# shivendrra/shredword-trainer

Measured on AMD Instinct MI355X. Metric: BPE merges/sec, higher is better.
Workload: dtype int32

## Files before the change

### include/shredword_bpe.h

```cpp
#ifndef SHREDWORD_BPE_H
#define SHREDWORD_BPE_H

#include <stddef.h>
#include <stdint.h>

#ifdef __cplusplus
extern "C" {
#endif

typedef struct BPEConfig {
  size_t target_vocab_size;
  int32_t unk_id;
  float character_coverage;
  uint64_t min_pair_freq;
} BPEConfig;

typedef struct Trainer Trainer;

Trainer* create_trainer(const BPEConfig* config);
void bpe_trainer_destroy(Trainer* trainer);
int bpe_load_corpus(Trainer* trainer, const char* input_path);
void bpe_init(Trainer* trainer);
void bpe_count_bigrams(Trainer* trainer);
int bpe_merge_batch(Trainer* trainer, int batch_size);
// ... 11 lines not shown
int updateTokenScores(void* trainer, char** texts, int n);
int trainUnigram(void* trainer, char** texts, int n, int iterations);
int getVocab(void* trainer, char*** tokens, double** scores, int* n);
int saveVocab(void* trainer, const char* path);
int loadVocab(void* trainer, const char* path);

int shred_set_option(Trainer* trainer, const char* key, const char* value);
int shred_reset(Trainer* trainer);
typedef const void* (*shred_gather_fn)(void* ctx, const void* send, size_t nbytes, size_t* out_bytes);
int shred_set_load_gather(Trainer* trainer, int rank, int world, shred_gather_fn gather, void* ctx);
double shred_probe_merge(Trainer* trainer, int32_t a, int32_t b, int iters);
int shred_probe_rollback(Trainer* trainer, int32_t a, int32_t b);
int64_t shred_debug_tokens(Trainer* trainer, int32_t* out, size_t cap);

int64_t shred_index_trace(Trainer* trainer, uint32_t* out, size_t cap);

typedef struct ShredStats {
  double load_seconds, init_seconds, train_seconds;
  double host_select_seconds, host_launch_seconds, host_wait_seconds, host_apply_seconds;
  double merge_kernel_ms, count_kernel_ms;
  double merge_kernel_bytes, count_kernel_bytes;
  uint64_t merge_launches, count_launches;
  uint64_t num_words, num_symbols, num_occurrences, num_merges, heap_size, live_tokens;
  uint64_t device_bytes, num_tiles;
  int32_t layout, world_size;
  uint64_t heap_pops, heap_stale_pops, heap_pushes, delta_records, tiles_visited;
  uint64_t apply_cycles_combine, apply_cycles_order, apply_cycles_walk;
  uint64_t spec_hits, spec_misses;
  uint64_t exchange_overflows;
  double hist_kernel_ms, hist_kernel_bytes;
  uint64_t hist_launches;
  uint64_t resident_launches;
  double resident_ms;
  double resident_latency_us;
  uint64_t load_on_gpu;
  uint64_t index_on;
  uint64_t index_merges, index_undos, index_launches;
  uint64_t index_candidates;
  uint64_t index_changed;
  uint64_t index_occurrences;
  double index_ms;
  double index_dev_us;
  double index_wait_us;
  double index_dev_lookup_us;
  double index_dev_scan_us;
  uint64_t index_scanned;
  double index_build_us;
  uint64_t index_no_sub;
  uint64_t index_staged;
  int64_t index_switch_merge;
  double index_switch_ms;
  uint64_t resident_aborts;
  uint64_t verify_checks;
  uint64_t verify_failures;
  uint64_t resident_merges;
  double resident_bytes;
  double resident_kernel_ms;
  uint64_t index_run_ints_read;
  uint64_t index_run_ints_written;
  uint64_t index_records;
  double resident_k3_bytes;
  uint64_t sel_merges;
  uint64_t sel_launches;
  uint64_t sel_rebuilds;
  double sel_kernel_ms;
  double sel_rebuild_ms;
  double sel_select_us;
  double sel_merge_us;
  uint64_t sel_table_pairs;
  uint64_t sel_table_slots;
  uint64_t sel_host_merges;
  uint64_t sel_table_grows;
  uint64_t index_raw_records;
  uint64_t index_finalized;
  double index_dev_out_us;
  double index_dev_fin_us;
  uint64_t index_fin_records;
  double sel_table_us;
  uint64_t index_spill_merges;
  uint64_t index_spill_keys;
  double host_apply_combine_seconds, host_apply_correct_seconds, host_apply_finish_seconds;
  double host_apply_early_seconds, host_apply_offer_seconds;
  uint64_t helper_adopted, apply_cycles_push;
} ShredStats;
int shred_get_stats(const Trainer* trainer, ShredStats* out);

int shred_device_count(void);

int shred_hbm_probe(int device, size_t bytes, int reps, double* read_gbps, double* copy_gbps);

void* shred_occupy(int device, int free_cus, double max_seconds);
void shred_release(void* handle);

int shred_dist_unique_id(void* out, size_t cap);
int shred_dist_init(int rank, int world_size, const void* unique_id, size_t len, int device);
int shred_dist_finalize(void);
int shred_dist_ranks(void);

#ifdef __cplusplus
}
#endif
#endif
```

### shredword-trainer_amd/csrc/hip/bpe_device.hip

```cpp
#include <algorithm>
#include <cstring>
#include <iterator>

#include "../host/device.h"
#include "../host/dist.h"
#include "hip_common.h"

namespace shred {

namespace {

constexpr uint32_t kFusedCollectMax = 4096;
constexpr uint32_t kNeedCollect = 0x80000000u;
constexpr uint32_t kTimingStride = 8;
constexpr uint32_t kInlineTiles = 768;
constexpr int kGroup = 4;
constexpr uint32_t kWin = 32;
constexpr int kMaxChain = 8;
constexpr int kChainShift = 27;
constexpr uint32_t kMtLds = 256;
[[maybe_unused]] constexpr int kStamps = 18;
#ifdef SHRED_STAMPS
#define STAMP(k) \
  if (threadIdx.x == 0) p.stamps[blockIdx.x * kStamps + (k)] = __builtin_amdgcn_s_memrealtime()
// ... 1437 lines not shown
  const u64* hs = (const u64*)(sl.host_count + 4);
  size_t n;
  const uint32_t nm = launched ? sl.host_count[2] : 0;
  const DeltaRecord* all = sl.host_recs;
  if (exchange_) {
    n = exchange_finish(sl, &all);
  } else {
    n = sl.host_count[0];
    if (n & kNeedCollect) {
      n &= ~kNeedCollect;
      k_collect<<<256, kThreads, 0, S(aux_stream_)>>>(sl.dcount, sl.dlist, U(sl.dsum), U(sl.dft),
                                                        drec + sl.host_count[3]);
      HIP_OK(hipGetLastError());
      k_zero_u32<<<1, 1, 0, S(aux_stream_)>>>(sl.dcount);
      HIP_OK(hipGetLastError());
      HIP_OK(hipStreamSynchronize(S(aux_stream_)));
    }
  }
  if (run_.n == 1) {
    run_.rp[0] = all;
    run_.rn[0] = n;
    run_.tp[0] = sl.host_mlist;
    run_.tn[0] = nm;
  } else {
    for (int i = 0; i < run_.n; ++i) {
      run_.recs[i].clear();
      run_.tiles[i].clear();
    }
    const DeltaRecord* r = all;
    for (size_t i = 0; i < n; ++i) {
      const uint32_t j = r[i].key / keys_per_merge_;
      if (j >= (uint32_t)run_.n) fatal("k_merge record of a merge outside the chain");
      DeltaRecord d = r[i];
      d.key -= j * keys_per_merge_;
      run_.recs[j].push_back(d);
    }
    for (uint32_t i = 0; i < nm; ++i) {
      const uint32_t e = sl.host_mlist[i];
      const uint32_t j = e >> kChainShift;
      if (j >= (uint32_t)run_.n) fatal("k_merge matched tile of a merge outside the chain");
      run_.tiles[j].push_back(e & ((1u << kChainShift) - 1u));
    }
    for (int i = 0; i < run_.n; ++i) {
      run_.rp[i] = run_.recs[i].data();
      run_.rn[i] = run_.recs[i].size();
      run_.tp[i] = run_.tiles[i].data();
      run_.tn[i] = run_.tiles[i].size();
    }
  }
  if (timing_) flush_timing(false);
  if (launched) live_tokens_est_ -= hs[0];
  records_total_ += n;
  records_max_ = std::max<uint64_t>(records_max_, n);
  if (merge_log_) {
    std::fprintf(merge_log_, "C %u %d %u %u %d %llu %zu", sl.seq, run_.X0, sl.n_iter, sl.grid, run_.n,
                 (unsigned long long)hs[0], n);
#ifdef SHRED_STAMPS
    std::vector<u64> st((size_t)sl.grid * kStamps);
    HIP_OK(hipStreamSynchronize(S(stream_)));
    HIP_OK(hipMemcpy(st.data(), stamps_, st.size() * sizeof(u64), hipMemcpyDeviceToHost));
    u64 t0 = ~0ull;
    for (uint32_t g = 0; g < sl.grid; ++g) t0 = std::min(t0, st[(size_t)g * kStamps]);
    for (int k = 1; k < 8; ++k) {
      u64 mx = 0;
      for (uint32_t g = 0; g < sl.grid; ++g) {
        const u64 v = st[(size_t)g * kStamps + k];
        if (v != 0 && v != ~0ull) mx = std::max(mx, v);
      }
      std::fprintf(merge_log_, " %.2f", mx >= t0 ? (double)(mx - t0) / 100.0 : -1.0);
    }
    std::fprintf(merge_log_, " %.0f", st[4] > st[0] ? (double)(st[17] - st[16]) / (double)(st[4] - st[0]) * 100.0 : -1.0);
    for (int k = 8; k < 16; ++k) {
      const u64 v = st[k], s0 = st[0];
      std::fprintf(merge_log_, " %.2f", v >= s0 && v != 0 ? (double)(v - s0) / 100.0 : -1.0);
    }
    HIP_OK(hipMemset(stamps_, 0, st.size() * sizeof(u64)));
#endif
    std::fprintf(merge_log_, "\n");
  }
}

size_t Device::collect(int32_t X, const DeltaRecord** recs) {
  HIP_OK(hipSetDevice(ordinal_));
  last_changes_ = false;
  if (wl_ && wl_->in_flight()) {
    const size_t n = wl_->collect(X, recs);
    last_changes_ = wl_->last_changes();
    records_total_ += n;
    records_max_ = std::max<uint64_t>(records_max_, n);
    return n;
  }
  if (!res_posted_.empty()) return collect_resident(X, recs);
  if (run_count_ == 0) fatal("collect: no launch in flight");
  ChainRun& run = run_at(0);
  const int j = X - run.X0;
  if (j != run.collected || j >= run.n) fatal("collect: merge X is not the next merge of the oldest launch");
  if (!run.waited) finish_launch(run);
  index_.set_tiles(X, run.tp[j], run.tn[j]);
  ++run.collected;
  *recs = run.rp[j];
  const size_t n = run.rn[j];
  if (run.collected == run.n) {
    run_head_ = (run_head_ + 1) & 1;
    --run_count_;
  }
  return n;
}

bool Device::peek(int32_t X, const DeltaRecord** recs, size_t* n) {
  return wl_ && wl_->in_flight() && wl_->peek(X, recs, n);
}

void Device::rollback(int32_t X) {
  HIP_OK(hipSetDevice(ordinal_));
  if (wl_ && wl_->in_flight()) {
    wl_->rollback(X);
    ++rollbacks_;
    return;
  }
  if (!res_posted_.empty()) {
    undo_resident_from(X);
    return;
  }
  park();
  ++rollbacks_;
  for (int k = run_count_ - 1; k >= 0; --k) {
    ChainRun& run = run_at(k);
    const int j0 = std::max(X - run.X0, run.collected);
    if (j0 >= run.n) continue;
    if (!run.waited && run.n == 1) {
      if (ntiles_) unmerge_launch(run, nullptr, 0);
      slot_[run.slot].launched = false;
      run.waited = true;
    } else {
      if (!run.waited) finish_launch(run);
      unmerge_run(run, j0);
    }
    run.n = j0;
  }
  while (run_count_ > 0 && run_at(run_count_ - 1).collected == run_at(run_count_ - 1).n) --run_count_;
}

void Device::unmerge_run(ChainRun& run_, int j0) {
  const int nundo = run_.n - j0;
  if (!ntiles_ || nundo <= 0) return;
  ulist_.clear();
  for (int j = j0; j < j0 + nundo; ++j) ulist_.insert(ulist_.end(), run_.tp[j], run_.tp[j] + run_.tn[j]);
  if (nundo > 1) {
    std::sort(ulist_.begin(), ulist_.end());
    ulist_.erase(std::unique(ulist_.begin(), ulist_.end()), ulist_.end());
  }
  MergeSlot& sl = slot_[run_.slot];
  if (merge_log_) std::fprintf(merge_log_, "R %u %d %zu %d\n", sl.seq, run_.X0 + j0, ulist_.size(), nundo);
  if (ulist_.empty()) return;
  if (unmerge_pending_) HIP_OK(hipStreamSynchronize(S(stream_)));
  std::memcpy(host_ulist_, ulist_.data(), ulist_.size() * sizeof(uint32_t));
  unmerge_pending_ = true;
  unmerge_launch(run_, host_ulist_, ulist_.size(), j0);
}

void Device::unmerge_launch(ChainRun& run_, const uint32_t* tiles, size_t n_tiles, int j0) {
  const int nundo = run_.n - j0;
  MergeSlot& sl = slot_[run_.slot];
  UnmergeParams& up = *static_cast<UnmergeParams*>(unmerge_params_);
  up.tok = tok_;
  up.tile_off = tile_off_;
  up.tile_len = tile_len_;
  if (tiles) {
    void* d = nullptr;
    HIP_OK(hipHostGetDevicePointer(&d, const_cast<uint32_t*>(tiles), 0));
    up.tiles = (const uint32_t*)d;
    up.ntl = (uint32_t)n_tiles;
    up.ntl_dev = nullptr;
  } else {
    up.tiles = (const uint32_t*)sl.dev_mlist;
    up.ntl = 0;
    up.ntl_dev = (const uint32_t*)sl.dev_count + 2;
  }
  up.nundo = nundo;
  up.ux0 = run_.X0 + j0;
  for (int j = 0; j < nundo; ++j) {
    up.ua[j] = run_.ab[2 * (j0 + j)];
    up.ub[j] = run_.ab[2 * (j0 + j) + 1];
  }
  up.dcount = sl.dcount;
  up.dlist = sl.dlist;
  up.dsum = U(sl.dsum);
  up.dft = U(sl.dft);
  up.sig = sig_;
  const int grid = tiles ? (int)std::min<size_t>((n_tiles + kWaves - 1) / kWaves, (size_t)kMaxMergeGroups)
                         : kMaxMergeGroups;
  k_unmerge<<<grid, kThreads, 0, S(stream_)>>>(up);
  HIP_OK(hipGetLastError());
}
// ... 34 lines not shown
```

### shredword-trainer_amd/csrc/hip/word_loop.hip

```cpp
#include <hip/hip_runtime.h>
#include <hipcub/hipcub.hpp>

#include <algorithm>
#include <cstdio>
#include <cstdlib>
#include <cstring>
#include <functional>
#include <thread>
#include <vector>

#include "../host/common.h"
#include "../host/word_loop.h"
#include "hip_common.h"

namespace shred {

namespace {

constexpr int kWlThreads = 512;
constexpr int kDh = 2048;
constexpr int kStripV = 7;
constexpr int kStrip = 4 * kStripV;
constexpr uint32_t kRunHdr = 3;
constexpr uint32_t kStripTok = kStrip - kRunHdr;
constexpr uint32_t kRunAlign = 4;
__host__ __device__ constexpr uint32_t run_cap(uint32_t len) {
  return (kRunHdr + len + kRunAlign - 1u) & ~(kRunAlign - 1u);
}
constexpr int kB = 8;
#ifdef SHRED_WL_NO_PREFETCH
constexpr bool kWlPrefetch = false;
#else
constexpr bool kWlPrefetch = true;
#endif
constexpr int kQ = kWlThreads * kB + kWlThreads;
constexpr int kBSelf = 6;
template <bool kSelf>
struct QueueShape {
  static constexpr int kBatch = kSelf ? kBSelf : kB;
  static constexpr int kCap = kWlThreads * kBatch + kWlThreads;
};
#ifdef SHRED_WL_STAMPS
#define WL_ST(...) __VA_ARGS__
#else
#define WL_ST(...)
#endif
constexpr int kXs = 16;
typedef int v4i_t __attribute__((ext_vector_type(4)));
__device__ __forceinline__ void st16(void* dst, int4 v) {
#ifdef SHRED_WL_NT_WORDS
  v4i_t x = {v.x, v.y, v.z, v.w};
  __builtin_nontemporal_store(x, reinterpret_cast<v4i_t*>(dst));
#else
  *reinterpret_cast<int4*>(dst) = v;
#endif
}
__device__ __forceinline__ void wl_stamp(uint32_t* xs, int i, unsigned long long t0) {
#ifdef SHRED_WL_STAMPS
  const unsigned long long now = __builtin_amdgcn_s_memrealtime();
  if ((threadIdx.x >> 6) == 0 && (threadIdx.x & 63) == (uint32_t)(__ffsll((long long)__ballot(1)) - 1))
    xs[i] = (uint32_t)(now - t0);
#endif
}
constexpr uint32_t kDeltaBucketsDev = 1024;
constexpr uint32_t kRing = 64;
constexpr uint32_t kOpMerge = 1, kOpStop = 2, kOpTimeout = 3, kOpUnmerge = 4;
constexpr uint32_t kNoList = 0xFFFFFFFFu;
constexpr int kStPoolTop = 1, kStError = 3;
constexpr uint32_t kErrPool = 1, kErrList = 2, kErrLookup = 4;

struct WlCmd {
  u64 g[8];
};
constexpr int kCmdGranules = 6;

struct WlSlotDev {
  DeltaRecord* recs;
  uint32_t* hdr;
  uint32_t rec_cap;
};

struct WEnt {
  u64 e;
  u64 sig;
};
__host__ __device__ __forceinline__ u64 hand_weight(uint32_t i) { return 0x9E3779B97F4A7C15ull + 2ull * i; }
constexpr int kCksWord = 30;
constexpr int kGroupShift = 28;
constexpr u64 kWordMask = (1ull << kGroupShift) - 1;
__host__ __device__ __forceinline__ uint32_t ent_groups(u64 e) { return (uint32_t)(e >> kGroupShift) & 0xFu; }

struct SelParams {
  u64* tab;
  u64 pmask;
  uint32_t* fr[2];
  uint32_t fcap;
  uint32_t* st;
  const u64* thr;
  u64* out;
  u64* log;
  u64 log_cap;
  int32_t X0;
  uint32_t n_max;
  u64 min_freq;
  uint32_t fill_max;
  uint32_t probe;
};
constexpr int kSelM = 0, kSelNF = 1, kSelBuf = 2, kSelStatus = 3, kSelIns = 4, kSelErr = 5, kSelStats = 6;
constexpr int kSelWords = kSelStats + 2 * 12 + 2;
constexpr int kSelLogW = kSelStats + 2 * 12;
constexpr uint32_t kSelDone = 1, kSelRebuild = 2, kSelFull = 3;
constexpr uint32_t kSelF = 1536, kSelK = 768, kSelRoom = 384, kSelSlack = 96;
constexpr u64 kCntMask = (1ull << 48) - 1;
constexpr int kPosShift = 48;
template <bool kOn>
struct SelLds {
  u64 key[1], cnt[1];
  uint32_t idx[1], n;
};
constexpr uint32_t kSelIdx = 4096;
template <>
struct SelLds<true> {
  u64 key[kSelF], cnt[kSelF];
  uint32_t idx[kSelIdx / 2], n;
};
struct WlParams {
  int32_t* wtok;
  const u64* weight;
  WEnt* pool;
  u64 pool_cap;
  const u64* dkey;
  const u64* dval;
  u64 dir_mask;
  u64* lst;
  uint32_t* lseq;
  uint32_t id_cap;
  u64* dsum;
  u64* dft;
  uint32_t* dlist;
  uint32_t* dstate;
  uint32_t cap;
  int32_t unk;
  const WlCmd* ring;
  uint32_t* status;
  uint32_t seq0;
  uint32_t idle_polls;
  uint32_t fin_max;
  uint32_t fin_min;
  uint32_t prefetch;
  uint32_t drain;
  uint32_t fast;
  WlSlotDev sl[WordLoop::kSlots];
  SelParams sel;
};

__device__ __forceinline__ u64 pair_key(int32_t a, int32_t b) { return ((u64)(uint32_t)a << 32) | (uint32_t)b; }
__device__ __forceinline__ uint32_t sel_idx_home(u64 k) { return (uint32_t)(mix64(k) >> 40) & (kSelIdx - 1); }
__device__ __forceinline__ int sel_idx_find(const SelLds<true>& F, u64 k) {
  uint32_t h = sel_idx_home(k);
#pragma unroll 1
  for (uint32_t probe = 0; probe < kSelIdx; ++probe) {
    const uint32_t v = (F.idx[h >> 1] >> ((h & 1u) * 16u)) & 0xFFFFu;
    if (v == 0) return -1;
    if (F.key[v - 1u] == k) return (int)(v - 1u);
    h = (h + 1u) & (kSelIdx - 1u);
  }
  return -1;
}
__device__ __forceinline__ bool sel_idx_insert(SelLds<true>& F, u64 k, uint32_t pos) {
  uint32_t h = sel_idx_home(k);
#pragma unroll 1
  for (uint32_t probe = 0; probe < kSelIdx;) {
    const uint32_t sh = (h & 1u) * 16u;
    const uint32_t old = F.idx[h >> 1];
    if (((old >> sh) & 0xFFFFu) == 0u) {
      if (atomicCAS(&F.idx[h >> 1], old, old | ((pos + 1u) << sh)) == old) return true;
      continue;
    }
    h = (h + 1u) & (kSelIdx - 1u);
    ++probe;
  }
  return false;
}

__device__ __forceinline__ u64 nbit(int32_t id, uint32_t s) {
  const uint32_t v = (uint32_t)id * 2u + s;
  return 1ull << ((v ^ (v >> 6) ^ (v >> 12) ^ (v >> 18)) & 63u);
}
__device__ __forceinline__ uint32_t ld_agent(const uint32_t* p) {
  return __hip_atomic_load(p, __ATOMIC_RELAXED, __HIP_MEMORY_SCOPE_AGENT);
}
__device__ __forceinline__ u64 ld_agent64(const u64* p) {
  return __hip_atomic_load(p, __ATOMIC_RELAXED, __HIP_MEMORY_SCOPE_AGENT);
}
__device__ __forceinline__ bool sel_better(u64 c, u64 k, u64 c2, u64 k2) { return c > c2 || (c == c2 && k < k2); }
__device__ __forceinline__ bool sel_at_least(u64 c, u64 k, u64 tc, u64 tk) { return c > tc || (c == tc && k <= tk); }
__device__ __forceinline__ u64 sel_slot(const SelParams& q, u64 pk, uint32_t* ins, uint32_t* err) {
  u64 h = mix64(pk) & q.pmask;
#pragma unroll 1
  for (uint32_t probe = 0; probe < 4096u; ++probe) {
    const u64 cur = ld_agent64(q.tab + 2 * h);
    if (cur == pk) return h;
    if (cur == kEmpty64) {
      const u64 prev = atomicCAS(q.tab + 2 * h, kEmpty64, pk);
      if (prev == kEmpty64) {
        atomicAdd(ins, 1u);
        return h;
      }
      if (prev == pk) return h;
    }
    h = (h + 1) & q.pmask;
  }
  atomicMax(err, 1u);
  return ~0ull;
}
struct SelNew {
  u64* key;
  u64* cnt;
  uint32_t* n;
  uint32_t cap;
  u64* dxa;
  uint32_t* over;
  u64* log;
  uint32_t* nlog;
};
__device__ __forceinline__ void sel_record(const SelParams& q, SelLds<true>& F, const SelNew& nw, int32_t unk,
                                           uint32_t key, u64 sum, int32_t a, int32_t b, int32_t X) {
  const uint32_t sl = key >> 2, cat = key & 3u;
  const int32_t id = sl == 0 ? unk : (int32_t)(sl - 1u);
  if (id == unk || sum == 0) return;
  const int32_t f = cat < 2u ? id : (cat == 2u ? b : X);
  const int32_t g = cat == 0u ? a : (cat == 1u ? X : id);
  if (f == a && g == b) return;
  const u64 pk = pair_key(f, g);
// ... 146 lines not shown
    const int32_t t1 = j + 1 < (int)kStripTok ? run_at(x, (int)kRunHdr + 1 + j) : 0;
    const bool emit = (uint32_t)j < L && !skip;
    const bool m = emit && (uint32_t)(j + 1) < L && t0 == a && t1 == b;
    s[(emit ? kRunHdr + k : 0u) * kWlThreads] = m ? X : t0;
    xm |= (m ? 1u : 0u) << k;
    k += emit ? 1u : 0u;
    skip = m;
  }
  if (xs) wl_stamp(xs, 4, t0);
  *len = k;
  *sig = 0;
  if (!xm) return 0;
  const uint32_t occ = (uint32_t)__popc(xm);
  const u64 rank = (e & kWordMask) << 32;
  uint32_t m = xm, o = 0;
  u64 f = 0;
  while (__ballot(m != 0u)) {
    if (m) {
      const uint32_t ko = (uint32_t)__ffs(m) - 1u;
      m &= m - 1u;
      const uint32_t jo = ko + o;
      ++o;
      const int32_t prev = ko > 0 ? s[(kRunHdr - 1u + ko) * kWlThreads] : 0;
      const bool has_n = jo + 2 < L;
      const int32_t nx = has_n ? s[(kRunHdr + 1u + ko) * kWlThreads] : 0;
      f |= occurrence<kProbes>(p, h, c, ko > 0, prev, has_n, nx == X ? a : nx, wc, rank | ((u64)jo << 2));
    }
  }
  if (xs) wl_stamp(xs, 5, t0);
  *sig = f;
  s[0] = (int32_t)k;
  int4* r4 = reinterpret_cast<int4*>(r);
  const uint32_t q0 = ((uint32_t)__ffs(xm) + kRunHdr - 1u) >> 2;
  int4 v[kStripV];
#pragma unroll
  for (int q = 0; q < kStripV; ++q) {
    v[q].x = s[(4 * q + 0) * kWlThreads];
    v[q].y = s[(4 * q + 1) * kWlThreads];
    v[q].z = s[(4 * q + 2) * kWlThreads];
    v[q].w = s[(4 * q + 3) * kWlThreads];
  }
  v[0].y = x.v[0].y;
  v[0].z = x.v[0].z;
#pragma unroll
  for (int q = 0; q < kStripV; ++q)
    if ((uint32_t)q <= ((k + kRunHdr - 1u) >> 2) && (q == 0 || (uint32_t)q >= q0)) st16(&r4[q], v[q]);
  if (xs) wl_stamp(xs, 6, t0);
  return occ;
}

__device__ __forceinline__ uint32_t unmerge_run(int32_t* t, uint32_t L, int32_t a, int32_t b, int32_t X) {
  uint32_t nx = 0;
  for (uint32_t j = 0; j < L; ++j) nx += t[j] == X;
  if (!nx) return L;
  uint32_t q = L + nx;
  for (uint32_t j = L; j-- > 0;) {
    const int32_t v = t[j];
    if (v == X) {
      t[--q] = b;
      t[--q] = a;
    } else {
      t[--q] = v;
    }
  }
  return L + nx;
}

__device__ __forceinline__ u64 wave_max64(u64 x) { return lane_read64(wave_scan_max64(x), 63); }

__device__ __forceinline__ uint32_t wave_incl_add(uint32_t x) {
  const int lane = threadIdx.x & 63;
#pragma unroll
  for (int d = 1; d < 64; d <<= 1) {
    const uint32_t y = __shfl_up(x, d, 64);
    if (lane >= d) x += y;
  }
  return x;
}

struct LoopS {
  alignas(16) uint32_t hs[32];
  uint32_t cmd[8];
  uint32_t nout, nchg, pool_top, err, scan, filter, nspill, qn, nkeys, nfin;
  uint32_t rd, wr;
  u64 lst_x;
  u64 last_lst;
  int32_t last_x;
  uint32_t st[4];
  u64 lk[2];
  u64 need;
  u64 occ, t[2];
  u64 t_wait, t_idle, t_undo;
  u64 t_seen;
  uint32_t t_rel;
  uint32_t xs[kXs];
  uint32_t sm, snk, snew, status, sel_pos, sover, scompact, sins, serr;
  u64 sel_cnt, dxa, t_rec, t_app, logn;
  uint32_t lognew, newtot;
  u64 bc[kWlThreads / 64], bk[kWlThreads / 64];
  uint32_t bs[kWlThreads / 64];
};


constexpr uint32_t kFinMax = 1024;
constexpr uint32_t kFinTab = 2 * kFinMax;
constexpr u64 kFinEmpty = 0x7FFFFFFF7FFFFFFFull;
static_assert(4 * kFinMax <= (uint32_t)kQ, "record arrays in the queue");
static_assert(3 * kFinTab * 8 <= (uint32_t)(kStrip * kWlThreads * 4), "combine table in the strip");
static_assert(kDeltaBucketsDev * 4 <= kDh * 4, "bucket counters in the hash keys");

__device__ __forceinline__ void fin_record(u64* q, uint32_t r, uint32_t key, u64 sum, u64 ft, int32_t unk, int32_t a,
                                           int32_t b, int32_t X) {
  const uint32_t sl = key >> 2, cat = key & 3u;
  const int32_t id = sl == 0 ? unk : (int32_t)(sl - 1u);
  const int32_t f = cat < 2u ? id : (cat == 2u ? b : X);
  const int32_t g = cat == 0u ? a : (cat == 1u ? X : id);
  q[r] = ((u64)(int64_t)f << 32) | (u64)(int64_t)g;
  q[kFinMax + r] = (cat & 1u) ? sum : (u64)(-(int64_t)sum);
  q[2 * kFinMax + r] = ft;
}

__device__ __forceinline__ void fin_gather(const WlParams& p, DeltaH& h, LoopS& S, u64* q, int32_t a, int32_t b,
                                           int32_t X) {
  const uint32_t tid = threadIdx.x;
  for (int i = tid; i < kDh; i += kWlThreads) {
    const uint32_t key = h.key[i];
    if (key != kEmpty32) fin_record(q, atomicAdd(&S.nout, 1u), key, h.sum[i], h.ft[i], p.unk, a, b, X);
  }
  const uint32_t nsp = S.nspill;
  for (uint32_t i = tid; i < nsp; i += kWlThreads) {
    const uint32_t key = p.dlist[i];
    const u64 sum = atomicExch(&p.dsum[key], 0ull);
    const u64 ft = atomicExch(&p.dft[key], kEmpty64);
    fin_record(q, atomicAdd(&S.nout, 1u), key, sum, ft, p.unk, a, b, X);
  }
}

__device__ uint32_t finalize_wave(const u64* q, const WlSlotDev& sd, int32_t a, int32_t b, uint32_t n) {
  const int lane = threadIdx.x & 63;
  const bool mine = (uint32_t)lane < n;
  const u64 hk = mine ? q[lane] : kFinEmpty;
  const u64 d = mine ? q[kFinMax + lane] : 0ull;
  const u64 ft = mine ? q[2 * kFinMax + lane] : kEmpty64;
  const u64 kab = ((u64)(int64_t)a << 32) | (u64)(int64_t)b;
  u64 sum = 0;
  bool lead = mine && hk != kab;
#pragma unroll 1
  for (uint32_t j = 0; j < n; ++j) {
    const u64 hj = lane_read64(hk, (int)j), fj = lane_read64(ft, (int)j), dj = lane_read64(d, (int)j);
    const bool same = hj == hk;
    sum += same ? dj : 0ull;
    lead = lead && !(same && fj < ft);
  }
  const u64 lm = __ballot(lead);
  const uint32_t bk = (uint32_t)hk & (kDeltaBucketsDev - 1);
  uint32_t r = 0;
#pragma unroll 1
  for (u64 rest = lm; rest; rest &= rest - 1) {
    const uint32_t j = (uint32_t)__builtin_ctzll(rest);
    const uint32_t bj = (uint32_t)__builtin_amdgcn_readlane((int)(uint32_t)hk, (int)j) & (kDeltaBucketsDev - 1);
    const u64 fj = lane_read64(ft, (int)j);
    r += (bj < bk || (bj == bk && fj > ft)) ? 1u : 0u;
  }
  if (lead) {
    u64* dst = reinterpret_cast<u64*>(sd.recs + r);
    dst[0] = hk;
    dst[1] = sum;
    dst[2] = ft;
  }
  return (uint32_t)__popcll(lm);
}

__device__ uint32_t finalize_changes(const WlParams& p, DeltaH& h, LoopS& S, u64* q, u64* tab, const WlSlotDev& sd,
                                     int32_t a, int32_t b, int32_t X, uint32_t n) {
  const uint32_t tid = threadIdx.x;
  const int lane = tid & 63, wid = tid >> 6;
  u64* const fhk = q;
  u64* const fd = q + kFinMax;
  u64* const fft = q + 2 * kFinMax;
  u64* const mft = q + 3 * kFinMax;
  u64* const thk = tab;
  u64* const tft = tab + kFinTab;
  u64* const td = tab + 2 * kFinTab;
  uint32_t* const cnt = h.key;
  fin_gather(p, h, S, q, a, b, X);
  for (uint32_t i = tid; i < kFinTab; i += kWlThreads) {
    thk[i] = kFinEmpty;
    tft[i] = kEmpty64;
    td[i] = 0;
  }
  __syncthreads();
  constexpr int kPer = (int)(kFinMax / kWlThreads);
  uint32_t slot[kPer];
#pragma unroll
  for (int j = 0; j < kPer; ++j) {
    const uint32_t i = tid + (uint32_t)j * kWlThreads;
    slot[j] = 0;
    if (i < n) {
      const u64 hk = fhk[i];
      uint32_t t = (uint32_t)mix64(hk) & (kFinTab - 1);
#pragma unroll 1
// ... 238 lines not shown
        S.cmd[2] = b;
        S.cmd[3] = X;
        S.cmd[4] = (op >> 8) & 0xFFu;
        S.cmd[5] = expect;
        S.cmd[6] = lcnt1;
        S.cmd[7] = loff;
        S.t_wait = t_wait;
      }
    }
    __syncthreads();
    const uint32_t op = S.cmd[0];
    const int32_t a = (int32_t)S.cmd[1], b = (int32_t)S.cmd[2], X = (int32_t)S.cmd[3];
    const uint32_t slot = S.cmd[4], seq = S.cmd[5];
    ++expect;
    if (op != kOpMerge && op != kOpUnmerge) {
      exit_op = kSelf ? S.status : op;
      break;
    }
    const u64 t_cmd = __builtin_amdgcn_s_memrealtime();
    WL_ST(const u64 c_cmd = __builtin_amdgcn_s_memtime();)
    if (wid == 0) {
      const bool undo = op == kOpUnmerge;
      const int32_t M = undo ? X : (a > b ? a : b);
      const bool recent = !undo && M == S.last_x;
      const uint32_t given = undo ? 0u : (S.cmd[6] ? S.cmd[6] : recent ? (uint32_t)(S.last_lst >> 32) + 1u : 0u);
      const uint32_t goff = S.cmd[6] ? S.cmd[7] : (uint32_t)S.last_lst;
      u64 lv64 = 0;
      bool lv = false;
      if (!given && (lane == 16 || lane == 17) && M >= 0 && (uint32_t)M < p.id_cap) {
        if (lane == 16) lv = p.lseq[M] != kNoList;
        if (lane == 17) lv64 = p.lst[M];
      }
      const u64 key = pair_key(a, b);
      const u64 h = mix64(key) & p.dir_mask;
      u64 dk = kEmpty64, dv = 0;
      if (!given && !undo && lane < 16) {
        dk = p.dkey[(h + (u64)lane) & p.dir_mask];
        dv = p.dval[(h + (u64)lane) & p.dir_mask];
      }
      const bool has_list = given || ((__ballot(lv) >> 16) & 1ull);
      const u64 wl = given ? ((u64)goff | ((u64)(given - 1u) << 32)) : __shfl(lv64, 17, 64);
      u64 off = 0, cnt = 0, need = 0;
      bool err = false;
      if (has_list) {
        off = (uint32_t)wl;
        cnt = wl >> 32;
        if (!undo) need = a == b ? nbit(M, 0) : b == M ? nbit(a, 0) : nbit(b, 1);
      } else if (undo) {
        err = true;
      } else {
        for (u64 base = 0;; base += 16) {
          if (base) {
            dk = kEmpty64;
            if (lane < 16) {
              dk = p.dkey[(h + base + (u64)lane) & p.dir_mask];
              dv = p.dval[(h + base + (u64)lane) & p.dir_mask];
            }
          }
          const u64 hit = __ballot(lane < 16 && dk == key);
          const u64 emp = __ballot(lane < 16 && dk == kEmpty64);
          const u64 any = hit | emp;
          if (any) {
            const int f = __ffsll((long long)any) - 1;
            const u64 vf = __shfl(dv, f, 64);
            if ((hit >> f) & 1ull) {
              off = (uint32_t)vf;
              cnt = vf >> 32;
            } else {
              err = true;
            }
            break;
          }
          if (base > p.dir_mask) {
            err = true;
            break;
          }
        }
      }
      if (lane == 0) {
        S.lk[0] = off;
        S.lk[1] = err ? 0 : cnt;
        S.need = need;
        S.nout = 0;
        S.nchg = 0;
        S.scan = 0;
        S.rd = 0;
        S.wr = 0;
        S.nspill = 0;
        S.nkeys = 0;
        S.filter = need != 0;
        S.occ = 0;
        S.err = 0;
        S.st[0] = S.st[1] = S.st[2] = S.st[3] = 0;
        WL_ST(for (int i = 0; i < kXs; ++i) S.xs[i] = 0; S.xs[8] = given ? 1u : 0u;)
        if (err) atomicMax(&p.dstate[kStError], undo ? kErrList : kErrLookup);
        if (!undo && (u64)S.pool_top + cnt > p.pool_cap) {
          S.err = 1;
          atomicMax(&p.dstate[kStError], kErrPool);
        }
        S.t[0] = __builtin_amdgcn_s_memrealtime() - t_cmd;
      }
    }
    __syncthreads();
    WL_ST(if (tid == 0) S.xs[0] = (uint32_t)(__builtin_amdgcn_s_memrealtime() - t_cmd);)
    const u64 off = S.lk[0], cnt = S.lk[1];
    const uint32_t top = S.pool_top;
    if (op == kOpUnmerge) {
      for (u64 i = tid; i < cnt; i += kWlThreads) {
        const u64 e = p.pool[off + i].e;
        int32_t* r = p.wtok + (uint32_t)(e >> 32);
        const uint32_t L = (uint32_t)r[0];
        const uint32_t nl = unmerge_run(r + kRunHdr, L, a, b, X);
        if (nl != L) r[0] = (int32_t)nl;
      }
      __syncthreads();
      if (tid == 0 && X >= 0 && (uint32_t)X < p.id_cap) {
        if (off + cnt == (u64)S.pool_top) S.pool_top = (uint32_t)off;
        p.lseq[X] = kNoList;
        if (S.last_x == X) S.last_x = -1;
      }
      if (tid == 0) {
        S.t_idle += t_cmd - S.t_wait;
        S.t_undo += __builtin_amdgcn_s_memrealtime() - t_cmd;
      }
      __syncthreads();
      continue;
    }
    const bool append = S.err == 0;
    const u64 need = S.need;
    if ((fast || (kSelf && p.fast != 0)) && op == kOpMerge && cnt <= (u64)kWlThreads) {
      u64 e = kEmpty64;
      bool pass = false;
      if (tid < cnt) {
        const WEnt v = p.pool[off + tid];
        e = v.e;
        pass = (v.sig & need) == need;
      }
      WL_ST(if (pass) wl_stamp(S.xs, 2, t_cmd);)
      uint32_t occ = 0, L = 0, nl = 0;
      u64 nsig = 0;
      if (pass) {
        int32_t* r = p.wtok + (uint32_t)(e >> 32);
        const Run x = load_run(r, ent_groups(e));
        const u64 wc = run_weight(x);
        L = (uint32_t)x.v[0].x;
        nl = L;
        WL_ST(wl_stamp(S.xs, 3, t_cmd);)
        if (L >= 2) {
          if (L <= kStripTok) {
            occ = merge_regs<kProbes>(p, s_h, mc, mys, r, x, L, e, wc, a, b, X, &nl, &nsig
                                      WL_ST(, S.xs, t_cmd));
          } else {
            occ = merge_run<kProbes>(p, s_h, mc, r + kRunHdr, L, e, wc, a, b, X, &nl, &nsig);
            if (occ) r[0] = (int32_t)nl;
          }
        }
      }
      const u64 chg = __ballot(occ != 0);
      if (chg) {
        const int lead = __ffsll((long long)chg) - 1;
        uint32_t nb = 0;
        if (lane == lead) nb = atomicAdd(&S.nchg, (uint32_t)__popcll(chg));
        nb = __shfl(nb, lead, 64);
        if (occ && append) {
          WEnt ne;
          ne.e = e;
          ne.sig = nsig;
          st16(&p.pool[(u64)top + nb + (uint32_t)__popcll(chg & ((1ull << lane) - 1ull))],
               make_int4((int)(uint32_t)ne.e, (int)(uint32_t)(ne.e >> 32), (int)(uint32_t)ne.sig, (int)(uint32_t)(ne.sig >> 32)));
        }
      }
      if (const u64 sm = __ballot(pass)) {
        const uint32_t w_occ = wave_sum(occ), w_rd = wave_sum(pass ? 1u + L : 0u);
        const uint32_t w_wr = wave_sum(occ ? 1u + nl : 0u);
        if (lane == 0) {
          atomicAdd(&S.occ, (u64)w_occ);
          atomicAdd(&S.scan, (uint32_t)__popcll(sm));
          atomicAdd(&S.rd, w_rd);
          atomicAdd(&S.wr, w_wr);
        }
      }
      WL_ST(wl_stamp(S.xs, 7, t_cmd);)
      const u64 t_wait = S.t_wait;
      WL_ST(const u64 t_seen_m = S.t_seen;)
      asm volatile("s_waitcnt lgkmcnt(0)\n\ts_barrier" ::: "memory");
      if (p.drain != 0 || S.nspill) __syncthreads();
      WL_ST(wl_stamp(S.xs, 9, t_cmd);)
      if constexpr (!kSelf) {
        const uint32_t nchg = append ? S.nchg : 0u;
        if (wid == 0 && lane == 0 && X >= 0 && (uint32_t)X < p.id_cap) {
          p.lst[X] = (u64)top | ((u64)nchg << 32);
          p.lseq[X] = seq;
        }
        if (wid == kFlagWave) {
          const WlSlotDev& sd = p.sl[slot & (WordLoop::kSlots - 1)];
          const u64 t_out = __builtin_amdgcn_s_memrealtime();
          WL_ST(if (lane == 0) S.xs[12] = (uint32_t)(t_out - t_cmd);)
          const uint32_t nsp = S.nspill;
          uint32_t bw = s_kbits[lane];
          s_kbits[lane] = 0;
          const uint32_t nb = (uint32_t)__popc(bw);
          const uint32_t incl = wave_scan_add(nb);
          const uint32_t nk = (uint32_t)__builtin_amdgcn_readlane((int)incl, 63);
          uint32_t ri = incl - nb;
          WL_ST(if (lane == 0) S.xs[13] = (uint32_t)(__builtin_amdgcn_s_memrealtime() - t_cmd);)
          u64 cks = 0;
          for (; bw; bw &= bw - 1u, ++ri) {
            const uint32_t h = (uint32_t)lane * 32u + (uint32_t)__builtin_ctz(bw);
            u64* dst = reinterpret_cast<u64*>(sd.recs + ri);
            const u64 w0 = (u64)s_h.key[h], w1 = s_h.sum[h], w2 = s_h.ft[h];
            dst[0] = w0;
            dst[1] = w1;
            dst[2] = w2;
            cks += w0 * hand_weight(16u + 3u * ri) + w1 * hand_weight(17u + 3u * ri) + w2 * hand_weight(18u + 3u * ri);
            s_h.key[h] = kEmpty32;
            s_h.sum[h] = 0;
            s_h.ft[h] = kEmpty64;
          }
          WL_ST(if (lane == 0) S.xs[14] = (uint32_t)(__builtin_amdgcn_s_memrealtime() - t_cmd);)
          for (uint32_t i = (uint32_t)lane; i < nsp; i += 64u) {
            const uint32_t key = p.dlist[i];
            const u64 sum = atomicExch(&p.dsum[key], 0ull);
            const u64 ft = atomicExch(&p.dft[key], kEmpty64);
            u64* dst = reinterpret_cast<u64*>(sd.recs + nk + i);
            dst[0] = (u64)key;
            dst[1] = sum;
            dst[2] = ft;
            const uint32_t r = nk + i;
            cks += (u64)key * hand_weight(16u + 3u * r) + sum * hand_weight(17u + 3u * r) + ft * hand_weight(18u + 3u * r);
          }
          WL_ST(if (lane == 0) S.xs[10] = (uint32_t)(__builtin_amdgcn_s_memrealtime() - t_cmd);)
          if (lane == 0) {
            S.lst_x = 0;
            S.last_x = -1;
            if (X >= 0 && (uint32_t)X < p.id_cap) {
              S.pool_top = top + nchg;
              S.lst_x = (u64)top | ((u64)(nchg + 1u) << 32);
              S.last_x = X;
              S.last_lst = (u64)top | ((u64)nchg << 32);
            }
            uint32_t* hs = S.hs;
            u64* hs64 = reinterpret_cast<u64*>(hs);
            const u64 now = __builtin_amdgcn_s_memrealtime();
            hs[0] = nk + nsp;
            hs[1] = 0u;
            hs[2] = (uint32_t)cnt;
            hs[3] = S.nchg;
            hs64[2] = S.occ;
            hs64[3] = now - t_cmd;
            hs64[4] = S.t[0];
            hs64[5] = t_out - t_cmd;
            hs[12] = S.scan;
            hs[13] = S.filter;
            hs[14] = S.rd;
            hs[15] = S.wr;
            hs[16] = hs[17] = hs[18] = 0u;
            hs[19] = nsp;
            hs[20] = (uint32_t)(S.t_idle + (t_cmd - t_wait));
            hs[21] = (uint32_t)S.t_undo;
            hs[22] = 0u;
            hs[23] = nk + nsp;
            hs64[12] = S.lst_x;
            hs64[13] = t_cmd;
            hs64[14] = t_wait;
            hs[30] = (uint32_t)(now - t_out);
            hs[31] = S.t_rel;
            S.t_idle = 0;
            S.t_undo = 0;
          }
          if (lane < 8) {
            const int4 hv = reinterpret_cast<const int4*>(S.hs)[lane];
            reinterpret_cast<int4*>(sd.hdr)[lane] = hv;
            const u64 lo = (u64)(uint32_t)hv.x | ((u64)(uint32_t)hv.y << 32), hi = (u64)(uint32_t)hv.z | ((u64)(uint32_t)hv.w << 32);
            cks += lo * hand_weight(2u * lane) + hi * hand_weight(2u * lane + 1u);
          }
          {
            cks += dpp64<0x111>(cks);
            cks += dpp64<0x112>(cks);
            cks += dpp64<0x114>(cks);
            cks += dpp64<0x118>(cks);
            cks += dpp64<0x142, 0xa, false>(cks);
            cks += dpp64<0x143, 0xc, false>(cks);
            cks = lane_read64(cks, 63);
          }
          if (lane == 0) {
            const u64 t_r0 = __builtin_amdgcn_s_memrealtime();
            WL_ST(sd.hdr[48] = (uint32_t)t_seen_m;
                const u64 c_now = __builtin_amdgcn_s_memtime(); const u64 t_now = __builtin_amdgcn_s_memrealtime();
                  S.xs[1] = (uint32_t)((c_now - c_cmd) * 100ull / (t_now - t_cmd + 1ull));
                  S.xs[11] = (uint32_t)(t_r0 - t_cmd); for (int i = 0; i < kXs; ++i) sd.hdr[32 + i] = S.xs[i];)
            u64* h64w = reinterpret_cast<u64*>(sd.hdr);
            h64w[kCksWord] = ((u64)seq << 32) | (cks & 0xFFFFFFFFull);
            h64w[kCksWord + 1] = ((u64)seq << 32) | (cks >> 32);
            __builtin_amdgcn_fence(__ATOMIC_RELEASE, "");
            S.t_rel = (uint32_t)(__builtin_amdgcn_s_memrealtime() - t_r0);
          }
        } else if (pfon && wid == poll_wave) {
          pre_v = lane < kCmdGranules
                      ? __hip_atomic_load(p.ring[expect % kRing].g + lane, __ATOMIC_RELAXED, __HIP_MEMORY_SCOPE_SYSTEM)
                      : 0ull;
          pre_ok = true;
        }
        continue;
      }
    } else {
    uint32_t my_occ = 0, my_scan = 0, my_rd = 0, my_wr = 0;
    if (tid == 0) S.qn = 0;
    for (u64 base = 0; base < cnt; base += (u64)kWlThreads * kBq) {
      u64 ex[kBq], sx[kBq];
#pragma unroll
      for (int q = 0; q < kBq; ++q) {
        const u64 i = base + (u64)q * kWlThreads + tid;
        ex[q] = kEmpty64;
        sx[q] = 0;
        if (i < cnt) {
          const WEnt v = p.pool[off + i];
          ex[q] = v.e;
          sx[q] = v.sig;
        }
      }
      if (base == 0 && tid == 0) {
        asm volatile("s_waitcnt vmcnt(0)" ::: "memory");
        S.st[0] = (uint32_t)(__builtin_amdgcn_s_memrealtime() - t_cmd);
      }
#pragma unroll
      for (int q = 0; q < kBq; ++q) {
        const bool pass = ex[q] != kEmpty64 && (sx[q] & need) == need;
        const u64 bl = __ballot(pass);
        if (bl) {
          const int lead = __ffsll((long long)bl) - 1;
          uint32_t qb = 0;
          if (lane == lead) qb = atomicAdd(&S.qn, (uint32_t)__popcll(bl));
          qb = __shfl(qb, lead, 64);
          if (pass) s_q[qb + (uint32_t)__popcll(bl & ((1ull << lane) - 1ull))] = ex[q];
        }
      }
      __syncthreads();
      const uint32_t qn = S.qn;
      __syncthreads();
      const bool last = base + (u64)kWlThreads * kBq >= cnt;
      if (qn < (uint32_t)kWlThreads && !last) continue;
      WL_ST(if (tid == 0) { if (!S.xs[1]) S.xs[1] = (uint32_t)(__builtin_amdgcn_s_memrealtime() - t_cmd); ++S.xs[9]; })
      const uint32_t qend = ((qn + kWlThreads - 1) / kWlThreads) * kWlThreads;
      u64 e_n = kEmpty64;
      Run x_n{};
      if (kWlPrefetch && tid < qn) {
        e_n = s_q[tid];
        x_n = load_run(p.wtok + (uint32_t)(e_n >> 32), ent_groups(e_n));
      }
      for (uint32_t qi = tid; qi < qend; qi += kWlThreads) {
        if (!kWlPrefetch && qi < qn) {
          e_n = s_q[qi];
          x_n = load_run(p.wtok + (uint32_t)(e_n >> 32), ent_groups(e_n));
        }
        const u64 e = e_n;
        const Run x = x_n;
        const u64 wc = run_weight(x);
// ... 154 lines not shown
        for (uint32_t i = tid; i < kSelIdx / 2; i += kWlThreads) s_f.idx[i] = 0;
        asm volatile("s_waitcnt lgkmcnt(0)\n\ts_barrier" ::: "memory");
        const uint32_t b0 = base;
#pragma unroll
        for (int j = 0; j < kPer; ++j) {
          const uint32_t i = (uint32_t)kPer * tid + (uint32_t)j;
          if (i >= n0 || !((keepm >> j) & 1u)) continue;
          s_f.cnt[base] = ck[j];
          s_f.key[base] = kk[j];
          ++base;
        }
        asm volatile("s_waitcnt lgkmcnt(0)\n\ts_barrier" ::: "memory");
        for (uint32_t i = b0; i < base; ++i)
          if (!sel_idx_insert(s_f, s_f.key[i], i)) S.sover = 1;
        asm volatile("s_waitcnt lgkmcnt(0)\n\ts_barrier" ::: "memory");
        if (tid == 0) {
          s_f.n = tot;
          ++S.scompact;
          if (tot > kSelF - kSelRoom) S.sover = 1;
        }
      }
      if (tid == 0) {
        q.st[kSelNF] = min(s_f.n, kSelF);
        q.st[kSelM] = S.sm + 1u;
        ++S.sm;
        u64* t64 = reinterpret_cast<u64*>(q.st + kSelStats);
        const u64 now = __builtin_amdgcn_s_memrealtime();
        t64[0] += t_cmd - S.t_wait;
        t64[1] += now - t_cmd;
        t64[2] += cnt;
        t64[3] += nchg;
        t64[4] += S.occ;
        t64[5] += nnew;
        t64[6] += now - t_tab;
        t64[7] += S.scompact ? 1u : 0u;
        t64[8] += S.t_rec - t_tab;
        t64[9] += S.t_app - S.t_rec;
        t64[10] += now - S.t_app;
        q.st[kSelBuf] = S.scompact;
        S.status = S.sover ? kSelRebuild : 0u;
      }
      __syncthreads();
      if (S.status) {
        exit_op = S.status;
        break;
      }
      continue;
    }
    const WlSlotDev& sd = p.sl[slot & (WordLoop::kSlots - 1)];
    if (tid == 0) {
      S.t[1] = __builtin_amdgcn_s_memrealtime() - t_cmd;
      S.lst_x = 0;
      if (X >= 0 && (uint32_t)X < p.id_cap) {
        p.lst[X] = (u64)top | ((u64)nchg << 32);
        p.lseq[X] = seq;
        S.pool_top = top + nchg;
        S.lst_x = (u64)top | ((u64)(nchg + 1u) << 32);
      }
      S.last_x = S.lst_x ? X : -1;
      S.last_lst = (u64)top | ((u64)nchg << 32);
    }
    const uint32_t nrec = S.nkeys + S.nspill;
    const bool fin = p.fin_max != 0 && nrec <= p.fin_max && nrec <= kFinMax && nrec >= p.fin_min;
    const u64 t_fin = __builtin_amdgcn_s_memrealtime();
    if (fin && nrec <= 64u) {
      fin_gather(p, s_h, S, s_q, a, b, X);
      __syncthreads();
      if (wid == 0) {
        const uint32_t m = finalize_wave(s_q, sd, a, b, nrec);
        if (lane == 0) S.nfin = m;
      }
      asm volatile("s_waitcnt vmcnt(0)" ::: "memory");
    } else if (fin) {
      finalize_changes(p, s_h, S, s_q, reinterpret_cast<u64*>(s_strip), sd, a, b, X, nrec);
      asm volatile("s_waitcnt vmcnt(0)" ::: "memory");
    } else if (pfon && wid == 1) {
      pre_v = lane < kCmdGranules
                  ? __hip_atomic_load(p.ring[expect % kRing].g + lane, __ATOMIC_RELAXED, __HIP_MEMORY_SCOPE_SYSTEM)
                  : 0ull;
      pre_ok = true;
    } else {
      const uint32_t rt = pfon ? (tid < 64u ? tid : tid - 64u) : tid;
      const uint32_t rs = pfon ? (uint32_t)kWlThreads - 64u : (uint32_t)kWlThreads;
      for (uint32_t i = rt; i < (uint32_t)kDh; i += rs) {
        const uint32_t key = s_h.key[i];
        if (key == kEmpty32) continue;
        const uint32_t r = atomicAdd(&S.nout, 1u);
        u64* dst = reinterpret_cast<u64*>(sd.recs + r);
        dst[0] = (u64)key;
        dst[1] = s_h.sum[i];
        dst[2] = s_h.ft[i];
        s_h.key[i] = kEmpty32;
        s_h.sum[i] = 0;
        s_h.ft[i] = kEmpty64;
      }
      const uint32_t nsp = S.nspill;
      for (uint32_t i = rt; i < nsp; i += rs) {
        const uint32_t key = p.dlist[i];
        const u64 sum = atomicExch(&p.dsum[key], 0ull);
        const u64 ft = atomicExch(&p.dft[key], kEmpty64);
        const uint32_t r = atomicAdd(&S.nout, 1u);
        u64* dst = reinterpret_cast<u64*>(sd.recs + r);
        dst[0] = (u64)key;
        dst[1] = sum;
        dst[2] = ft;
      }
      asm volatile("s_waitcnt vmcnt(0)" ::: "memory");
    }
    asm volatile("s_waitcnt lgkmcnt(0)\n\ts_barrier" ::: "memory");
    WL_ST(if (tid == 0) S.xs[10] = (uint32_t)(__builtin_amdgcn_s_memrealtime() - t_cmd);)
    if (fin)
      for (int i = tid; i < kDh; i += kWlThreads) {
        s_h.key[i] = kEmpty32;
        s_h.sum[i] = 0;
        s_h.ft[i] = kEmpty64;
      }
    if (tid == 0) {
      sd.hdr[0] = fin ? S.nfin : S.nout;
      sd.hdr[22] = fin ? 1u : 0u;
      sd.hdr[23] = nrec;
      sd.hdr[30] = (uint32_t)(__builtin_amdgcn_s_memrealtime() - t_fin);
      sd.hdr[2] = (uint32_t)cnt;
      sd.hdr[3] = S.nchg;
      u64* h64 = reinterpret_cast<u64*>(sd.hdr);
      h64[2] = S.occ;
      h64[3] = (u64)__builtin_amdgcn_s_memrealtime() - t_cmd;
      h64[4] = S.t[0];
      h64[5] = S.t[1];
      sd.hdr[12] = S.scan;
      sd.hdr[13] = S.filter;
      sd.hdr[14] = S.rd;
      sd.hdr[15] = S.wr;
      sd.hdr[16] = S.st[0];
      sd.hdr[17] = S.st[1];
      sd.hdr[18] = S.st[2];
      sd.hdr[19] = S.nspill;
      sd.hdr[20] = (uint32_t)(S.t_idle + (t_cmd - S.t_wait));
      sd.hdr[21] = (uint32_t)S.t_undo;
      sd.hdr[31] = S.t_rel;
      h64[12] = S.lst_x;
      h64[13] = t_cmd;
      h64[14] = S.t_wait;
      S.t_idle = 0;
      S.t_undo = 0;
      const u64 t_r0 = __builtin_amdgcn_s_memrealtime();
      WL_ST(S.xs[11] = (uint32_t)(t_r0 - t_cmd); for (int i = 0; i < kXs; ++i) sd.hdr[32 + i] = S.xs[i];)
      __hip_atomic_store(sd.hdr + 1, seq, __ATOMIC_RELEASE, __HIP_MEMORY_SCOPE_SYSTEM);
      S.t_rel = (uint32_t)(__builtin_amdgcn_s_memrealtime() - t_r0);
    }
    asm volatile("s_waitcnt lgkmcnt(0)\n\ts_barrier" ::: "memory");
  }
  if (tid == 0) {
    p.dstate[kStPoolTop] = S.pool_top;
    if constexpr (kSelf) {
      p.sel.st[kSelIns] = S.sins;
      *reinterpret_cast<u64*>(p.sel.st + kSelLogW) = S.logn;
      p.sel.st[kSelErr] = S.serr;
      p.sel.st[kSelStatus] = exit_op;
      __threadfence_system();
      return;
    }
    p.status[1] = expect - 1u;
    __threadfence_system();
    __hip_atomic_store(&p.status[0], exit_op, __ATOMIC_RELEASE, __HIP_MEMORY_SCOPE_SYSTEM);
  }
}

namespace {

__global__ void k_wl_pair_counts(const int32_t* wtok, const uint32_t* woff, uint32_t W, uint32_t* cnt) {
  for (uint32_t w = blockIdx.x * blockDim.x + threadIdx.x; w <= W; w += gridDim.x * blockDim.x) {
    const uint32_t L = w < W ? (uint32_t)wtok[woff[w]] : 0u;
    cnt[w] = L >= 2 ? L - 1 : 0u;
  }
}
__global__ void k_wl_emit_pairs(const int32_t* wtok, const uint32_t* woff, const uint32_t* base, uint32_t W,
                                int32_t unk, u64* key, uint32_t* val) {
  for (uint32_t w = blockIdx.x * blockDim.x + threadIdx.x; w < W; w += gridDim.x * blockDim.x) {
    const uint32_t o = woff[w], b = base[w], np = base[w + 1] - b;
    const int32_t* t = wtok + o + kRunHdr;
    for (uint32_t j = 0; j < np; ++j) {
      const int32_t x = t[j], y = t[j + 1];
      key[b + j] = (x != unk && y != unk) ? pair_key(x, y) : kEmpty64;
      val[b + j] = w;
    }
  }
}

__global__ void k_wl_mark(const u64* key, const uint32_t* val, uint64_t n, uint32_t* keep, uint32_t* head) {
  for (uint64_t i = blockIdx.x * (uint64_t)blockDim.x + threadIdx.x; i < n; i += (uint64_t)gridDim.x * blockDim.x) {
    const u64 k = key[i];
    const bool valid = k != kEmpty64;
    const bool first_key = valid && (i == 0 || key[i - 1] != k);
    keep[i] = valid && (first_key || val[i - 1] != val[i]);
    head[i] = first_key;
  }
}

__global__ void k_wl_scatter(const u64* key, const uint32_t* val, uint64_t n, const uint32_t* keep,
                             const uint32_t* pos, const uint32_t* head, const uint32_t* kidx, const uint32_t* woff,
                             WEnt* pool, u64* ikey, u64* ival) {
  for (uint64_t i = blockIdx.x * (uint64_t)blockDim.x + threadIdx.x; i < n; i += (uint64_t)gridDim.x * blockDim.x) {
// ... 136 lines not shown
    }
    const u64 bl = __ballot(take);
    if (!bl) continue;
    const int lead = __ffsll((long long)bl) - 1;
    uint32_t base = 0;
    if (lane == lead) base = atomicAdd(nout, (uint32_t)__popcll(bl));
    base = __shfl(base, lead, 64);
    const uint32_t pos = base + (uint32_t)__popcll(bl & ((1ull << lane) - 1ull));
    if (take && pos < cap) out[pos] = (uint32_t)i;
  }
}

__global__ void k_sel_gather(const uint32_t* slots, uint32_t n, const u64* tab, u64* key, u64* negc, uint32_t* idx) {
  for (uint32_t i = blockIdx.x * blockDim.x + threadIdx.x; i < n; i += gridDim.x * blockDim.x) {
    key[i] = tab[2 * (u64)slots[i]];
    negc[i] = ~(tab[2 * (u64)slots[i] + 1] & kCntMask);
    idx[i] = i;
  }
}

__global__ void k_sel_pick(const uint32_t* slots, const uint32_t* idx, uint32_t n, uint32_t* fr) {
  for (uint32_t i = blockIdx.x * blockDim.x + threadIdx.x; i < n; i += gridDim.x * blockDim.x)
    fr[i] = slots[idx ? idx[i] : i];
}

__global__ void k_sel_insert(const PairCount* pc, uint64_t n, SelParams q) {
  for (uint64_t i = blockIdx.x * (uint64_t)blockDim.x + threadIdx.x; i < n; i += (uint64_t)gridDim.x * blockDim.x) {
    const u64 h = sel_slot(q, pair_key(pc[i].a, pc[i].b), q.st + kSelIns, q.st + kSelErr);
    if (h != ~0ull) q.tab[2 * h + 1] = pc[i].count & kCntMask;
  }
}

__global__ void k_sel_apply_log(const u64* log, u64 n, SelParams q) {
  for (u64 i = blockIdx.x * (u64)blockDim.x + threadIdx.x; i < n; i += (u64)gridDim.x * blockDim.x) {
    const u64 h = sel_slot(q, log[2 * i], q.st + kSelIns, q.st + kSelErr);
    if (h != ~0ull) atomicAdd(q.tab + 2 * h + 1, log[2 * i + 1]);
  }
}

__global__ void k_sel_clear(u64* tab, u64 n) {
  for (u64 i = blockIdx.x * (u64)blockDim.x + threadIdx.x; i < n; i += (u64)gridDim.x * blockDim.x) {
    tab[2 * i] = kEmpty64;
    tab[2 * i + 1] = 0;
  }
}

__global__ void k_sel_export(const u64* tab, u64 cap, PairCount* out, uint32_t* n) {
  for (u64 i = blockIdx.x * (u64)blockDim.x + threadIdx.x; i < cap; i += (u64)gridDim.x * blockDim.x) {
    const u64 k = tab[2 * i], c = tab[2 * i + 1] & kCntMask;
    if (k == kEmpty64 || c == 0) continue;
    const uint32_t j = atomicAdd(n, 1u);
    out[j] = PairCount{(int32_t)(uint32_t)(k >> 32), (int32_t)(uint32_t)k, c, 0};
  }
}

template <class T>
T* wl_alloc(size_t n, size_t* acc) {
  void* p = nullptr;
  HIP_OK(hipMalloc(&p, std::max<size_t>(n, 1) * sizeof(T)));
  *acc += std::max<size_t>(n, 1) * sizeof(T);
  return static_cast<T*>(p);
}

constexpr uint32_t kRunPad = 4 * kStripV + 4;

}

WordLoop::WordLoop(int ordinal, void* stream, int32_t unk_id) : ordinal_(ordinal), stream_(stream), unk_(unk_id) {
  HIP_OK(hipSetDevice(ordinal_));
  const unsigned pin = hipHostMallocMapped | hipHostMallocCoherent;
  HIP_OK(hipHostMalloc(&ring_, sizeof(WlCmd) * kRing, pin));
  std::memset(ring_, 0, sizeof(WlCmd) * kRing);
  HIP_OK(hipHostGetDevicePointer(&ring_dev_, ring_, 0));
  HIP_OK(hipHostMalloc((void**)&status_, 64, pin));
  std::memset(status_, 0, 64);
  HIP_OK(hipHostGetDevicePointer(&status_dev_, status_, 0));
  if (const char* e = std::getenv("SHREDWORD_WL_IDLE_POLLS")) idle_polls_ = (uint32_t)std::strtoul(e, nullptr, 10);
  if (const char* e = std::getenv("SHREDWORD_WL_FINALIZE")) fin_max_ = (uint32_t)std::strtoul(e, nullptr, 10);
  if (const char* e = std::getenv("SHREDWORD_WL_FIN_MIN")) fin_min_ = (uint32_t)std::strtoul(e, nullptr, 10);
  if (const char* e = std::getenv("SHREDWORD_WL_PREFETCH")) prefetch_ = std::atoi(e) != 0;
  if (const char* e = std::getenv("SHREDWORD_WL_DRAIN")) drain_ = std::atoi(e) != 0;
  if (const char* e = std::getenv("SHREDWORD_WL_PROBES")) probes_ = std::atoi(e);
  if (const char* e = std::getenv("SHREDWORD_WL_FAST")) fast_ = std::atoi(e) != 0;
  if (const char* e = std::getenv("SHREDWORD_SELECT_REPORT")) sel_report_ = std::atoi(e) != 0;
  for (auto& e : ev_) {
    hipEvent_t ev;
    HIP_OK(hipEventCreate(&ev));
    e = ev;
  }
}

WordLoop::~WordLoop() {
  (void)hipSetDevice(ordinal_);
  if (running_ && posted_.empty()) stop();
  (void)hipStreamSynchronize(S(stream_));
  free_all();
  for (Slot& s : slot_) {
    if (s.host_recs) (void)hipHostFree(s.host_recs);
    if (s.host_hdr) (void)hipHostFree(s.host_hdr);
  }
  if (ring_) (void)hipHostFree(ring_);
  if (status_) (void)hipHostFree(status_);
  for (auto e : ev_)
    if (e) (void)hipEventDestroy((hipEvent_t)e);
}

void WordLoop::free_all() {
  sel_free();
  void* ptrs[] = {wtok_, wtok0_, woff_, tile_first_, tile_nw_, pool_, dkey_, dval_, init_key_, init_val_,
                  lst_, lseq_, dsum_, dft_, dlist_, dstate_};
  for (void* p : ptrs)
    if (p) HIP_OK(hipFree(p));
  wtok_ = wtok0_ = nullptr;
  woff_ = tile_first_ = tile_nw_ = lseq_ = dlist_ = dstate_ = nullptr;
  pool_ = dkey_ = dval_ = init_key_ = init_val_ = lst_ = dsum_ = dft_ = nullptr;
  cap_ = id_cap_ = 0;
  dir_cap_ = 0;
  bytes_ = 0;
  ready_ = false;
}

bool WordLoop::upload(const TiledStream& ts, const uint64_t* d_weight) {
  HIP_OK(hipSetDevice(ordinal_));
  if (running_) stop();
  free_all();
  const size_t T = ts.num_tiles();
  const int P = (int)std::max<size_t>(1, std::min<size_t>({16, std::max(1u, std::thread::hardware_concurrency()),
                                                          T / 64 + 1}));
  auto par = [&](const std::function<void(int)>& f) {
    if (P == 1) return f(0);
    std::vector<std::thread> pool;
    for (int k = 0; k < P; ++k) pool.emplace_back(f, k);
    for (auto& th : pool) th.join();
  };
  auto range = [&](int k, size_t* t0, size_t* t1) {
    *t0 = T * (size_t)k / (size_t)P;
    *t1 = T * (size_t)(k + 1) / (size_t)P;
  };
  std::vector<uint32_t> tnw(T, 0), tfirst(T, 0);
  std::vector<uint64_t> tints(T + 1, 0), ttok(T, 0);
  std::vector<int32_t> tr0(T, -1);
  std::vector<char> bad((size_t)P, 0);
  par([&](int k) {
    size_t t0, t1;
    range(k, &t0, &t1);
    for (size_t t = t0; t < t1 && !bad[(size_t)k]; ++t) {
      const int32_t* p = ts.tok.data() + ts.off[t];
      uint32_t nw = 0, wl = 0;
      uint64_t ints = 0, ntk = 0;
      for (uint32_t i = 0; i < ts.len[t]; ++i) {
        if (p[i] < kHeaderLimit) {
          const int32_t r = (int32_t)(uint32_t)(p[i] - kHeaderBase);
          if (nw == 0) tr0[t] = r;
          else if (r != tr0[t] + (int32_t)nw) bad[(size_t)k] = 1;
          if (nw) ints += run_cap(wl);
          ++nw;
          wl = 0;
        } else {
          if (nw == 0) bad[(size_t)k] = 1;
          ++wl;
          ++ntk;
        }
      }
      if (nw) ints += run_cap(wl);
      tnw[t] = nw;
      tints[t] = ints;
// ... 232 lines not shown

void WordLoop::ensure_slots(uint32_t cap) {
  const uint32_t rec_cap = 4 * (cap + 1) + 64;
  const unsigned pin = hipHostMallocMapped | hipHostMallocNonCoherent;
  for (Slot& sl : slot_) {
    if (sl.host_recs) HIP_OK(hipHostFree(sl.host_recs));
    HIP_OK(hipHostMalloc((void**)&sl.host_recs, (size_t)rec_cap * sizeof(DeltaRecord), pin));
    HIP_OK(hipHostGetDevicePointer(&sl.dev_recs, sl.host_recs, 0));
    if (!sl.host_hdr) {
      HIP_OK(hipHostMalloc((void**)&sl.host_hdr, 256, pin));
      std::memset(sl.host_hdr, 0, 256);
      HIP_OK(hipHostGetDevicePointer(&sl.dev_hdr, sl.host_hdr, 0));
    }
    sl.rec_cap = rec_cap;
  }
}

void WordLoop::reserve(int32_t max_id) {
  const uint32_t need = (uint32_t)std::max<int32_t>(max_id, 0) + 2 + kSlots;
  if (need <= cap_ && dsum_) return;
  if (!posted_.empty()) fatal("WordLoop::reserve with a merge in flight");
  stop();
  uint32_t cap = std::max<uint32_t>(cap_ ? cap_ : 4096, 4096);
  while (cap < need) cap *= 2;
  hipStream_t s = S(stream_);
  for (void* p : {(void*)dsum_, (void*)dft_, (void*)dlist_})
    if (p) HIP_OK(hipFree(p));
  const size_t keys = 4 * ((size_t)cap + 1);
  dsum_ = wl_alloc<u64>(keys, &bytes_);
  dft_ = wl_alloc<u64>(keys, &bytes_);
  dlist_ = wl_alloc<uint32_t>(keys, &bytes_);
  HIP_OK(hipMemsetAsync(dsum_, 0, keys * sizeof(u64), s));
  HIP_OK(hipMemsetAsync(dft_, 0xFF, keys * sizeof(u64), s));
  u64* nl = wl_alloc<u64>(cap, &bytes_);
  uint32_t* ns = wl_alloc<uint32_t>(cap, &bytes_);

  HIP_OK(hipMemsetAsync(ns, 0xFF, (size_t)cap * sizeof(uint32_t), s));

  if (lseq_) {
    HIP_OK(hipMemcpyAsync(nl, lst_, (size_t)id_cap_ * sizeof(u64), hipMemcpyDeviceToDevice, s));
    HIP_OK(hipMemcpyAsync(ns, lseq_, (size_t)id_cap_ * sizeof(uint32_t), hipMemcpyDeviceToDevice, s));

    HIP_OK(hipStreamSynchronize(s));
    for (void* q : {(void*)lst_, (void*)lseq_}) HIP_OK(hipFree(q));
  }
  lst_ = nl;
  lseq_ = ns;

  id_cap_ = cap;
  cap_ = cap;
  lists_.resize(cap, 0ull);
  ensure_slots(cap);
  HIP_OK(hipStreamSynchronize(s));
}

void WordLoop::launch(uint32_t seq0) {
  WlParams p{};
  p.wtok = wtok_;
  p.weight = weight_;
  p.pool = reinterpret_cast<WEnt*>(pool_);
  p.pool_cap = pool_cap_;
  p.dkey = dkey_;
  p.dval = dval_;
  p.dir_mask = dir_cap_ - 1;
  p.lst = lst_;
  p.lseq = lseq_;

  p.id_cap = id_cap_;
  p.dsum = dsum_;
  p.dft = dft_;
  p.dlist = dlist_;
  p.dstate = dstate_;
  p.cap = cap_;
  p.unk = unk_;
  p.ring = static_cast<const WlCmd*>(ring_dev_);
  p.status = static_cast<uint32_t*>(status_dev_);
  p.seq0 = seq0;
  p.idle_polls = idle_polls_;
  p.fin_max = fin_max_;
  p.fin_min = fin_min_;
  p.prefetch = prefetch_ ? 1u : 0u;
  p.drain = drain_ ? 1u : 0u;
  p.fast = fast_ ? 1u : 0u;
  for (int k = 0; k < kSlots; ++k) {
    p.sl[k].recs = static_cast<DeltaRecord*>(slot_[k].dev_recs);
    p.sl[k].hdr = static_cast<uint32_t*>(slot_[k].dev_hdr);
    p.sl[k].rec_cap = slot_[k].rec_cap;
  }
  status_[0] = 0;
  HIP_OK(hipEventRecord((hipEvent_t)ev_[0], S(stream_)));
  switch (probes_) {
    case 0: k_word_loop<false, 0><<<1, kWlThreads, 0, S(stream_)>>>(p); break;
    case 1: k_word_loop<false, 1><<<1, kWlThreads, 0, S(stream_)>>>(p); break;
    default: k_word_loop<false, kProbesDefault><<<1, kWlThreads, 0, S(stream_)>>>(p); break;
  }
  HIP_OK(hipGetLastError());
  HIP_OK(hipEventRecord((hipEvent_t)ev_[1], S(stream_)));
  running_ = true;
  ++st_.launches;
}

void WordLoop::recover_timeout() {
  HIP_OK(hipStreamSynchronize(S(stream_)));
  running_ = false;
  const uint32_t next = __atomic_load_n(&status_[1], __ATOMIC_ACQUIRE);
  if (next != seq_ + 1) {
    if (seq_ + 1 - next > kRing) fatal("k_word_loop: more commands behind its time-out than the ring holds");
    launch(next);
  }
}

uint32_t WordLoop::post(uint32_t op, int32_t a, int32_t b, int32_t X, uint32_t loff, uint32_t lcnt1) {
  if (running_ && __atomic_load_n(&status_[0], __ATOMIC_ACQUIRE) == kOpTimeout) recover_timeout();
  if (!running_) {
    if (op == kOpStop) return 0;
    launch(seq_ + 1);
  }
  const uint32_t seq = ++seq_;
  const uint32_t slot = (uint32_t)X & (kSlots - 1);
  u64* g = static_cast<WlCmd*>(ring_)[seq % kRing].g;
  const uint32_t vals[kCmdGranules] = {op | (slot << 8), (uint32_t)a, (uint32_t)b, (uint32_t)X, loff, lcnt1};
  for (int k = 0; k < kCmdGranules; ++k) __atomic_store_n(&g[k], (u64)seq | ((u64)vals[k] << 32), __ATOMIC_RELAXED);
  std::atomic_thread_fence(std::memory_order_release);
  return seq;
}

void WordLoop::post_merge(int32_t a, int32_t b, int32_t X) {
  if (!ready_) fatal("WordLoop::post_merge before upload");
  if (posted_.size() >= (size_t)kSlots) fatal("WordLoop: every merge slot is in flight");
  if (X < 0 || (uint32_t)X + 2 > cap_) fatal("WordLoop: merge id beyond the reserved ids");
  const int32_t M = a > b ? a : b;
  const uint64_t l = M >= 0 && (size_t)M < lists_.size() ? lists_[M] : 0;
  const uint32_t seq = post(kOpMerge, a, b, X, (uint32_t)l, (uint32_t)(l >> 32));
  posted_.push_back({X, a, b, seq, now_seconds()});
  dirty_ = true;
}

bool WordLoop::handed_over(const Slot& sl, uint32_t seq) const {
  const uint64_t* h64 = reinterpret_cast<const uint64_t*>(sl.host_hdr);
  const uint64_t g0 = __atomic_load_n(&h64[kCksWord], __ATOMIC_ACQUIRE), g1 = __atomic_load_n(&h64[kCksWord + 1], __ATOMIC_ACQUIRE);
  if ((uint32_t)(g0 >> 32) != seq || (uint32_t)(g1 >> 32) != seq) return false;
  const uint64_t want = (g0 & 0xFFFFFFFFull) | (g1 << 32);
  const uint32_t n = __atomic_load_n(&sl.host_hdr[0], __ATOMIC_ACQUIRE);
  if (n > sl.rec_cap) return false;
  uint64_t c = 0;
  for (uint32_t i = 0; i < 16; ++i) c += __atomic_load_n(&h64[i], __ATOMIC_RELAXED) * hand_weight(i);
  const uint64_t* r = reinterpret_cast<const uint64_t*>(sl.host_recs);
  for (uint32_t i = 0; i < 3 * n; ++i) c += __atomic_load_n(&r[i], __ATOMIC_RELAXED) * hand_weight(16u + i);
  return c == want;
}

void WordLoop::wait_flag(const Slot& sl, uint32_t seq) {
  volatile uint32_t* flag = sl.host_hdr + 1;
  const uint64_t* h64 = reinterpret_cast<const uint64_t*>(sl.host_hdr);
  const double t0 = now_seconds();
  unsigned spins = 0;
  for (;;) {
    if (__atomic_load_n(flag, __ATOMIC_ACQUIRE) == seq) break;
    if ((uint32_t)(__atomic_load_n(&h64[kCksWord + 1], __ATOMIC_ACQUIRE) >> 32) == seq && handed_over(sl, seq)) break;
    __builtin_ia32_pause();
    if (++spins % 4096 != 0) continue;
    const uint32_t st = __atomic_load_n(&status_[0], __ATOMIC_ACQUIRE);
    if (st == kOpTimeout) {
      recover_timeout();
    } else if (st != 0) {
      fatal("k_word_loop ended with a merge in flight");
    }
    if (now_seconds() - t0 > 60.0) {
      const hipError_t e = hipStreamQuery(S(stream_));
      if (e != hipSuccess && e != hipErrorNotReady) HIP_OK(e);
      if (now_seconds() - t0 > 300.0) fatal("k_word_loop did not signal completion within 300 s");
    }
  }
}

size_t WordLoop::collect(int32_t X, const DeltaRecord** recs) {
  if (posted_.empty() || posted_.front().X != X) fatal("WordLoop::collect: X is not the oldest posted merge");
  const Post pp = posted_.front();
  posted_.erase(posted_.begin());
  const Slot& sl = slot_[(uint32_t)X & (kSlots - 1)];
  wait_flag(sl, pp.seq);
  const double t_seen = now_seconds();
  st_.wait_us += 1e6 * (t_seen - pp.t_post);
  const uint32_t* h = sl.host_hdr;
  const uint64_t* h64 = reinterpret_cast<const uint64_t*>(h);
  const size_t n = h[0];
  st_.merges += 1;
  st_.candidates += h[2];
  st_.scanned += h[12];
  st_.run_ints_read += h[14];
  st_.run_ints_written += h[15];
  st_.records += h[0];
  st_.raw_records += h[22] ? h[23] : h[0];
  st_.finalized += h[22] ? 1u : 0u;
  st_.dev_out_us += 1e-2 * (double)h[30];
  st_.dev_rel_us += 1e-2 * (double)h[31];
  st_.spill_merges += h[19] ? 1u : 0u;
  st_.spill_keys += h[19];
  if (h[22]) {
    st_.dev_fin_us += 1e-2 * (double)h[30];
    st_.fin_records += h[23];
  }
  last_changes_ = h[22] != 0;
  st_.changed += h[3];
  st_.occurrences += h64[2];
  st_.dev_us += 1e-2 * (double)h64[3];
  st_.dev_lookup_us += 1e-2 * (double)h64[4];
  st_.dev_scan_us += 1e-2 * (double)(h64[5] - h64[4]);
  if (timing_) {
    const uint32_t rec[kTraceFields] = {(uint32_t)X, h[2], h[12], h[3], (uint32_t)h64[2], (uint32_t)(10 * h64[3]),
                                        (uint32_t)(10 * h64[4]), (uint32_t)(10 * (h64[5] - h64[4])),
                                        10 * h[16], 10 * h[17], 10 * h[18], h[19], 10 * h[20],
                                        10 * h[21], (uint32_t)(1e9 * (t_seen - pp.t_post)),
                                        (uint32_t)(1e8 * (pp.t_post - t_epoch_)), (uint32_t)(1e8 * (t_seen - t_epoch_)),
                                        (uint32_t)h64[13], (uint32_t)h64[14],
                                        h[32], h[33], h[34], h[35], h[36], h[37], h[38], h[39], h[40], h[41],
                                        h[42], h[43], h[44], h[45], h[46], h[47],
                                        h[31], h[48]};
    trace_.insert(trace_.end(), rec, rec + kTraceFields);
  }
  if (n > sl.rec_cap) fatal("k_word_loop: record overflow");
  if (h64[12] && (size_t)X < lists_.size()) lists_[X] = h64[12];
  *recs = sl.host_recs;
  return n;
}

bool WordLoop::peek(int32_t X, const DeltaRecord** recs, size_t* n) const {
  if (posted_.empty() || posted_.front().X != X) return false;
  const Slot& sl = slot_[(uint32_t)X & (kSlots - 1)];
  if (__atomic_load_n(sl.host_hdr + 1, __ATOMIC_ACQUIRE) != posted_.front().seq &&
      !handed_over(sl, posted_.front().seq))
    return false;
  if (sl.host_hdr[22]) return false;
  const size_t k = sl.host_hdr[0];
  if (k > sl.rec_cap) return false;
  *recs = sl.host_recs;
  *n = k;
  return true;
}

void WordLoop::rollback(int32_t X) {
  while (!posted_.empty() && posted_.back().X >= X) {
    const Post pp = posted_.back();
    posted_.pop_back();
    post(kOpUnmerge, pp.a, pp.b, pp.X);
    ++st_.undos;
  }
}

void WordLoop::stop() {
  if (!running_) return;
  HIP_OK(hipSetDevice(ordinal_));
  if (!posted_.empty()) fatal("WordLoop::stop with a merge in flight");
  post(kOpStop, 0, 0, 0);
  HIP_OK(hipStreamSynchronize(S(stream_)));
  running_ = false;
  float ms = 0;
  HIP_OK(hipEventElapsedTime(&ms, (hipEvent_t)ev_[0], (hipEvent_t)ev_[1]));
  st_.kernel_ms += ms;
  uint32_t ds[8];
  HIP_OK(hipMemcpy(ds, dstate_, sizeof(ds), hipMemcpyDeviceToHost));

  if (std::getenv("SHREDWORD_WL_REPORT") && st_.merges)
    std::fprintf(stderr, "[WL] %llu merges: device %.2f us a merge, of it the flag's system release %.2f us, "
                 "records out %.2f us; %llu merges spilled %llu delta keys to HBM\n", (unsigned long long)st_.merges,
                 st_.dev_us / (double)st_.merges, st_.dev_rel_us / (double)st_.merges,
                 st_.dev_out_us / (double)st_.merges, (unsigned long long)st_.spill_merges,
                 (unsigned long long)st_.spill_keys);
  if (ds[kStError]) {
    static const char* what[] = {"", "index pool exhausted", "an undone merge had no word list", "",
                                 "a merged pair had no word list"};
    std::fprintf(stderr, "[ERROR]\t k_word_loop: %s (code %u)\n", ds[kStError] < 5 ? what[ds[kStError]] : "?",
                 ds[kStError]);
    fatal("k_word_loop failed");
  }
}


void WordLoop::sel_free() {
  void* ptrs[] = {ptab_, fr_[0], fr_[1], sst_dev_, thr_, sout_, upd_, shist_, scol_};
  for (void* q : ptrs)
    if (q) HIP_OK(hipFree(q));
  ptab_ = thr_ = sout_ = nullptr;
  fr_[0] = fr_[1] = sst_dev_ = upd_ = shist_ = scol_ = nullptr;
  pcap_ = sout_cap_ = upd_cap_ = scol_cap_ = 0;
  fcap_ = 0;
}

bool WordLoop::sel_rebuild(uint64_t min_freq) {
  const double t0 = now_seconds();
  hipStream_t s = S(stream_);
  HIP_OK(hipMemsetAsync(shist_, 0, kSelBuckets * sizeof(uint32_t), s));
  k_sel_hist<<<1024, 512, 0, s>>>(ptab_, pcap_, min_freq, shist_);
  HIP_OK(hipGetLastError());
  std::vector<uint32_t> hist(kSelBuckets);
  HIP_OK(hipMemcpyAsync(hist.data(), shist_, kSelBuckets * sizeof(uint32_t), hipMemcpyDeviceToHost, s));
  HIP_OK(hipStreamSynchronize(s));
  uint64_t acc = 0;
  uint32_t bstar = kSelBuckets;
  for (uint32_t b = kSelBuckets; b-- > 0;) {
    if (!hist[b]) continue;
    acc += hist[b];
    bstar = b;
    if (acc >= kSelK) break;
  }
  uint32_t st[kSelStats] = {};
  HIP_OK(hipMemcpyAsync(st, sst_dev_, sizeof(st), hipMemcpyDeviceToHost, s));
  HIP_OK(hipStreamSynchronize(s));
  u64 thr[2] = {~0ull, 0ull};
  uint32_t nf = 0;
  if (acc > 0) {
    if (acc > scol_cap_) {
      if (scol_) HIP_OK(hipFree(scol_));
      scol_cap_ = std::max<uint64_t>(2 * acc, 1 << 16);
      scol_ = wl_alloc<uint32_t>(scol_cap_ + 1, &bytes_);
    }
// ... 293 lines not shown
```

### shredword-trainer_amd/csrc/host/device.h

```cpp
#pragma once

#include <algorithm>
#include <cstddef>
#include <cstdio>
#include <cstdint>
#include <string>
#include <vector>

#include "corpus.h"
#include "engine.h"
#include "selector.h"
#include "tiles.h"
#include "word_loop.h"

namespace shred {

struct KernelTimes {
  double merge_ms = 0;
  double compact_ms = 0;
  double count_ms = 0;
  uint64_t merge_launches = 0;
  uint64_t count_launches = 0;
  double merge_bytes = 0;
  double count_bytes = 0;
  double hist_ms = 0;
  double hist_bytes = 0;
  uint64_t hist_launches = 0;
  uint64_t res_merges = 0;
  double res_bytes = 0;
  double res_k3_bytes = 0;
  double res_ms = 0;
};

class Device : public Backend {
 public:
  static bool available(std::string* why);
  static int hbm_probe(int ordinal, size_t bytes, int reps, double* read_gbps, double* copy_gbps);
  static void* occupy(int ordinal, int free_cus, double max_seconds);
  static void release(void* handle);

  explicit Device(int device_ordinal);
  ~Device();
  Device(const Device&) = delete;
  Device& operator=(const Device&) = delete;

  void upload(const TiledStream& ts, Layout layout, const std::vector<uint64_t>& weights, int32_t max_id);
  void reset_tokens();
  bool has_tokens() const { return ntiles_ > 0 || uploaded_; }

  void count_pairs(int32_t unk_id, std::vector<PairCount>* out) override;
  void pair_max(int32_t unk_id, int32_t a, int32_t b, uint64_t* max_freq, uint64_t* ab_freq) override;

  void merge_chain(const int32_t* ab, int n, int32_t X0) override;
  int device_select(const std::vector<PairCount>& pairs, int32_t X0, int n, uint64_t min_freq,
                    std::vector<SelectedMerge>* out) override;
  bool device_select_now() const override { return !hybrid_resident_phase() || switch_pending_; }
  struct Exchange {
    int rank = 0, world = 1;
    void* comm = nullptr;
    void (*allgather)(void* comm, const void* send, void* recv, size_t bytes, void* stream) = nullptr;
    uint32_t bucket_records = 1024;
  };
  void set_exchange(const Exchange& x);
  size_t collect(int32_t X, const DeltaRecord** recs) override;
  bool records_are_changes() const override { return last_changes_; }
  bool peek(int32_t X, const DeltaRecord** recs, size_t* n) override;
  static constexpr int kChainMax = 8;
  int max_chain() const override {
    return speculate_ && !resident_eligible() && !index_eligible() ? kChainMax : 1;
  }
  bool index_id_room(int32_t max_id) const;
  bool can_overlap() const override {
    if (switch_pending_) return false;
    if (index_eligible()) return speculate_ && index_id_room(max_id_seen_ + 1 + spec_depth_);
    return speculate_ && (!resident_eligible() || (uint32_t)max_id_seen_ + 3 < min_slot_cap());
  }
  static constexpr int kResSlots = 4;
  int overlap_depth() const override { return resident_eligible() || index_eligible() ? spec_depth_ : 1; }
  int max_guesses() const override { return resident_eligible() || index_eligible() ? kResSlots - 1 : 1; }
  void set_spec_depth(int d) { spec_depth_ = std::max(1, std::min(d, kResSlots - 1)); }
  uint32_t min_slot_cap() const {
    uint32_t c = UINT32_MAX;
    for (const MergeSlot& s : slot_) c = std::min(c, s.cap);
    return c;
  }
  void reserve_ids(int32_t max_id) override;
  uint64_t exchange_overflows() const { return x_overflows_; }
  void rollback(int32_t X) override;
  void quiesce() override { park(); }
  void park();
  void set_resident(bool on);
  bool resident() const { return resident_on_; }
  bool resident_eligible() const { return resident_on_ && resident_ok_ && !exchange_ && !index_eligible(); }
  void set_index(bool on);
  bool index_on() const { return index_on_; }
  bool hybrid_resident_phase() const {
    return hybrid_ && !idx_phase_ && resident_on_ && resident_ok_ && !exchange_ && ntiles_ > 0;
  }
  bool index_eligible() const {
    return index_on_ && wl_ && wl_->ready() && !exchange_ && !hybrid_resident_phase();
  }
  void set_hybrid(bool on) {
    park();
    hybrid_ = on;
  }
  void set_switch_occurrences(uint64_t n) { switch_occ_ = n; }
  void set_finalize(int64_t n) {
    fin_ = n;
    if (wl_ && n >= 0) {
      index_sync();
      wl_->set_finalize((uint32_t)n);
    }
  }
  int64_t switch_merge() const { return switch_x_; }
  double switch_ms() const { return switch_ms_; }
  const WordLoop* word_loop() const { return wl_; }
  uint64_t resident_launches() const { return res_launches_; }
  uint64_t resident_aborts() const { return res_aborts_; }
  bool resident_tokens_in_lds() const { return res_lds_tok_; }
  double resident_ms() const { return res_ms_; }
  double resident_latency_us() const { return res_lat_n_ ? res_lat_us_ / (double)res_lat_n_ : 0.0; }
  void set_speculation(bool on) { speculate_ = on; }
  uint64_t rollbacks() const { return rollbacks_; }
  void set_merge_groups(int groups);

  void token_freq(size_t T, std::vector<uint64_t>* freq) override;
  void download_tokens(std::vector<int32_t>* out);

  void set_timing(bool on) {
    timing_ = on;
    if (wl_) wl_->set_timing(on);
  }
  const KernelTimes& times() {
    flush_timing(true);
    return times_;
  }
  void set_unk(int32_t unk) { unk_ = unk; }
  uint64_t records_total() const { return records_total_; }
  uint64_t visited_tiles() const { return visited_tiles_; }
  uint64_t records_max() const { return records_max_; }
  void clear_times() {
    flush_timing(true);
    times_ = KernelTimes();
    records_total_ = records_max_ = 0;
    visited_tiles_ = 0;
    res_launches_ = 0;
    res_ms_ = res_lat_us_ = 0;
    res_lat_n_ = 0;
// ... 47 lines not shown
    int32_t ab[2 * kChainMax] = {};
    const DeltaRecord* rp[kChainMax] = {};
    size_t rn[kChainMax] = {};
    const uint32_t* tp[kChainMax] = {};
    size_t tn[kChainMax] = {};
    std::vector<DeltaRecord> recs[kChainMax];
    std::vector<uint32_t> tiles[kChainMax];
  };
  void ensure_slots(MergeSlot& s, uint32_t need);
  void free_slot(MergeSlot& s, bool keep_host);
  void free_all();
  void wait_flag(const MergeSlot& s);
  void finish_launch(ChainRun& run);
  size_t exchange_bucket_bytes() const { return 32 + (size_t)xchg_.bucket_records * 24; }
  void exchange_launch(MergeSlot& sl);
  size_t exchange_finish(MergeSlot& sl, const DeltaRecord** recs);
  void count_pairs_dense(int32_t unk_id, uint64_t live, std::vector<PairCount>* out);
  struct PairMaxQuery {
    int32_t a, b;
    uint64_t max_freq, ab_freq;
  };
  PairMaxQuery* pmq_ = nullptr;
  void reduce_pair_max(const PairCount* dout, uint32_t n);
  void unmerge_run(ChainRun& run, int j0);
  void unmerge_launch(ChainRun& run, const uint32_t* tiles, size_t n_tiles, int j0 = 0);
  void flush_timing(bool block);
  void rebuild_signatures();

  int ordinal_ = 0;
  void* stream_ = nullptr;
  void* aux_stream_ = nullptr;
  void* ev_[6] = {};
  static constexpr int kEvPairs = 16;
  void* mev_[kEvPairs][2] = {};
  struct PendingEv {
    int pair;
    double bytes;
  };
  std::vector<PendingEv> ev_pending_;
  std::vector<int> ev_free_;
  bool timing_ = false;
  KernelTimes times_;
  Exchange xchg_;
  bool exchange_ = false;
  uint8_t* xrecv2_ = nullptr;
  size_t xrecv2_bytes_ = 0;
  std::vector<uint8_t> xstage_;
  uint64_t x_overflows_ = 0;
  int cu_count_ = 256;
  bool uploaded_ = false;
  Layout layout_ = Layout::kTypes;

  size_t ntiles_ = 0;
  size_t tok_elems_ = 0;
  int32_t* tok_ = nullptr;
  int32_t* tok0_ = nullptr;
  uint64_t* tile_off_ = nullptr;
  uint32_t* tile_len_ = nullptr;
  uint32_t* tile_len0_ = nullptr;
  uint64_t* weight_ = nullptr;
  uint64_t live_tokens0_ = 0;
  uint32_t* sig_ = nullptr;
  unsigned long long* stamps_ = nullptr;
  uint64_t nentries_ = 0;
  size_t ft_tiles_ = 0;
  uint64_t ft_live_tokens_ = 0;
  uint64_t live_tokens_est_ = 0;

  MergeSlot slot_[kResSlots];
  ChainRun runs_[2];
  int run_head_ = 0, run_count_ = 0;
  ChainRun& run_at(int k) { return runs_[(run_head_ + k) & 1]; }
  uint32_t keys_per_merge_ = 0;
  uint32_t* host_ulist_ = nullptr;
  void* dev_ulist_ = nullptr;
  std::vector<uint32_t> ulist_;
  bool unmerge_pending_ = false;
  uint32_t seq_ = 0;
  int32_t unk_ = 0;
  uint64_t records_total_ = 0, records_max_ = 0;
  int32_t max_id_seen_ = 0;
  int32_t max_id0_ = 0;
  bool speculate_ = true;
  bool last_changes_ = false;
  int64_t fin_ = -1;
  uint64_t rollbacks_ = 0;

  void* merge_params_ = nullptr;
  void* unmerge_params_ = nullptr;
  int max_groups_ = 256;
  FILE* merge_log_ = nullptr;
  TileIndex index_;
  bool skip_ = true;
  std::vector<uint32_t> cand_, cand1_, cand2_;
  uint64_t visited_tiles_ = 0;
  int merge_blocks_per_cu_ = 4;

  size_t bytes_alloc_ = 0;

  void index_sync();
  void index_refresh();
  WordLoop* wl_ = nullptr;
  bool index_on_ = true;
  bool words_stale_ = false;
  bool wl_pristine_index_ = true;
  bool hybrid_ = true;
  bool idx_phase_ = false;
  bool switch_pending_ = false;
  uint64_t switch_occ_ = 2000;
  static constexpr int kSwitchWindow = 64;
  uint64_t sw_win_[kSwitchWindow] = {};
  uint64_t sw_n_ = 0;
  int64_t switch_x_ = -1;
  double switch_ms_ = 0;
  int32_t reserved_max_id_ = 0;
  void hybrid_switch(int32_t X);
  void resident_abort_fallback();
  std::vector<void*> retired_streams_;
  uint64_t res_aborts_ = 0;
  uint32_t* res_arrive_ = nullptr;
  uint32_t res_arrive_polls_ = 20000;
  uint32_t res_region_keys_ = 32;
  uint64_t wl_ms_seen_ = 0;
  double wl_kms_seen_ = 0;

  struct ResPost {
    int32_t X, a, b;
    uint32_t seq;
    int slot;
    uint32_t nparts;
    double t_post;
  };
  void plan_resident(const TiledStream& ts);
  void free_resident();
  void drain_retired();
  void start_resident();
  uint32_t post_resident(uint32_t op, int32_t a, int32_t b, int32_t X, int slot);
  bool wait_resident(const MergeSlot& sl, int32_t X);
  int pick_resident_slot();
  bool resident_aborted() const;
  void post_resident_merge(const int32_t* ab, int32_t X0);
  void undo_resident_from(int32_t X);
  size_t collect_resident(int32_t X, const DeltaRecord** recs);
  [[noreturn]] void resident_dump(const char* why);
  bool resident_on_ = true;
  bool resident_ok_ = false;
  bool res_running_ = false;
  bool res_lds_tok_ = true;
  std::vector<ResPost> res_posted_;
  std::vector<uint32_t> res_post_parts_[kResSlots];
  int spec_depth_ = 1;
  int32_t res_abandoned_[kResSlots] = {-1, -1, -1, -1};
  int res_next_slot_ = 0;
  uint32_t res_grid_ = 0, res_tok_words_ = 0, res_w_words_ = 0;
  uint32_t res_sig_words_ = 0;
  bool res_w_global_ = false;
  size_t res_shm_ = 0;
  uint32_t* res_wg_tiles_ = nullptr;
  uint32_t* res_wg_rank_ = nullptr;
  uint32_t* res_tile_lofs_ = nullptr;
  std::vector<uint32_t> res_owner_;
  std::vector<uint32_t> res_wg_ntiles_;
  std::vector<uint32_t> res_all_;
  std::vector<uint32_t> res_wg_first_;
  std::vector<uint32_t> res_parts_;
  void* res_mbox_ = nullptr;
  void* res_mbox_dev_ = nullptr;
// ... 22 lines not shown
```

### shredword-trainer_amd/csrc/host/engine.cpp

```cpp
#include "engine.h"

#include <algorithm>
#include <string>
#include <unordered_map>

#include "common.h"

namespace shred {

void Engine::configure(size_t target_vocab_size, int32_t unk_id, uint64_t min_pair_freq) {
  target_vocab_ = target_vocab_size;
  unk_ = unk_id;
  min_freq_ = min_pair_freq;
  sel_.reset(unk_, min_freq_);
}

void Engine::forget_merges() {
  merge_a_.clear();
  merge_b_.clear();
  sel_.reset(unk_, min_freq_);
}

void Engine::refresh_selector(Backend& be) {
  if (!selector_stale_) return;
  selector_stale_ = false;
  sel_.reset(unk_, min_freq_);
  std::vector<PairCount> pairs;
  be.count_pairs(unk_, &pairs);
  sel_.add_counts(std::move(pairs));
}

void Engine::check_exact(Backend& be) {
  if (!verify_exact_ || !sel_.exact() || selector_stale_) return;
  std::vector<PairCount> fresh;
  be.count_pairs(unk_, &fresh);
  ++exact_checks_;
  const size_t bad = sel_.exact_mismatches(fresh);
  if (bad) {
    if (!exact_fail_)
      std::fprintf(stderr, "[ERROR]\t exactness check after %zu merges: %zu pair counts differ from a fresh K1\n",
                   merge_a_.size(), bad);
    ++exact_fail_;
  }
}

void Engine::count_bigrams(Backend& be) {
  refresh_selector(be);
  std::vector<PairCount> pairs;
  be.count_pairs(unk_, &pairs);
  const size_t unique = pairs.size();
  if (capture_) {
    const uint64_t n = pairs.size();
    std::fwrite("P", 1, 1, capture_);
    std::fwrite(&n, 8, 1, capture_);
    std::fwrite(pairs.data(), sizeof(PairCount), n, capture_);
  }
  sel_.add_counts(std::move(pairs));
  check_exact(be);
  if (log_ >= 1)
    std::printf("[INFO]\t Counted %zu unique pairs\n[INFO]\t Added %zu pairs to heap (freq >= %llu)\n", unique,
                sel_.heap_size(), (unsigned long long)min_freq_);
}

Engine::~Engine() { helper_stop(); }

void Engine::helper_start() {
  if (helper_ || !helper_on_) return;
  helper_ = new Helper();
  Helper* h = helper_;
  const Selector* sel = &sel_;
  h->th = std::thread([h, sel] {
    unsigned idle = 0;
    for (;;) {
      const int st = h->state.load(std::memory_order_acquire);
      if (st == 1) {
        sel->prepare(h->a, h->b, h->X, h->recs, h->n, &h->out, h->pf, h->pfm);
        h->state.store(2, std::memory_order_release);
        idle = 0;
      } else if (st == 3) {
        return;
      } else if (++idle < (1u << 20)) {
        __builtin_ia32_pause();
      } else {
        std::this_thread::yield();
      }
    }
  });
}

void Engine::helper_stop() {
  if (!helper_) return;
  helper_drain();
  helper_->state.store(3, std::memory_order_release);
  helper_->th.join();
  delete helper_;
  helper_ = nullptr;
}

void Engine::helper_drain() {
  if (!helper_) return;
  while (helper_->state.load(std::memory_order_acquire) == 1) __builtin_ia32_pause();
  helper_->state.store(0, std::memory_order_relaxed);
}

void Engine::helper_offer(Backend& be) {
  if (!helper_ || pending_.empty() || helper_->state.load(std::memory_order_acquire) != 0) return;
  const Guess& g = pending_.front();
  const DeltaRecord* recs = nullptr;
  size_t n = 0;
  if (!be.peek(g.X, &recs, &n)) return;
  Helper* h = helper_;
  h->a = g.a;
  h->b = g.b;
  h->X = g.X;
  h->recs = recs;
  h->n = n;
  h->pf = sel_.table_base();
  h->pfm = sel_.table_mask();
  h->state.store(1, std::memory_order_release);
}

void Engine::finish_speculation(Backend& be) {
  if (pending_.empty()) return;
  helper_drain();
  be.undo_guesses(pending_.front().X);
  pending_.clear();
  ++spec_misses_;
}

void Engine::verify_selection(Backend& be, int32_t a, int32_t b, uint64_t freq) {
  if (!pending_.empty()) {
    helper_drain();
    be.undo_guesses(pending_.front().X);
    pending_.clear();
  }
  uint64_t mx = 0, fab = 0;
  be.pair_max(unk_, a, b, &mx, &fab);
  ++verify_checks_;
  if (mx != freq || fab != freq) {
    if (!verify_fail_)
      std::fprintf(stderr, "[ERROR]\t argmax check at merge %zu: selected (%d,%d) freq=%llu, device recount: max=%llu, "
                   "(%d,%d)=%llu\n", merge_a_.size(), a, b, (unsigned long long)freq, (unsigned long long)mx, a, b,
                   (unsigned long long)fab);
    ++verify_fail_;
  }
}

bool Engine::merge_one(Backend& be, int remaining) {
  int32_t a, b;
  uint64_t freq;
  const bool exact = sel_.exact();
  if (!exact) {
    finish_speculation(be);
    if (!sel_.truth_live()) {
      std::vector<PairCount> pc;
      be.count_pairs(unk_, &pc);
      sel_.set_truth(pc);
    }
  }
  if (exact) helper_offer(be);
  const double t0 = now_seconds();
  const bool ok = sel_.select(&a, &b, &freq);
  const double t1 = now_seconds();
  times_.select_s += t1 - t0;
  if (!ok) {
    finish_speculation(be);
    return false;
  }
  const int32_t X = kBaseVocab + (int32_t)merge_a_.size();
  if (verify_every_ && merge_a_.size() % (size_t)verify_every_ == 0) verify_selection(be, a, b, freq);
  if (log_ >= 2)
    std::printf("[MERGE]\t Merging (%d,%d) freq=%llu -> new_id=%d (merge %zu)\n", a, b, (unsigned long long)freq, X,
                merge_a_.size() + 1);
  if (trace_) std::fprintf(trace_, "M %d %d %llu %d\n", a, b, (unsigned long long)freq, X);
  merge_a_.push_back(a);
  merge_b_.push_back(b);
  if (probe_k_) {
    std::vector<int32_t> c(2 * probe_k_);
    c.resize(2 * sel_.predict_chain(a, b, probe_window_, probe_k_, c.data()));
    chain_log_.push_back(std::move(c));
  }
  bool launched = false;
  if (!pending_.empty()) {
    const Guess& g = pending_.front();
    if (g.X == X && g.a == a && g.b == b) {
      launched = true;
      if (g.posted) be.guess_confirmed();
      pending_.erase(pending_.begin());
      ++spec_hits_;
    } else {
      finish_speculation(be);
    }
  }
  const bool spec = speculate_ && exact;
  const int chain = spec ? std::max(1, std::min(std::min(chain_max_, be.max_chain()), remaining)) : 1;
  if (!launched) {
    chain_ab_.assign(2 * (size_t)chain, 0);
    chain_ab_[0] = a;
    chain_ab_[1] = b;
    const int n = 1 + (chain > 1 ? (int)sel_.predict_chain(a, b, chain_window_, (size_t)chain - 1, chain_ab_.data() + 2) : 0);
    for (int i = 1; i < n; ++i) pending_.push_back({chain_ab_[2 * i], chain_ab_[2 * i + 1], X + i});
    ++launches_;
    be.merge_chain(chain_ab_.data(), n, X);
  }
  if (spec && chain == 1) {
    const size_t depth = early_guess_ ? 1 : (size_t)std::max(1, be.overlap_depth());
    while (pending_.size() < depth && (int)pending_.size() + 1 < remaining && be.can_overlap()) {
      used_.assign({a, b});
      for (const Guess& p : pending_) {
        used_.push_back(p.a);
        used_.push_back(p.b);
      }
      Guess g{0, 0, X + 1 + (int32_t)pending_.size(), true};
      if (!sel_.predict_avoid(used_.data(), used_.size(), pred_window_, &g.a, &g.b)) break;
      pending_.push_back(g);
      ++launches_;
      be.post_guess(g.a, g.b, g.X);
    }
  }
  const double t2 = now_seconds();
  const DeltaRecord* recs = nullptr;
  bool adopted = false;
  if (helper_) {
    const int st = helper_->state.load(std::memory_order_acquire);
    if (st != 0 && launched && helper_->X == X && helper_->a == a && helper_->b == b) {
      while (helper_->state.load(std::memory_order_acquire) == 1) __builtin_ia32_pause();
      be.collect(X, &recs);
      sel_.adopt(&helper_->out);
      helper_->state.store(0, std::memory_order_relaxed);
      adopted = true;
      ++helper_used_;
    } else if (st != 0) {
      helper_drain();
    }
  }
  const size_t n = adopted ? 0 : be.collect(X, &recs);
  const double t3 = now_seconds();
  if (capture_ && !adopted && !be.records_are_changes()) {
    const int32_t h[3] = {a, b, X};
    const uint64_t nn = n;
    std::fwrite("M", 1, 1, capture_);
    std::fwrite(h, 4, 3, capture_);
    std::fwrite(&nn, 8, 1, capture_);
    std::fwrite(recs, sizeof(DeltaRecord), n, capture_);
  }
  if (!adopted) {
    if (be.records_are_changes())
      sel_.apply_changes(a, b, X, reinterpret_cast<const Selector::Change*>(recs), n);
    else
      sel_.apply_combine(a, b, X, recs, n);
  }
  const double ta = now_seconds();
  if (correct_ && spec && chain == 1 && pending_.size() == 1 && pending_.front().X == X + 1 && remaining > 1 &&
      be.can_overlap()) {
    const Guess g = pending_.front();
    int32_t pa, pb;
    uint64_t pf = 0, gf = 0;
    uint32_t gv = 0;
    sel_.lookup(g.a, g.b, &gf, &gv);
    if (sel_.predict_after(X, gf, &pa, &pb, &pf)) {
      helper_drain();
      be.undo_guesses(g.X);
      pending_.clear();
      pending_.push_back({pa, pb, X + 1, true});
      ++launches_;
      ++corrections_;
      be.post_guess(pa, pb, X + 1);
    }
  }
  const double tb = now_seconds();
  sel_.apply_finish(a, b, X);
  const double tc = now_seconds();
  if (early_guess_ && spec && chain == 1 && pending_.size() == 1 && pending_.front().X == X + 1 && remaining > 2 &&
      be.can_overlap() && be.max_guesses() >= 2 && (uint64_t)sel_.last_records() <= early_max_records_) {
    const Guess g1 = pending_.front();
    used_.assign({g1.a, g1.b});
    Guess g{0, 0, X + 2, true};
    if (sel_.predict_avoid(used_.data(), used_.size(), pred_window_, &g.a, &g.b)) {
      pending_.push_back(g);
      ++launches_;
      be.post_guess(g.a, g.b, g.X);
    }
  }
  const double td = now_seconds();
  if (spec) helper_offer(be);
  times_.launch_s += t2 - t1;
  times_.wait_s += t3 - t2;
  if (launched) {
    times_.wait_hit_s += t3 - t2;
    ++times_.n_hit;
  } else {
    times_.wait_miss_s += t3 - t2;
    ++times_.n_miss;
  }
  const double t4 = now_seconds();
  times_.apply_s += t4 - t3;
  times_.combine_s += ta - t3;
  times_.correct_s += tb - ta;
  times_.finish_s += tc - tb;
  times_.early_s += td - tc;
  times_.offer_s += t4 - td;
  if (mtrace_on_)
    mtrace_.push_back(MergeTime{(float)(1e6 * (t1 - t0)), (float)(1e6 * (t2 - t1)), (float)(1e6 * (t3 - t2)),
                                (float)(1e6 * (t4 - t3)), (uint32_t)n, (uint8_t)(launched ? 1 : 0)});
  return true;
}

int Engine::merge_batch(Backend& be, int batch) {
  refresh_selector(be);
  if (sel_.heap_empty()) {
    if (log_ >= 2) std::printf("[INFO]\t Heap is empty, no more merges possible\n");
    return 0;
  }
  int done = 0;
  be.reserve_ids(kBaseVocab +
                 (int32_t)std::min<size_t>(merge_a_.size() + (size_t)batch,
                                           std::max<size_t>(target_vocab_, merge_a_.size() + kBaseVocab + 1)));
  while (done < batch && !sel_.heap_empty()) {
    if (!merge_one(be, batch - done)) break;
    ++done;
  }
  finish_speculation(be);
  be.quiesce();
  check_exact(be);
  return done;
}

int Engine::train_device(Backend& be, double t0) {
  sel_.reset(unk_, min_freq_);
  std::vector<PairCount> pairs;
  be.count_pairs(unk_, &pairs);
  times_.init_s += now_seconds() - t0;
  const int target = (int)target_vocab_ - kBaseVocab;
  int n = 0;
  std::vector<SelectedMerge> sm;
  const int32_t X0 = kBaseVocab + (int32_t)merge_a_.size();
  bool exhausted = false;
  if (target > 0 && !be.device_select_now()) {
    be.reserve_ids(X0 + target);
    std::unordered_map<uint64_t, uint64_t> cnt;
    cnt.reserve(2 * pairs.size() + 1024);
    std::vector<std::pair<uint64_t, uint64_t>> heap;
    heap.reserve(pairs.size());
    for (const PairCount& p : pairs) {
      const uint64_t k = pack_pair(p.a, p.b);
      cnt[k] = p.count;
      if (p.count >= min_freq_ && p.count > 0) heap.push_back({p.count, ~k});
    }
    std::make_heap(heap.begin(), heap.end());
    std::unordered_map<uint64_t, int64_t> net;
    while (n < target && !be.device_select_now()) {
      uint64_t best = 0, bk = 0;
      bool found = false;
      while (!heap.empty()) {
        std::pop_heap(heap.begin(), heap.end());
        const auto top = heap.back();
        heap.pop_back();
        const uint64_t k = ~top.second;
        const auto it = cnt.find(k);
        if (it == cnt.end() || it->second != top.first) continue;
        best = top.first;
        bk = k;
        found = true;
        break;
      }
      if (!found) {
        exhausted = true;
        break;
      }
      const int32_t a = pair_first(bk), b = pair_second(bk), X = X0 + n;
      if (verify_every_ > 0 && n % verify_every_ == 0) {
        std::vector<PairCount> fresh;
        be.count_pairs(unk_, &fresh);
        uint64_t mc = 0, mk = ~0ull;
        for (const PairCount& p : fresh) {
          const uint64_t k = pack_pair(p.a, p.b);
          if (p.count > mc || (p.count == mc && k < mk)) {
            mc = p.count;
            mk = k;
          }
        }
        ++verify_checks_;
        if (mc != best || mk != bk) {
          if (!verify_fail_)
            std::fprintf(stderr, "[ERROR]\t tiebreak=device check at merge %d (host phase): selected (%d,%d) freq=%llu, "
                         "fresh K1 max (%d,%d) freq=%llu\n", n, a, b, (unsigned long long)best, pair_first(mk),
                         pair_second(mk), (unsigned long long)mc);
          ++verify_fail_;
        }
      }
      be.merge_scan(a, b, X);
      const DeltaRecord* recs = nullptr;
      const size_t nr = be.collect(X, &recs);
      net.clear();
      if (be.records_are_changes()) {
        const auto* ch = reinterpret_cast<const Selector::Change*>(recs);
        for (size_t i = 0; i < nr; ++i) {
          const int32_t f = (int32_t)(uint32_t)(ch[i].hk >> 32), s = (int32_t)(uint32_t)ch[i].hk;
          if ((f == a && s == b) || f == unk_ || s == unk_) continue;
          net[pack_pair(f, s)] += ch[i].delta;
        }
      }
      for (size_t i = 0; i < nr && !be.records_are_changes(); ++i) {
        const uint32_t cat = recs[i].key & 3u, slot = recs[i].key >> 2;
        const int32_t id = slot == 0 ? unk_ : (int32_t)(slot - 1);
        int32_t f, s;
        switch (cat) {
          case kOldLeft: f = id; s = a; break;
          case kNewLeft: f = id; s = X; break;
          case kOldRight: f = b; s = id; break;
          default: f = X; s = id; break;
        }
        if ((f == a && s == b) || f == unk_ || s == unk_) continue;
        const int64_t d = (cat == kOldLeft || cat == kOldRight) ? -(int64_t)recs[i].sum : (int64_t)recs[i].sum;
        net[pack_pair(f, s)] += d;
      }
      for (const auto& kd : net) {
        if (kd.second == 0) continue;
        uint64_t& v = cnt[kd.first];
        v = kd.second < 0 ? (v >= (uint64_t)(-kd.second) ? v - (uint64_t)(-kd.second) : 0) : v + (uint64_t)kd.second;
        if (v >= min_freq_ && v > 0) {
          heap.push_back({v, ~kd.first});
          std::push_heap(heap.begin(), heap.end());
        }
      }
      cnt[bk] = 0;
      sm.push_back(SelectedMerge{a, b, best});
      ++n;
    }
    pairs.clear();
    for (const auto& kv : cnt)
      if (kv.second) pairs.push_back(PairCount{pair_first(kv.first), pair_second(kv.first), kv.second, 0});
    std::sort(pairs.begin(), pairs.end(), [](const PairCount& x, const PairCount& y) {
      return pack_pair(x.a, x.b) < pack_pair(y.a, y.b);
    });
    host_phase_merges_ += (uint64_t)n;
    if (verify_every_ > 0 && n > 0 && !exhausted) {
      std::vector<PairCount> fresh;
      be.count_pairs(unk_, &fresh);
      std::sort(fresh.begin(), fresh.end(), [](const PairCount& x, const PairCount& y) {
        return pack_pair(x.a, x.b) < pack_pair(y.a, y.b);
      });
      bool same = fresh.size() == pairs.size();
      for (size_t i = 0; same && i < fresh.size(); ++i)
        same = fresh[i].a == pairs[i].a && fresh[i].b == pairs[i].b && fresh[i].count == pairs[i].count;
      ++verify_checks_;
      if (!same) {
        if (!verify_fail_)
          std::fprintf(stderr, "[ERROR]\t tiebreak=device: the host counts after %d merges differ from a fresh K1\n", n);
        ++verify_fail_;
      }
    }
  }
  const int chunk = verify_every_ > 0 ? verify_every_ : target;
  const int n_host = n;
  while (n < target && !exhausted) {
    if (n > n_host) {
      pairs.clear();
      be.count_pairs(unk_, &pairs);
    }
    if (pairs.empty()) break;
    const int want = std::min(chunk, target - n);
    std::vector<SelectedMerge> part;
    const int got = be.device_select(pairs, X0 + n, want, min_freq_, &part);
    if (got < 0) {
      std::fprintf(stderr, "[ERROR]\t tiebreak=device needs the device's indexed merge loop (types layout, one GPU, "
                   "index on)\n");
      return -1;
    }
    if (verify_every_ > 0 && got > 0) {
      uint64_t mc = 0, mk = ~0ull;
      for (const PairCount& p : pairs) {
        const uint64_t k = pack_pair(p.a, p.b);
        if (p.count > mc || (p.count == mc && k < mk)) {
          mc = p.count;
          mk = k;
        }
      }
      ++verify_checks_;
      if (part[0].freq != mc || pack_pair(part[0].a, part[0].b) != mk) {
        if (!verify_fail_)
          std::fprintf(stderr, "[ERROR]\t tiebreak=device check at merge %d: selected (%d,%d) freq=%llu, fresh K1 max "
                       "(%d,%d) freq=%llu\n", n, part[0].a, part[0].b, (unsigned long long)part[0].freq,
                       pair_first(mk), (int32_t)(uint32_t)mk, (unsigned long long)mc);
        ++verify_fail_;
      }
// ... 131 lines not shown
```

### shredword-trainer_amd/csrc/host/engine.h

```cpp
#pragma once

#include <atomic>
#include <cstddef>
#include <cstdint>
#include <cstdio>
#include <thread>
#include <vector>

#include "common.h"
#include "selector.h"

namespace shred {

class Backend {
 public:
  virtual ~Backend() = default;
  virtual void count_pairs(int32_t unk_id, std::vector<PairCount>* out) = 0;
  virtual void merge_chain(const int32_t* ab, int n, int32_t X0) = 0;
  void merge_scan(int32_t a, int32_t b, int32_t X) {
    const int32_t ab[2] = {a, b};
    merge_chain(ab, 1, X);
  }
  void post_guess(int32_t a, int32_t b, int32_t X) {
    if (guesses_ >= max_guesses()) fatal("post_guess: more unconfirmed guesses than the backend holds");
    ++guesses_;
    merge_scan(a, b, X);
  }
  void guess_confirmed() {
    if (guesses_ > 0) --guesses_;
  }
  void undo_guesses(int32_t X) {
    rollback(X);
    guesses_ = 0;
  }
  int guesses_in_flight() const { return guesses_; }
  virtual size_t collect(int32_t X, const DeltaRecord** recs) = 0;
  virtual bool records_are_changes() const { return false; }
  virtual bool peek(int32_t X, const DeltaRecord** recs, size_t* n) { return false; }
  virtual int max_chain() const { return 1; }
  virtual bool can_overlap() const { return false; }
  virtual int overlap_depth() const { return 1; }
  virtual int max_guesses() const { return 1; }
  virtual void rollback(int32_t X) {}
  virtual void quiesce() {}
  virtual void reserve_ids(int32_t max_id) {}
  virtual void token_freq(size_t T, std::vector<uint64_t>* freq) = 0;
  virtual int device_select(const std::vector<PairCount>& pairs, int32_t X0, int n, uint64_t min_freq,
                            std::vector<SelectedMerge>* out) {
    return -1;
  }
  virtual bool device_select_now() const { return true; }
  virtual void pair_max(int32_t unk_id, int32_t a, int32_t b, uint64_t* max_freq, uint64_t* ab_freq) {
    std::vector<PairCount> pc;
    count_pairs(unk_id, &pc);
    *max_freq = *ab_freq = 0;
    for (const PairCount& p : pc) {
      if (p.count > *max_freq) *max_freq = p.count;
      if (p.a == a && p.b == b) *ab_freq = p.count;
    }
  }

 private:
  int guesses_ = 0;
};

struct EngineTimes {
  double init_s = 0, train_s = 0;
  double select_s = 0, launch_s = 0, wait_s = 0, apply_s = 0;
  double wait_hit_s = 0, wait_miss_s = 0;
  uint64_t n_hit = 0, n_miss = 0;
  double combine_s = 0, correct_s = 0, finish_s = 0, early_s = 0, offer_s = 0;
};

class Engine {
 public:
  void configure(size_t target_vocab_size, int32_t unk_id, uint64_t min_pair_freq);
  void reset_selection() {
    selector_stale_ = false;
    sel_.reset(unk_, min_freq_);
  }
  void reload() { sel_.reset_info(); }
  void forget_merges();

  void count_bigrams(Backend& be);
  int merge_batch(Backend& be, int batch);
  int train(Backend& be);
  void write_outputs(const std::vector<uint64_t>& freq, const char* model_path, const char* vocab_path) const;

  void set_log(int level) { log_ = level; }
  int log() const { return log_; }
  void set_trace(FILE* f) { trace_ = f; }
  size_t num_merges() const { return merge_a_.size(); }
  int32_t merge_first(size_t m) const { return merge_a_[m]; }
  int32_t merge_second(size_t m) const { return merge_b_[m]; }
  const Selector& selector() const { return sel_; }
  EngineTimes& times() { return times_; }
  void set_chain(int max_len, size_t window) {
    chain_max_ = max_len < 1 ? 1 : max_len;
    chain_window_ = window;
  }
  void set_speculation(bool on) { speculate_ = on; }
  void set_correction(bool on) { correct_ = on; }
  void set_early_guess(bool on) { early_guess_ = on; }
  void set_early_max_records(uint64_t n) { early_max_records_ = n; }
  void set_apply_helper(bool on) { helper_on_ = on; }
  void set_pred_window(size_t n) { pred_window_ = n ? n : 1; }
  uint64_t helper_used() const { return helper_used_; }
  ~Engine();
  uint64_t corrections() const { return corrections_; }
  void set_verify(int every) { verify_every_ = every < 0 ? 0 : every; }
  void set_tiebreak_device(bool on) { tiebreak_device_ = on; }
  bool tiebreak_device() const { return tiebreak_device_; }
  uint64_t verify_checks() const { return verify_checks_; }
  void set_verify_exact(bool on) { verify_exact_ = on; }
  uint64_t exact_checks() const { return exact_checks_; }
  uint64_t exact_failures() const { return exact_fail_; }
  uint64_t verify_failures() const { return verify_fail_; }
  uint64_t host_phase_merges() const { return host_phase_merges_; }
  void finish_speculation(Backend& be);
  uint64_t spec_hits() const { return spec_hits_; }
  uint64_t spec_misses() const { return spec_misses_; }
  uint64_t launches() const { return launches_; }
  void set_chain_probe(size_t k, size_t window) { probe_k_ = k; probe_window_ = window; }
  const std::vector<std::vector<int32_t>>& chain_log() const { return chain_log_; }

 private:
  bool merge_one(Backend& be, int remaining);
  void verify_selection(Backend& be, int32_t a, int32_t b, uint64_t freq);

  size_t target_vocab_ = 0;
  int32_t unk_ = 0;
  uint64_t min_freq_ = 2000;
  int log_ = 1;
  FILE* trace_ = nullptr;
  FILE* capture_ = nullptr;
  Selector sel_;
  std::vector<int32_t> merge_a_, merge_b_;
  EngineTimes times_;
  bool speculate_ = true;
  int chain_max_ = 1;
  size_t chain_window_ = 2048;
  size_t pred_window_ = 256;
  struct Guess {
    int32_t a, b, X;
    bool posted = false;
  };
  std::vector<Guess> pending_;
  std::vector<int32_t> used_;
  std::vector<int32_t> chain_ab_;
  uint64_t spec_hits_ = 0, spec_misses_ = 0, launches_ = 0;
  int verify_every_ = 0;
  bool tiebreak_device_ = false;
  int train_device(Backend& be, double t0);
  bool verify_exact_ = false;
  uint64_t exact_checks_ = 0, exact_fail_ = 0;
  void check_exact(Backend& be);
  bool selector_stale_ = false;
  void refresh_selector(Backend& be);
  bool correct_ = true;
  bool early_guess_ = false;
  uint64_t early_max_records_ = ~0ull;
  uint64_t corrections_ = 0;
  uint64_t verify_checks_ = 0, verify_fail_ = 0;
  uint64_t host_phase_merges_ = 0;
  struct Helper {
    std::thread th;
    std::atomic<int> state{0};
    int32_t a = 0, b = 0, X = 0;
    const DeltaRecord* recs = nullptr;
    size_t n = 0;
    const void* pf = nullptr;
    uint64_t pfm = 0;
    Selector::Prepared out;
  };
  Helper* helper_ = nullptr;
  bool helper_on_ = false;
  uint64_t helper_used_ = 0;
  void helper_start();
  void helper_stop();
  void helper_drain();
  void helper_offer(Backend& be);
  size_t probe_k_ = 0, probe_window_ = 256;
  std::vector<std::vector<int32_t>> chain_log_;
  struct MergeTime { float select_us, launch_us, wait_us, apply_us; uint32_t records; uint8_t hit; };
  std::vector<MergeTime> mtrace_;
  bool mtrace_on_ = false;
};

}
```

### shredword-trainer_amd/csrc/host/selector.cpp

```cpp
#include "selector.h"

#include <immintrin.h>

#include <algorithm>
#include <cstring>

#include "common.h"

namespace shred {

namespace {
__attribute__((target("bmi2"))) bool sort_ft_desc_radix(Selector::Change* c, size_t m, std::vector<uint64_t>& ka,
                                                        std::vector<uint64_t>& kb, std::vector<Selector::Change>& tmp) {
  uint64_t orv = 0, andv = ~0ull;
  for (size_t i = 0; i < m; ++i) {
    orv |= c[i].ft;
    andv &= c[i].ft;
  }
  const uint64_t live = orv & ~andv;
  const int bits = __builtin_popcountll(live);
  const int ib = 64 - __builtin_clzll((uint64_t)m);
  if (bits + ib > 64) return false;
  const uint64_t fm = bits == 64 ? ~0ull : (1ull << bits) - 1;
  ka.resize(m);
// ... 312 lines not shown
    for (;;) {
      const size_t l = 2 * i + 1;
      if (l >= n) break;
      const uint64_t lf = node_freq(rd(l));
      const uint64_t rf = l + 1 < n ? node_freq(rd(l + 1)) : 0;
      const bool right = l + 1 < n && rf > lf;
      if ((right ? rf : lf) < floor) break;
      const size_t c = l + right;
      if (!wr(i, rd(c))) return false;
      i = c;
    }
    if (!wr(i, x)) return false;
  }
  return false;
}

size_t Selector::predict_chain(int32_t a, int32_t b, size_t window, size_t k, int32_t* out) const {
  const size_t n = std::min(window, heap_size());
  const HeapNode* h = heap_.data() + 1;
  std::vector<std::pair<uint64_t, size_t>> cand;
  for (size_t i = 0; i < n; ++i) {
    const HeapEnt e{h[i].a, h[i].b, node_freq(h[i]), node_version(h[i])};
    if (e.freq < min_freq_ || e.a == unk_ || e.b == unk_) continue;
    const Info* in = find(pack_pair(e.a, e.b));
    if (!in || in->version() != e.version || in->freq() != e.freq) continue;
    cand.push_back({e.freq, i});
  }
  std::stable_sort(cand.begin(), cand.end(), [](const auto& x, const auto& y) { return x.first > y.first; });
  std::vector<int32_t> used = {a, b};
  size_t m = 0;
  for (const auto& c : cand) {
    if (m == k) break;
    const HeapNode& e = h[c.second];
    bool clash = false;
    for (int32_t u : used) clash |= e.a == u || e.b == u;
    if (clash) continue;
    out[2 * m] = e.a;
    out[2 * m + 1] = e.b;
    used.push_back(e.a);
    used.push_back(e.b);
    ++m;
  }
  return m;
}

bool Selector::select(int32_t* a, int32_t* b, uint64_t* freq) {
  while (!heap_empty()) {
    HeapEnt top = pop();
    if (!heap_empty())
      __builtin_prefetch(&table_[mix64(pack_pair(heap_[1].a, heap_[1].b)) & mask_]);
    Info& in = get(top.a, top.b);
    if (top.version != in.version()) {
      ++ctr_.stale;
      continue;
    }
    uint64_t actual = exact_ ? ((top.a == unk_ || top.b == unk_) ? 0 : in.freq()) : recount(top.a, top.b);
    if (actual != in.freq()) {
      in.set_freq(actual);
      in.bump_version();
      if (actual >= min_freq_) push(top.a, top.b, actual, in.version());
      continue;
    }
    if (actual < min_freq_) continue;
    *a = top.a;
    *b = top.b;
    *freq = actual;
    return true;
  }
  return false;
}

void Selector::apply(int32_t a, int32_t b, int32_t X, const DeltaRecord* recs, size_t n) {
  apply_combine(a, b, X, recs, n);
  apply_finish(a, b, X);
}

void Selector::prepare(int32_t a, int32_t b, int32_t X, const DeltaRecord* recs, size_t n, Prepared* p,
                       const void* prefetch_base, uint64_t prefetch_mask) const {
  const uint64_t c0 = __builtin_ia32_rdtsc();
  p->a = a;
  p->b = b;
  p->X = X;
  p->records = n;
  std::vector<Change>& changes = p->changes;
  changes.clear();
  size_t cap = 64;
  while (cap < 2 * n + 2) cap <<= 1;
  p->index.assign(cap, 0);
  uint32_t* index = p->index.data();
  const uint64_t cm = cap - 1;
  const Info* pt = static_cast<const Info*>(prefetch_base);
  for (size_t i = 0; i < n; ++i) {
    const uint32_t cat = recs[i].key & 3u;
    const uint32_t slot = recs[i].key >> 2;
    const int32_t id = slot == 0 ? unk_ : (int32_t)(slot - 1);
    int32_t first, second;
    switch (cat) {
      case kOldLeft: first = id; second = a; break;
      case kNewLeft: first = id; second = X; break;
      case kOldRight: first = b; second = id; break;
      default: first = X; second = id; break;
    }
    const uint64_t hk = ((uint64_t)(int64_t)first << 32) | (uint64_t)(int64_t)second;
    const int64_t d = (cat == kOldLeft || cat == kOldRight) ? -(int64_t)recs[i].sum : (int64_t)recs[i].sum;
    uint64_t j = mix64(hk) & cm;
    for (;;) {
      uint32_t s = index[j];
      if (!s) {
        if (pt) __builtin_prefetch(&pt[mix64(pack_pair((int32_t)(hk >> 32), (int32_t)hk)) & prefetch_mask]);
        changes.push_back({hk, d, recs[i].ft});
        index[j] = (uint32_t)changes.size();
        break;
      }
      Change& c = changes[s - 1];
      if (c.hk == hk) {
        c.delta += d;
        if (recs[i].ft < c.ft) c.ft = recs[i].ft;
        break;
      }
      j = (j + 1) & cm;
    }
  }
  const uint64_t c1 = __builtin_ia32_rdtsc();
  p->cyc_combine = c1 - c0;
  static_assert(kDeltaBuckets == 1024, "two 5-bit passes");
  const size_t nc = changes.size();
  std::vector<Change>& staged = p->staged;
  std::vector<Change>& ordered = p->ordered;
  staged.resize(nc);
  ordered.resize(nc);
  {
    uint32_t cnt[33] = {};
    for (const Change& c : changes) cnt[(c.hk & 31u) + 1]++;
    for (int k = 0; k < 32; ++k) cnt[k + 1] += cnt[k];
    for (const Change& c : changes) staged[cnt[c.hk & 31u]++] = c;
  }
  {
    uint32_t cnt[33] = {};
    for (const Change& c : staged) cnt[((c.hk >> 5) & 31u) + 1]++;
    for (int k = 0; k < 32; ++k) cnt[k + 1] += cnt[k];
    for (const Change& c : staged) ordered[cnt[(c.hk >> 5) & 31u]++] = c;
  }
  for (size_t i = 0; i < nc;) {
    const uint64_t bk = ordered[i].hk % kDeltaBuckets;
    size_t e = i + 1;
    while (e < nc && ordered[e].hk % kDeltaBuckets == bk) ++e;
    if (e - i > 16 && kHaveBmi2) {
      static thread_local std::vector<uint64_t> ka, kb;
      static thread_local std::vector<Change> tmp;
      if (sort_ft_desc_radix(ordered.data() + i, e - i, ka, kb, tmp)) {
        i = e;
        continue;
      }
    }
    if (e - i > 1) std::sort(ordered.begin() + i, ordered.begin() + e, [](const Change& x, const Change& y) { return x.ft > y.ft; });
    i = e;
  }
  p->cyc_order = __builtin_ia32_rdtsc() - c1;
}

void Selector::apply_combine(int32_t a, int32_t b, int32_t X, const DeltaRecord* recs, size_t n) {
  prepare(a, b, X, recs, n, &own_, table_.data(), mask_);
  ctr_.records += n;
  ctr_.changes += own_.changes.size();
  ctr_.cyc_combine += own_.cyc_combine;
  ctr_.cyc_order += own_.cyc_order;
}

void Selector::apply_changes(int32_t a, int32_t b, int32_t X, const Change* c, size_t n) {
  own_.a = a;
  own_.b = b;
  own_.X = X;
  own_.records = n;
  own_.ordered.assign(c, c + n);
  own_.cyc_combine = own_.cyc_order = 0;
  for (size_t i = 0; i < n; ++i)
    __builtin_prefetch(&table_[mix64(pack_pair((int32_t)(c[i].hk >> 32), (int32_t)c[i].hk)) & mask_]);
  ctr_.records += n;
  ctr_.changes += n;
}

void Selector::adopt(Prepared* p) {
  std::swap(own_, *p);
  for (const Change& c : own_.ordered)
    __builtin_prefetch(&table_[mix64(pack_pair((int32_t)(c.hk >> 32), (int32_t)c.hk)) & mask_]);
  ctr_.records += own_.records;
  ctr_.changes += own_.changes.size();
  ctr_.cyc_combine += own_.cyc_combine;
  ctr_.cyc_order += own_.cyc_order;
}

bool Selector::predict_after(int32_t X, uint64_t above, int32_t* pa, int32_t* pb, uint64_t* pf) const {
  uint64_t best_f = above;
  bool found = false;
  for (const Change& c : own_.ordered) {
    const int32_t f = (int32_t)(uint32_t)(c.hk >> 32), s = (int32_t)(uint32_t)c.hk;
    if ((f != X && s != X) || f == unk_ || s == unk_ || c.delta <= 0) continue;
    const uint64_t v = (uint64_t)c.delta;
    if (v > best_f && v >= min_freq_) {
      best_f = v;
      *pa = f;
      *pb = s;
      found = true;
    }
  }
  if (found) *pf = best_f;
  return found;
}

void Selector::apply_finish(int32_t a, int32_t b, int32_t X) {
  const uint64_t c2 = __builtin_ia32_rdtsc();
  const std::vector<Change>& ordered_ = own_.ordered;
  if (2 * (count_ + ordered_.size() + 1) > table_.size()) grow();
  pushes_.clear();
  for (const Change& c : ordered_) {
    const int32_t f = (int32_t)(uint32_t)(c.hk >> 32), s = (int32_t)(uint32_t)c.hk;
    if (f == a && s == b) continue;
    Info& in = get(f, s);
    if (c.delta < 0) {
      const uint64_t m = (uint64_t)(-c.delta);
      in.set_freq(in.freq() >= m ? in.freq() - m : 0);
    } else {
      in.set_freq(in.freq() + (uint64_t)c.delta);
    }
    if (in.freq() >= min_freq_) {
      in.bump_version();
      pushes_.push_back(HeapNode{in.fv, f, s});
    }
  }
  Info& merged = get(a, b);
  merged.set_freq(0);
  merged.bump_version();
  if (truth_live_) {
    for (const Change& c : ordered_) {
      const int32_t f = (int32_t)(uint32_t)(c.hk >> 32), s = (int32_t)(uint32_t)c.hk;
      if ((f == a && s == b) || f == unk_ || s == unk_) continue;
      uint64_t& v = truth_[pack_pair(f, s)];
      v = c.delta < 0 ? (v >= (uint64_t)(-c.delta) ? v - (uint64_t)(-c.delta) : 0) : v + (uint64_t)c.delta;
    }
    truth_[pack_pair(a, b)] = 0;
  }
  const uint64_t c3 = __builtin_ia32_rdtsc();
  ctr_.cyc_walk += c3 - c2;
  for (const HeapNode& p : pushes_) push(p.a, p.b, node_freq(p), node_version(p));
  ctr_.cyc_push += __builtin_ia32_rdtsc() - c3;
}

}
```

### shredword-trainer_amd/csrc/host/selector.h

```cpp
#pragma once

#include <sys/mman.h>

#include <cstddef>
#include <cstdint>
#include <new>
#include <unordered_map>
#include <vector>

namespace shred {

template <class T>
struct HugeAlloc {
  using value_type = T;
  static constexpr size_t kHuge = size_t(1) << 21;
  HugeAlloc() = default;
  template <class U>
  HugeAlloc(const HugeAlloc<U>&) {}
  T* allocate(size_t n) {
    const size_t bytes = n * sizeof(T);
    if (bytes < kHuge) return static_cast<T*>(::operator new(bytes));
    const size_t len = (bytes + kHuge - 1) & ~(kHuge - 1);
    char* p = static_cast<char*>(mmap(nullptr, len + kHuge, PROT_READ | PROT_WRITE, MAP_PRIVATE | MAP_ANONYMOUS, -1, 0));
    if (p == MAP_FAILED) throw std::bad_alloc();
    char* a = reinterpret_cast<char*>((reinterpret_cast<uintptr_t>(p) + kHuge - 1) & ~(uintptr_t)(kHuge - 1));
    if (a > p) munmap(p, a - p);
    if (a + len < p + len + kHuge) munmap(a + len, (p + len + kHuge) - (a + len));
    madvise(a, len, MADV_HUGEPAGE);
    return reinterpret_cast<T*>(a);
  }
  void deallocate(T* ptr, size_t n) {
    const size_t bytes = n * sizeof(T);
    if (bytes < kHuge) {
      ::operator delete(ptr);
      return;
    }
    munmap(ptr, (bytes + kHuge - 1) & ~(kHuge - 1));
  }
  template <class U>
  bool operator==(const HugeAlloc<U>&) const { return true; }
  template <class U>
  bool operator!=(const HugeAlloc<U>&) const { return false; }
};
template <class T>
using HugeVec = std::vector<T, HugeAlloc<T>>;

struct DeltaRecord {
  uint32_t key;
  uint32_t pad;
  uint64_t sum;
  uint64_t ft;
};
static_assert(sizeof(DeltaRecord) == 24, "DeltaRecord layout is shared with the device");

enum DeltaCategory : uint32_t {
  kOldLeft = 0,
  kNewLeft = 1,
  kOldRight = 2,
  kNewRight = 3,
};

struct PairCount {
  int32_t a, b;
  uint64_t count;
  uint64_t ft;
};

struct SelectedMerge {
  int32_t a, b;
  uint64_t freq;
};

class Selector {
 public:
  struct Change { uint64_t hk; int64_t delta; uint64_t ft; };
  struct Prepared {
    int32_t a = 0, b = 0, X = 0;
    size_t records = 0;
    std::vector<Change> changes, staged, ordered;
    std::vector<uint32_t> index;
    uint64_t cyc_combine = 0, cyc_order = 0;
  };
  void apply_changes(int32_t a, int32_t b, int32_t X, const Change* c, size_t n);
  void prepare(int32_t a, int32_t b, int32_t X, const DeltaRecord* recs, size_t n, Prepared* p,
               const void* prefetch_base, uint64_t prefetch_mask) const;
  const void* table_base() const { return table_.data(); }
  uint64_t table_mask() const { return mask_; }
  void adopt(Prepared* p);

  void reset(int32_t unk_id, uint64_t min_pair_freq);
  void reset_info();

  void add_counts(std::vector<PairCount> pairs);

  bool select(int32_t* a, int32_t* b, uint64_t* freq);

  void apply(int32_t a, int32_t b, int32_t X, const DeltaRecord* recs, size_t n);
  void apply_combine(int32_t a, int32_t b, int32_t X, const DeltaRecord* recs, size_t n);
  void apply_finish(int32_t a, int32_t b, int32_t X);
  bool predict_after(int32_t X, uint64_t above, int32_t* pa, int32_t* pb, uint64_t* pf) const;

  bool predict_next(int32_t a, int32_t b, size_t window, int32_t* pa, int32_t* pb) const;
  bool predict_avoid(const int32_t* used, size_t n_used, size_t window, int32_t* pa, int32_t* pb) const;
  size_t predict_chain(int32_t a, int32_t b, size_t window, size_t k, int32_t* out) const;

  void set_simulate_pops(bool on) { simulate_pops_ = on; }

  bool exact() const { return exact_; }
  size_t exact_mismatches(const std::vector<PairCount>& fresh) const;
  bool truth_live() const { return truth_live_; }
  void set_truth(const std::vector<PairCount>& pairs);

  size_t heap_size() const { return heap_.empty() ? 0 : heap_.size() - 1; }
  bool heap_empty() const { return heap_.size() <= 1; }
  uint64_t heap_top_freq() const { return heap_empty() ? 0 : node_freq(heap_[1]); }
  size_t num_pairs() const { return count_; }
  bool lookup(int32_t a, int32_t b, uint64_t* freq, uint32_t* version) const;
  int32_t unk_id() const { return unk_; }
  struct Counters {
    uint64_t pops = 0, stale = 0, pushes = 0, records = 0, changes = 0;
    uint64_t cyc_combine = 0, cyc_order = 0, cyc_walk = 0, cyc_push = 0;
  };
  const Counters& counters() const { return ctr_; }
  size_t last_records() const { return own_.records; }

 private:
  struct Info {
    uint64_t key;
    uint64_t fv;
    uint64_t freq() const { return fv >> 24; }
    uint32_t version() const { return (uint32_t)(fv & 0xFFFFFFu); }
    void set_freq(uint64_t f) {
      if (f >> 40) info_overflow();
      fv = f << 24 | (fv & 0xFFFFFFu);
    }
    void set_version(uint32_t v) { fv = (fv & ~0xFFFFFFull) | (v & 0xFFFFFFu); }
    void bump_version() {
      if ((fv & 0xFFFFFFu) == 0xFFFFFFu) info_overflow();
      ++fv;
    }
  };
  [[noreturn]] static void info_overflow();
  struct HeapEnt { int32_t a, b; uint64_t freq; uint32_t version; };
  struct HeapNode { uint64_t fv; int32_t a, b; };
  static uint64_t node_freq(const HeapNode& n) { return n.fv >> 24; }
  static uint32_t node_version(const HeapNode& n) { return (uint32_t)(n.fv & 0xFFFFFFu); }
  static constexpr uint64_t kEmptyKey = 0x8000000080000000ull;

  Info& get(int32_t a, int32_t b);
  const Info* find(uint64_t key) const;
  void push(int32_t a, int32_t b, uint64_t freq, uint32_t version);
  HeapEnt pop();
  void grow();

  int32_t unk_ = 0;
  uint64_t min_freq_ = 2000;
  HugeVec<Info> table_;
  std::vector<uint64_t> created_;
  size_t count_ = 0;
  bool exact_ = true;
  bool truth_live_ = false;
  std::unordered_map<uint64_t, uint64_t> truth_;
  uint64_t recount(int32_t a, int32_t b) const;
  uint64_t mask_ = 0;
  HugeVec<HeapNode> heap_;
  Prepared own_;
  std::vector<HeapNode> pushes_;
  bool simulate_select(const int32_t* used, size_t n_used, uint64_t floor, int32_t* pa, int32_t* pb) const;
  bool simulate_pops_ = true;
  mutable std::vector<uint32_t> ov_stamp_;
  mutable std::vector<size_t> ov_pos_;
  mutable std::vector<HeapNode> ov_node_;
  mutable uint32_t ov_gen_ = 0;
  Counters ctr_;
};

}
```

### shredword-trainer_amd/csrc/host/trainer.cpp

```cpp
#include <hip/hip_runtime.h>

#include <cstdio>
#include <cstdlib>
#include <algorithm>
#include <cstring>
#include <memory>
#include <string>
#include <vector>

#include "../../../include/shredword_bpe.h"
#include "common.h"
#include "corpus.h"
#include "device.h"
#include "dist.h"
#include "engine.h"
#include "tiles.h"

using namespace shred;

struct Trainer {
  BPEConfig config{};
  WordTable wt;
  bool loaded = false;
  bool device_stale = true;
// ... 396 lines not shown
  if (!t || !ensure_device(t, "shred_debug_tokens")) return -1;
  std::vector<int32_t> v;
  t->dev->download_tokens(&v);
  if (out) std::memcpy(out, v.data(), std::min(cap, v.size()) * sizeof(int32_t));
  return (int64_t)v.size();
}

int64_t shred_index_trace(Trainer* t, uint32_t* out, size_t cap) {
  if (!t || !t->dev) return -1;
  const WordLoop* wl = t->dev->word_loop();
  if (!wl) return 0;
  const std::vector<uint32_t>& v = wl->trace();
  if (out) std::memcpy(out, v.data(), std::min(cap, v.size()) * sizeof(uint32_t));
  return (int64_t)v.size();
}

int shred_get_stats(const Trainer* tc, ShredStats* s) {
  if (!tc || !s) return -1;
  Trainer* t = const_cast<Trainer*>(tc);
  std::memset(s, 0, sizeof(*s));
  const EngineTimes& et = t->engine.times();
  s->load_seconds = t->load_s;
  s->init_seconds = et.init_s;
  s->train_seconds = et.train_s;
  s->host_select_seconds = et.select_s;
  s->host_launch_seconds = et.launch_s;
  s->host_wait_seconds = et.wait_s;
  s->host_apply_seconds = et.apply_s;
  s->host_apply_combine_seconds = et.combine_s;
  s->host_apply_correct_seconds = et.correct_s;
  s->host_apply_finish_seconds = et.finish_s;
  s->host_apply_early_seconds = et.early_s;
  s->host_apply_offer_seconds = et.offer_s;
  if (t->dev) {
    const KernelTimes& k = t->dev->times();
    s->merge_kernel_ms = k.merge_ms;
    s->count_kernel_ms = k.count_ms;
    s->merge_kernel_bytes = k.merge_bytes;
    s->count_kernel_bytes = k.count_bytes;
    s->merge_launches = k.merge_launches;
    s->count_launches = k.count_launches;
    s->hist_kernel_ms = k.hist_ms;
    s->hist_kernel_bytes = k.hist_bytes;
    s->hist_launches = k.hist_launches;
    s->device_bytes = t->dev->device_bytes();
    s->num_tiles = t->dev->num_tiles();
    s->live_tokens = t->dev->live_tokens();
    s->resident_launches = t->dev->resident_launches();
    s->resident_ms = t->dev->resident_ms();
    s->resident_latency_us = t->dev->resident_latency_us();
    s->resident_aborts = t->dev->resident_aborts();
    s->resident_merges = k.res_merges;
    s->resident_bytes = k.res_bytes;
    s->resident_k3_bytes = k.res_k3_bytes;
    s->resident_kernel_ms = k.res_ms;
    if (const WordLoop* wl = t->dev->word_loop()) {
      const WordLoopStats& w = wl->stats();
      s->index_on = t->dev->index_eligible() ? 1 : 0;
      s->index_merges = w.merges;
      s->index_undos = w.undos;
      s->index_launches = w.launches;
      s->index_candidates = w.candidates;
      s->index_changed = w.changed;
      s->index_occurrences = w.occurrences;
      s->index_ms = w.kernel_ms;
      s->index_dev_us = w.dev_us;
      s->index_wait_us = w.wait_us;
      s->index_dev_lookup_us = w.dev_lookup_us;
      s->index_dev_scan_us = w.dev_scan_us;
      s->index_scanned = w.scanned;
      s->index_build_us = w.build_us;
      s->index_no_sub = w.no_sub;
      s->index_staged = w.staged;
      s->index_run_ints_read = w.run_ints_read;
      s->index_run_ints_written = w.run_ints_written;
      s->index_records = w.records;
      s->index_raw_records = w.raw_records;
      s->index_finalized = w.finalized;
      s->index_dev_out_us = w.dev_out_us;
      s->index_dev_fin_us = w.dev_fin_us;
      s->index_fin_records = w.fin_records;
      s->index_spill_merges = w.spill_merges;
      s->index_spill_keys = w.spill_keys;
      s->index_switch_merge = t->dev->switch_merge();
      s->index_switch_ms = t->dev->switch_ms();
      const SelectStats& q = wl->select_stats();
      s->sel_merges = q.merges;
      s->sel_launches = q.launches;
      s->sel_rebuilds = q.rebuilds;
      s->sel_kernel_ms = q.kernel_ms;
      s->sel_rebuild_ms = q.rebuild_ms;
      s->sel_select_us = q.select_us;
      s->sel_merge_us = q.merge_us;
      s->sel_table_us = q.table_us;
      s->sel_table_pairs = q.table_pairs;
      s->sel_table_slots = q.table_slots;
      s->sel_table_grows = q.grows;
    }
  }
  {
    s->load_on_gpu = t->wt.counted_on_gpu ? 1 : 0;
  }
  s->num_words = t->wt.num_words();
  s->num_symbols = t->wt.num_symbols();
  s->num_occurrences = t->wt.total_occurrences;
  s->num_merges = t->engine.num_merges();
  s->sel_host_merges = t->engine.host_phase_merges();
  s->heap_size = t->engine.selector().heap_size();
  const Selector::Counters& c = t->engine.selector().counters();
  s->heap_pops = c.pops;
  s->heap_stale_pops = c.stale;
  s->heap_pushes = c.pushes;
  s->delta_records = c.records;
  s->apply_cycles_combine = c.cyc_combine;
  s->apply_cycles_order = c.cyc_order;
  s->apply_cycles_walk = c.cyc_walk;
  s->apply_cycles_push = c.cyc_push;
  s->helper_adopted = t->engine.helper_used();
  if (t->dev) s->tiles_visited = t->dev->visited_tiles();
  if (t->dev) s->exchange_overflows = t->dev->exchange_overflows();
  s->spec_hits = t->engine.spec_hits();
  s->spec_misses = t->engine.spec_misses();
  s->verify_checks = t->engine.verify_checks();
  s->verify_failures = t->engine.verify_failures();
  s->layout = (int32_t)t->layout;
  s->world_size = dist_active() ? dist_state().world : 1;
  return 0;
}

int shred_device_count(void) {
  int n = 0;
  if (hipGetDeviceCount(&n) != hipSuccess) return 0;
  return n;
}

int shred_hbm_probe(int device, size_t bytes, int reps, double* read_gbps, double* copy_gbps) {
  return Device::hbm_probe(device, bytes, reps, read_gbps, copy_gbps);
}

void* shred_occupy(int device, int free_cus, double max_seconds) { return Device::occupy(device, free_cus, max_seconds); }
void shred_release(void* handle) { Device::release(handle); }

int shred_dist_unique_id(void* out, size_t cap) { return dist_unique_id(out, cap); }
int shred_dist_init(int rank, int world, const void* id, size_t len, int device) {
  return dist_init(rank, world, id, len, device);
}
int shred_dist_finalize(void) { return dist_finalize(); }
int shred_dist_ranks(void) { return dist_comm_ranks(); }

}
```

### shredword-trainer_amd/csrc/host/word_loop.h

```cpp
#pragma once

#include <cstddef>
#include <cstdint>
#include <vector>

#include "selector.h"
#include "tiles.h"

namespace shred {

struct WordLoopStats {
  uint64_t merges = 0;
  uint64_t undos = 0;
  uint64_t candidates = 0;
  uint64_t scanned = 0;
  uint64_t changed = 0;
  uint64_t occurrences = 0;
  uint64_t launches = 0;
  double kernel_ms = 0;
  double dev_us = 0;
  double dev_lookup_us = 0;
  double dev_scan_us = 0;
  double wait_us = 0;
  double build_us = 0;
  uint64_t no_sub = 0;
  uint64_t staged = 0;
  uint64_t run_ints_read = 0;
  uint64_t run_ints_written = 0;
  uint64_t records = 0;
  uint64_t raw_records = 0;
  uint64_t finalized = 0;
  double dev_rel_us = 0;
  double dev_out_us = 0;
  double dev_fin_us = 0;
  uint64_t fin_records = 0;
  uint64_t spill_merges = 0;
  uint64_t spill_keys = 0;
};

struct SelectStats {
  uint64_t merges = 0, launches = 0, rebuilds = 0;
  double kernel_ms = 0, rebuild_ms = 0;
  double select_us = 0, merge_us = 0;
  double table_us = 0;
  double rec_us = 0, append_us = 0, tail_us = 0;
  double log_ms = 0;
  uint64_t log_entries = 0;
  uint64_t listed = 0, changed = 0, occurrences = 0, new_pairs = 0;
  uint64_t table_slots = 0, table_pairs = 0, frontier_max = 0;
  uint64_t grows = 0;
};

class WordLoop {
 public:
  static constexpr int kSlots = 4;

  WordLoop(int ordinal, void* stream, int32_t unk_id);
  ~WordLoop();
  WordLoop(const WordLoop&) = delete;
  WordLoop& operator=(const WordLoop&) = delete;

  bool upload(const TiledStream& ts, const uint64_t* d_weight);
  bool ready() const { return ready_; }
  void reset();
  bool load_current(const TiledStream& ts);
  void rebuild() { build_index(); }
  void load_tiles(const int32_t* tok, const uint64_t* tile_off, const uint32_t* tile_len);
  void reset_words();
  void reserve(int32_t max_id);

  void post_merge(int32_t a, int32_t b, int32_t X);
  size_t collect(int32_t X, const DeltaRecord** recs);
  bool last_changes() const { return last_changes_; }
  void set_finalize(uint32_t n) { fin_max_ = n; }
  uint32_t finalize_max() const { return fin_max_; }
  bool peek(int32_t X, const DeltaRecord** recs, size_t* n) const;
  void rollback(int32_t X);
  size_t in_flight() const { return posted_.size(); }
  uint32_t id_room() const { return cap_; }
  int run_select(const std::vector<PairCount>& pairs, int32_t X0, uint32_t n_max, uint64_t min_freq,
                 std::vector<SelectedMerge>* out);
  const SelectStats& select_stats() const { return sst_; }
  void stop();
  bool running() const { return running_; }
  void set_stream(void* s) {
    if (running_) stop();
    stream_ = s;
  }

  void sync_tiles(int32_t* tok, const uint64_t* tile_off, uint32_t* tile_len);
  bool tiles_dirty() const { return dirty_; }
  void mark_tiles_current() { dirty_ = false; }

  const WordLoopStats& stats() const { return st_; }
  void clear_stats() {
    st_ = WordLoopStats();
    const uint64_t slots = sst_.table_slots;
    sst_ = SelectStats();
    sst_.table_slots = slots;
    trace_.clear();
  }
  static constexpr int kTraceFields = 37;
  const std::vector<uint32_t>& trace() const { return trace_; }
  void set_timing(bool on) { timing_ = on; }
  size_t device_bytes() const { return bytes_; }
  uint32_t words() const { return nwords_; }
  uint64_t initial_keys() const { return init_keys_n_; }
  uint64_t pool_used() const;

 private:
  struct Slot {
    DeltaRecord* host_recs = nullptr;
    void* dev_recs = nullptr;
    uint32_t* host_hdr = nullptr;
    void* dev_hdr = nullptr;
    uint32_t rec_cap = 0;
  };
  struct Post {
    int32_t X, a, b;
    uint32_t seq;
    double t_post;
  };
  void free_all();
  void build_index();
  void restore_index();
  void launch(uint32_t seq0);
  void recover_timeout();
  uint32_t post(uint32_t op, int32_t a, int32_t b, int32_t X, uint32_t loff = 0, uint32_t lcnt1 = 0);
  void wait_flag(const Slot& s, uint32_t seq);
  bool handed_over(const Slot& s, uint32_t seq) const;
  void ensure_slots(uint32_t cap);

  int ordinal_ = 0;
  void* stream_ = nullptr;
  int32_t unk_ = 0;
  bool ready_ = false, running_ = false, dirty_ = false, timing_ = false;
  std::vector<uint64_t> lists_;
  double t_epoch_ = now_seconds();

  uint32_t nwords_ = 0;
  uint64_t nint_ = 0;
  uint64_t ntok_ = 0;
  uint32_t ntiles_ = 0;
  int32_t* wtok_ = nullptr;
  int32_t* wtok0_ = nullptr;
  uint32_t* woff_ = nullptr;
  std::vector<uint32_t> woff_h_;
  const unsigned long long* weight_ = nullptr;
  uint32_t* tile_first_ = nullptr;
  uint32_t* tile_nw_ = nullptr;
  unsigned long long* pool_ = nullptr;
  uint64_t pool_cap_ = 0;
  unsigned long long* dkey_ = nullptr;
  unsigned long long* dval_ = nullptr;
  uint64_t dir_cap_ = 0;
  unsigned long long* init_key_ = nullptr;
  unsigned long long* init_val_ = nullptr;
  uint64_t init_keys_n_ = 0;
  uint64_t init_pool_n_ = 0;
  unsigned long long* lst_ = nullptr;
  uint32_t* lseq_ = nullptr;
  uint32_t id_cap_ = 0;
  unsigned long long* dsum_ = nullptr;
  unsigned long long* dft_ = nullptr;
  uint32_t* dlist_ = nullptr;
  uint32_t* dstate_ = nullptr;
  uint32_t cap_ = 0;

  Slot slot_[kSlots];
  void* ring_ = nullptr;
  void* ring_dev_ = nullptr;
  uint32_t* status_ = nullptr;
  void* status_dev_ = nullptr;
  uint32_t seq_ = 0;
  uint32_t idle_polls_ = 1u << 22;
  bool sel_report_ = false;
  uint32_t fin_max_ = 0;
  uint32_t fin_min_ = 0;
  bool prefetch_ = true;
  bool drain_ = false;
  int probes_ = 32;
  bool fast_ = true;
  bool last_changes_ = false;
  std::vector<Post> posted_;
  void sel_free();
  bool sel_rebuild(uint64_t min_freq);
  unsigned long long* ptab_ = nullptr;
  uint64_t pcap_ = 0;
  uint32_t* fr_[2] = {nullptr, nullptr};
  uint32_t fcap_ = 0;
  uint32_t* sst_dev_ = nullptr;
  unsigned long long* thr_ = nullptr;
  unsigned long long* sout_ = nullptr;
  uint64_t sout_cap_ = 0;
  uint32_t* upd_ = nullptr;
  uint64_t upd_cap_ = 0;
  uint32_t* shist_ = nullptr;
  uint32_t* scol_ = nullptr;
  uint64_t scol_cap_ = 0;
  SelectStats sst_;
  void* ev_[2] = {};
  WordLoopStats st_;
  std::vector<uint32_t> trace_;
  size_t bytes_ = 0;
};

}
```

### shredword-trainer_amd/shredword/cbase.py

```python
import ctypes
import os
import sysconfig
from ctypes import (POINTER, Structure, c_bool, c_char_p, c_double, c_float, c_int, c_int32, c_int64,
                    c_size_t, c_uint32, c_uint64, c_void_p)


def _get_lib_path():
    env = os.environ.get("SHREDWORD_LIB")
    if env:
        return os.path.abspath(env)
    pkg_dir = os.path.dirname(os.path.abspath(__file__))
    names = ("libtrainer", "trainer")
    exts = [e for e in (".so", ".pyd", ".dll", ".dylib", sysconfig.get_config_var("EXT_SUFFIX")) if e]
    search = [pkg_dir, os.path.join(pkg_dir, "lib"), os.path.join(pkg_dir, "..", "build")]
    for d in search:
        if not os.path.isdir(d):
            continue
        for root, _dirs, files in os.walk(d):
            for f in sorted(files):
                if f.startswith(names) and any(f.endswith(e) for e in exts):
                    return os.path.abspath(os.path.join(root, f))
    available = []
    for d in search:
        if os.path.isdir(d):
            available.extend(os.listdir(d))
    raise FileNotFoundError(f"Could not find trainer library in {search}. Available files: {available}")


_lib_path = _get_lib_path()
lib = ctypes.CDLL(_lib_path, mode=getattr(ctypes, "RTLD_GLOBAL", 0))

MIN_HEAP_SIZE, MAX_OCCS_PER_MERGE, INITIAL_VOCAB_SIZE, INITIAL_STR_SIZE = 4096, 50000, 256, 4096


class BPEConfig(Structure):
    _fields_ = [("target_vocab_size", c_size_t), ("unk_id", c_int32),
                ("character_coverage", c_float), ("min_pair_freq", c_uint64)]


class ShredStats(Structure):
    _fields_ = [("load_seconds", c_double), ("init_seconds", c_double), ("train_seconds", c_double),
                ("host_select_seconds", c_double), ("host_launch_seconds", c_double),
                ("host_wait_seconds", c_double), ("host_apply_seconds", c_double),
                ("merge_kernel_ms", c_double), ("count_kernel_ms", c_double),
                ("merge_kernel_bytes", c_double), ("count_kernel_bytes", c_double),
                ("merge_launches", c_uint64), ("count_launches", c_uint64),
                ("num_words", c_uint64), ("num_symbols", c_uint64), ("num_occurrences", c_uint64),
                ("num_merges", c_uint64), ("heap_size", c_uint64), ("live_tokens", c_uint64),
                ("device_bytes", c_uint64), ("num_tiles", c_uint64),
                ("layout", c_int32), ("world_size", c_int32),
                ("heap_pops", c_uint64), ("heap_stale_pops", c_uint64), ("heap_pushes", c_uint64),
                ("delta_records", c_uint64), ("tiles_visited", c_uint64),
                ("apply_cycles_combine", c_uint64), ("apply_cycles_order", c_uint64),
                ("apply_cycles_walk", c_uint64),
                ("spec_hits", c_uint64), ("spec_misses", c_uint64),
                ("exchange_overflows", c_uint64),
                ("hist_kernel_ms", c_double), ("hist_kernel_bytes", c_double), ("hist_launches", c_uint64),
                ("resident_launches", c_uint64), ("resident_ms", c_double), ("resident_latency_us", c_double),
                ("load_on_gpu", c_uint64),
                ("index_on", c_uint64), ("index_merges", c_uint64), ("index_undos", c_uint64),
                ("index_launches", c_uint64), ("index_candidates", c_uint64), ("index_changed", c_uint64),
                ("index_occurrences", c_uint64), ("index_ms", c_double), ("index_dev_us", c_double),
                ("index_wait_us", c_double),
                ("index_dev_lookup_us", c_double), ("index_dev_scan_us", c_double),
                ("index_scanned", c_uint64), ("index_build_us", c_double), ("index_no_sub", c_uint64),
                ("index_staged", c_uint64), ("index_switch_merge", c_int64), ("index_switch_ms", c_double),
                ("resident_aborts", c_uint64), ("verify_checks", c_uint64), ("verify_failures", c_uint64),
                ("resident_merges", c_uint64), ("resident_bytes", c_double), ("resident_kernel_ms", c_double),
                ("index_run_ints_read", c_uint64), ("index_run_ints_written", c_uint64),
                ("index_records", c_uint64), ("resident_k3_bytes", c_double),
                ("sel_merges", c_uint64), ("sel_launches", c_uint64), ("sel_rebuilds", c_uint64),
                ("sel_kernel_ms", c_double), ("sel_rebuild_ms", c_double), ("sel_select_us", c_double),
                ("sel_merge_us", c_double), ("sel_table_pairs", c_uint64), ("sel_table_slots", c_uint64),
                ("sel_host_merges", c_uint64), ("sel_table_grows", c_uint64),
                ("index_raw_records", c_uint64), ("index_finalized", c_uint64),
                ("index_dev_out_us", c_double), ("index_dev_fin_us", c_double), ("index_fin_records", c_uint64),
                ("sel_table_us", c_double), ("index_spill_merges", c_uint64), ("index_spill_keys", c_uint64),
                ("host_apply_combine_seconds", c_double), ("host_apply_correct_seconds", c_double),
                ("host_apply_finish_seconds", c_double), ("host_apply_early_seconds", c_double),
                ("host_apply_offer_seconds", c_double), ("helper_adopted", c_uint64),
                ("apply_cycles_push", c_uint64)]


Trainer = c_void_p

lib.create_trainer.argtypes, lib.create_trainer.restype = [POINTER(BPEConfig)], Trainer
lib.bpe_trainer_destroy.argtypes, lib.bpe_trainer_destroy.restype = [Trainer], None
lib.bpe_init.argtypes, lib.bpe_init.restype = [Trainer], None
lib.bpe_count_bigrams.argtypes, lib.bpe_count_bigrams.restype = [Trainer], None
lib.bpe_load_corpus.argtypes, lib.bpe_load_corpus.restype = [Trainer, c_char_p], c_int
lib.bpe_merge_batch.argtypes, lib.bpe_merge_batch.restype = [Trainer, c_int], c_int
lib.bpe_train.argtypes, lib.bpe_train.restype = [Trainer], c_int
lib.bpe_save.argtypes, lib.bpe_save.restype = [Trainer, c_char_p, c_char_p], None

lib.trainerCreate.argtypes, lib.trainerCreate.restype = [c_int, c_float, c_int, c_int], c_void_p
lib.trainerDestroy.argtypes, lib.trainerDestroy.restype = [c_void_p], None
lib.addTextToTrainer.argtypes, lib.addTextToTrainer.restype = [c_void_p, c_char_p], c_bool
lib.preprocessTexts.argtypes, lib.preprocessTexts.restype = [c_void_p], c_bool
lib.extractInitialSubwords.argtypes, lib.extractInitialSubwords.restype = [c_void_p], c_bool
lib.computeLoss.argtypes, lib.computeLoss.restype = [c_void_p, POINTER(c_char_p), c_int], c_float
lib.computeTokenLoss.argtypes, lib.computeTokenLoss.restype = [c_void_p, c_char_p, POINTER(c_char_p), c_int], c_double
lib.pruneVocabStep.argtypes, lib.pruneVocabStep.restype = [c_void_p, POINTER(c_char_p), c_int, c_double], c_bool
lib.updateTokenScores.argtypes, lib.updateTokenScores.restype = [c_void_p, POINTER(c_char_p), c_int], c_bool
lib.trainUnigram.argtypes, lib.trainUnigram.restype = [c_void_p, POINTER(c_char_p), c_int, c_int], c_bool
lib.getVocab.argtypes, lib.getVocab.restype = [c_void_p, POINTER(POINTER(c_char_p)), POINTER(POINTER(c_double)), POINTER(c_int)], c_bool
lib.saveVocab.argtypes, lib.saveVocab.restype = [c_void_p, c_char_p], c_bool
lib.loadVocab.argtypes, lib.loadVocab.restype = [c_void_p, c_char_p], c_bool

lib.shred_set_option.argtypes, lib.shred_set_option.restype = [Trainer, c_char_p, c_char_p], c_int
lib.shred_reset.argtypes, lib.shred_reset.restype = [Trainer], c_int
GATHER_FN = ctypes.CFUNCTYPE(ctypes.c_void_p, ctypes.c_void_p, ctypes.c_void_p, ctypes.c_size_t,
                             ctypes.POINTER(ctypes.c_size_t))
lib.shred_set_load_gather.argtypes = [Trainer, c_int, c_int, GATHER_FN, ctypes.c_void_p]
lib.shred_set_load_gather.restype = c_int
lib.shred_probe_merge.argtypes, lib.shred_probe_merge.restype = [Trainer, c_int32, c_int32, c_int], c_double
if hasattr(lib, "shred_probe_rollback"):
    lib.shred_probe_rollback.argtypes, lib.shred_probe_rollback.restype = [Trainer, c_int32, c_int32], c_int
    lib.shred_debug_tokens.argtypes, lib.shred_debug_tokens.restype = [Trainer, POINTER(c_int32), c_size_t], c_int64
    lib.shred_index_trace.argtypes, lib.shred_index_trace.restype = [Trainer, POINTER(c_uint32), c_size_t], c_int64
lib.shred_get_stats.argtypes, lib.shred_get_stats.restype = [Trainer, POINTER(ShredStats)], c_int
lib.shred_device_count.argtypes, lib.shred_device_count.restype = [], c_int
lib.shred_hbm_probe.argtypes = [c_int, c_size_t, c_int, POINTER(c_double), POINTER(c_double)]
lib.shred_hbm_probe.restype = c_int
lib.shred_occupy.argtypes, lib.shred_occupy.restype = [c_int, c_int, c_double], c_void_p
lib.shred_release.argtypes, lib.shred_release.restype = [c_void_p], None
lib.shred_dist_unique_id.argtypes, lib.shred_dist_unique_id.restype = [c_void_p, c_size_t], c_int
lib.shred_dist_init.argtypes, lib.shred_dist_init.restype = [c_int, c_int, c_void_p, c_size_t, c_int], c_int
lib.shred_dist_finalize.argtypes, lib.shred_dist_finalize.restype = [], c_int
lib.shred_dist_ranks.argtypes, lib.shred_dist_ranks.restype = [], c_int

Encoder = c_void_p
lib.shred_encoder_create.argtypes = [POINTER(c_int32), c_size_t, POINTER(c_int32), c_int]
lib.shred_encoder_create.restype = Encoder
lib.shred_encoder_load.argtypes, lib.shred_encoder_load.restype = [c_char_p, c_char_p, c_int32, c_int], Encoder
lib.shred_encoder_destroy.argtypes, lib.shred_encoder_destroy.restype = [Encoder], None
lib.shred_encoder_info.argtypes = [Encoder, POINTER(c_size_t), POINTER(c_int32)]
lib.shred_encoder_info.restype = c_int
lib.shred_encode.argtypes = [Encoder, c_void_p, c_size_t, c_void_p, c_size_t]
lib.shred_encode.restype = c_int64
lib.shred_encode_device.argtypes = [Encoder, c_void_p, c_size_t, c_void_p, c_size_t, c_void_p, POINTER(c_double)]
lib.shred_encode_device.restype = c_int64
lib.shred_decode.argtypes = [Encoder, c_void_p, c_size_t, c_void_p, c_size_t]
lib.shred_decode.restype = c_int64
lib.shred_encoder_token_lengths.argtypes = [Encoder, POINTER(c_int32), c_size_t]
lib.shred_encoder_token_lengths.restype = c_int
lib.shred_encode_spans.argtypes = [Encoder, c_void_p, c_size_t, c_void_p, c_size_t, c_void_p, c_void_p, c_size_t,
                                   POINTER(c_size_t)]
lib.shred_encode_spans.restype = c_int64
lib.shred_encode_spans_device.argtypes = [Encoder, c_void_p, c_size_t, c_void_p, c_size_t, c_void_p, c_void_p,
                                          c_size_t, POINTER(c_size_t), c_void_p, POINTER(c_double)]
lib.shred_encode_spans_device.restype = c_int64
lib.shred_encoder_set_specials.argtypes = [Encoder, c_void_p, POINTER(c_size_t), c_size_t]
lib.shred_encoder_set_specials.restype = c_int
lib.shred_encoder_num_specials.argtypes, lib.shred_encoder_num_specials.restype = [Encoder], c_size_t
lib.shred_encode_special.argtypes = lib.shred_encode_spans.argtypes
lib.shred_encode_special.restype = c_int64
lib.shred_encode_special_device.argtypes = lib.shred_encode_spans_device.argtypes
lib.shred_encode_special_device.restype = c_int64
lib.shred_encode_docs.argtypes = [Encoder, c_void_p, c_size_t, c_void_p, c_size_t, c_int, c_void_p, c_size_t,
                                  c_void_p, c_void_p]
lib.shred_encode_docs.restype = c_int64
lib.shred_encode_docs_device.argtypes = lib.shred_encode_docs.argtypes + [c_void_p, POINTER(c_double)]
lib.shred_encode_docs_device.restype = c_int64
lib.shred_decode_device.argtypes = [Encoder, c_void_p, c_size_t, c_void_p, c_size_t, c_void_p, c_size_t, c_void_p,
# ... 24 lines not shown
```

Baseline: 65840.

## Emit pair-delta changes from word-loop kernel so host can skip combine

```diff
diff --git a/include/shredword_bpe.h b/include/shredword_bpe.h
--- a/include/shredword_bpe.h
+++ b/include/shredword_bpe.h
@@ -117,6 +117,9 @@
   double host_apply_combine_seconds, host_apply_correct_seconds, host_apply_finish_seconds;
   double host_apply_early_seconds, host_apply_offer_seconds;
   uint64_t helper_adopted, apply_cycles_push;
+  uint64_t index_change_merges;
+  uint64_t index_needs_combine;
+  uint64_t apply_combines;
 } ShredStats;
 int shred_get_stats(const Trainer* trainer, ShredStats* out);
 
diff --git a/shredword-trainer_amd/csrc/hip/bpe_device.hip b/shredword-trainer_amd/csrc/hip/bpe_device.hip
--- a/shredword-trainer_amd/csrc/hip/bpe_device.hip
+++ b/shredword-trainer_amd/csrc/hip/bpe_device.hip
@@ -1543,10 +1543,12 @@
 
 size_t Device::collect(int32_t X, const DeltaRecord** recs) {
   HIP_OK(hipSetDevice(ordinal_));
-  last_changes_ = false;
+  last_form_ = RecordForm::kRecords;
+  last_needs_combine_ = true;
   if (wl_ && wl_->in_flight()) {
     const size_t n = wl_->collect(X, recs);
-    last_changes_ = wl_->last_changes();
+    last_form_ = wl_->last_form();
+    last_needs_combine_ = wl_->last_needs_combine();
     records_total_ += n;
     records_max_ = std::max<uint64_t>(records_max_, n);
     return n;
@@ -1571,6 +1573,9 @@
 bool Device::peek(int32_t X, const DeltaRecord** recs, size_t* n) {
   return wl_ && wl_->in_flight() && wl_->peek(X, recs, n);
 }
+
+RecordForm Device::peek_form() const { return wl_ ? wl_->peek_form() : RecordForm::kRecords; }
+bool Device::peek_needs_combine() const { return wl_ ? wl_->peek_needs_combine() : true; }
 
 void Device::rollback(int32_t X) {
   HIP_OK(hipSetDevice(ordinal_));
diff --git a/shredword-trainer_amd/csrc/hip/word_loop.hip b/shredword-trainer_amd/csrc/hip/word_loop.hip
--- a/shredword-trainer_amd/csrc/hip/word_loop.hip
+++ b/shredword-trainer_amd/csrc/hip/word_loop.hip
@@ -85,6 +85,13 @@
   u64 sig;
 };
 __host__ __device__ __forceinline__ u64 hand_weight(uint32_t i) { return 0x9E3779B97F4A7C15ull + 2ull * i; }
+__host__ __device__ __forceinline__ u64 hand_tag(uint32_t seq) { return (u64)seq * 0xD6E8FEB86659FD93ull; }
+__host__ __device__ __forceinline__ u64 hand_term(u64 w, uint32_t i, u64 tag) {
+  u64 x = w + tag;
+  x ^= x >> 32;
+  x *= hand_weight(i);
+  return x ^ (x >> 29);
+}
 constexpr int kCksWord = 30;
 constexpr int kGroupShift = 28;
 constexpr u64 kWordMask = (1ull << kGroupShift) - 1;
@@ -150,6 +157,7 @@
   uint32_t prefetch;
   uint32_t drain;
   uint32_t fast;
+  uint32_t changes;
   WlSlotDev sl[WordLoop::kSlots];
   SelParams sel;
 };
@@ -462,6 +470,7 @@
   alignas(16) uint32_t hs[32];
   uint32_t cmd[8];
   uint32_t nout, nchg, pool_top, err, scan, filter, nspill, qn, nkeys, nfin;
+  uint32_t clash;
   uint32_t rd, wr;
   u64 lst_x;
   u64 last_lst;
@@ -489,14 +498,20 @@
 static_assert(3 * kFinTab * 8 <= (uint32_t)(kStrip * kWlThreads * 4), "combine table in the strip");
 static_assert(kDeltaBucketsDev * 4 <= kDh * 4, "bucket counters in the hash keys");
 
-__device__ __forceinline__ void fin_record(u64* q, uint32_t r, uint32_t key, u64 sum, u64 ft, int32_t unk, int32_t a,
-                                           int32_t b, int32_t X) {
+__device__ __forceinline__ bool rec_change(uint32_t key, u64 sum, int32_t unk, int32_t a, int32_t b, int32_t X,
+                                           u64* hk, u64* delta) {
   const uint32_t sl = key >> 2, cat = key & 3u;
   const int32_t id = sl == 0 ? unk : (int32_t)(sl - 1u);
   const int32_t f = cat < 2u ? id : (cat == 2u ? b : X);
   const int32_t g = cat == 0u ? a : (cat == 1u ? X : id);
-  q[r] = ((u64)(int64_t)f << 32) | (u64)(int64_t)g;
-  q[kFinMax + r] = (cat & 1u) ? sum : (u64)(-(int64_t)sum);
+  *hk = ((u64)(int64_t)f << 32) | (u64)(int64_t)g;
+  *delta = (cat & 1u) ? sum : (u64)(-(int64_t)sum);
+  return id == (cat < 2u ? b : a) || id == X || (id < 0 && cat >= 2u);
+}
+
+__device__ __forceinline__ void fin_record(u64* q, uint32_t r, uint32_t key, u64 sum, u64 ft, int32_t unk, int32_t a,
+                                           int32_t b, int32_t X) {
+  rec_change(key, sum, unk, a, b, X, &q[r], &q[kFinMax + r]);
   q[2 * kFinMax + r] = ft;
 }
 
@@ -901,6 +916,7 @@
         S.lk[1] = err ? 0 : cnt;
         S.need = need;
         S.nout = 0;
+        S.clash = 0;
         S.nchg = 0;
         S.scan = 0;
         S.rd = 0;
@@ -1024,14 +1040,25 @@
           uint32_t ri = incl - nb;
           WL_ST(if (lane == 0) S.xs[13] = (uint32_t)(__builtin_amdgcn_s_memrealtime() - t_cmd);)
           u64 cks = 0;
+          const u64 tag = hand_tag(seq);
+          const bool as_chg = p.changes != 0;
+          bool clash = false;
           for (; bw; bw &= bw - 1u, ++ri) {
             const uint32_t h = (uint32_t)lane * 32u + (uint32_t)__builtin_ctz(bw);
             u64* dst = reinterpret_cast<u64*>(sd.recs + ri);
-            const u64 w0 = (u64)s_h.key[h], w1 = s_h.sum[h], w2 = s_h.ft[h];
+            u64 w0 = (u64)s_h.key[h], w1 = s_h.sum[h];
+            const u64 w2 = s_h.ft[h];
+            u64 hk, dl;
+            const bool cl = rec_change((uint32_t)w0, w1, p.unk, a, b, X, &hk, &dl);
+            if (as_chg) {
+              w0 = hk;
+              w1 = dl;
+              clash |= cl;
+            }
             dst[0] = w0;
             dst[1] = w1;
             dst[2] = w2;
-            cks += w0 * hand_weight(16u + 3u * ri) + w1 * hand_weight(17u + 3u * ri) + w2 * hand_weight(18u + 3u * ri);
+            cks += hand_term(w0, 16u + 3u * ri, tag) + hand_term(w1, 17u + 3u * ri, tag) + hand_term(w2, 18u + 3u * ri, tag);
             s_h.key[h] = kEmpty32;
             s_h.sum[h] = 0;
             s_h.ft[h] = kEmpty64;
@@ -1042,12 +1069,20 @@
             const u64 sum = atomicExch(&p.dsum[key], 0ull);
             const u64 ft = atomicExch(&p.dft[key], kEmpty64);
             u64* dst = reinterpret_cast<u64*>(sd.recs + nk + i);
-            dst[0] = (u64)key;
-            dst[1] = sum;
+            u64 w0 = (u64)key, w1 = sum, hk, dl;
+            const bool cl = rec_change(key, sum, p.unk, a, b, X, &hk, &dl);
+            if (as_chg) {
+              w0 = hk;
+              w1 = dl;
+              clash |= cl;
+            }
+            dst[0] = w0;
+            dst[1] = w1;
             dst[2] = ft;
             const uint32_t r = nk + i;
-            cks += (u64)key * hand_weight(16u + 3u * r) + sum * hand_weight(17u + 3u * r) + ft * hand_weight(18u + 3u * r);
+            cks += hand_term(w0, 16u + 3u * r, tag) + hand_term(w1, 17u + 3u * r, tag) + hand_term(ft, 18u + 3u * r, tag);
           }
+          const uint32_t form = as_chg ? (2u | (__ballot(clash) != 0ull ? 0x100u : 0u)) : 0u;
           WL_ST(if (lane == 0) S.xs[10] = (uint32_t)(__builtin_amdgcn_s_memrealtime() - t_cmd);)
           if (lane == 0) {
             S.lst_x = 0;
@@ -1077,7 +1112,7 @@
             hs[19] = nsp;
             hs[20] = (uint32_t)(S.t_idle + (t_cmd - t_wait));
             hs[21] = (uint32_t)S.t_undo;
-            hs[22] = 0u;
+            hs[22] = form;
             hs[23] = nk + nsp;
             hs64[12] = S.lst_x;
             hs64[13] = t_cmd;
@@ -1091,7 +1126,7 @@
             const int4 hv = reinterpret_cast<const int4*>(S.hs)[lane];
             reinterpret_cast<int4*>(sd.hdr)[lane] = hv;
             const u64 lo = (u64)(uint32_t)hv.x | ((u64)(uint32_t)hv.y << 32), hi = (u64)(uint32_t)hv.z | ((u64)(uint32_t)hv.w << 32);
-            cks += lo * hand_weight(2u * lane) + hi * hand_weight(2u * lane + 1u);
+            cks += hand_term(lo, 2u * lane, tag) + hand_term(hi, 2u * lane + 1u, tag);
           }
           {
             cks += dpp64<0x111>(cks);
@@ -1412,13 +1447,22 @@
     } else {
       const uint32_t rt = pfon ? (tid < 64u ? tid : tid - 64u) : tid;
       const uint32_t rs = pfon ? (uint32_t)kWlThreads - 64u : (uint32_t)kWlThreads;
+      const bool as_chg = p.changes != 0;
+      bool clash = false;
       for (uint32_t i = rt; i < (uint32_t)kDh; i += rs) {
         const uint32_t key = s_h.key[i];
         if (key == kEmpty32) continue;
         const uint32_t r = atomicAdd(&S.nout, 1u);
         u64* dst = reinterpret_cast<u64*>(sd.recs + r);
-        dst[0] = (u64)key;
-        dst[1] = s_h.sum[i];
+        u64 w0 = (u64)key, w1 = s_h.sum[i], hk, dl;
+        const bool cl = rec_change(key, w1, p.unk, a, b, X, &hk, &dl);
+        if (as_chg) {
+          w0 = hk;
+          w1 = dl;
+          clash |= cl;
+        }
+        dst[0] = w0;
+        dst[1] = w1;
         dst[2] = s_h.ft[i];
         s_h.key[i] = kEmpty32;
         s_h.sum[i] = 0;
@@ -1431,10 +1475,18 @@
         const u64 ft = atomicExch(&p.dft[key], kEmpty64);
         const uint32_t r = atomicAdd(&S.nout, 1u);
         u64* dst = reinterpret_cast<u64*>(sd.recs + r);
-        dst[0] = (u64)key;
-        dst[1] = sum;
+        u64 w0 = (u64)key, w1 = sum, hk, dl;
+        const bool cl = rec_change(key, sum, p.unk, a, b, X, &hk, &dl);
+        if (as_chg) {
+          w0 = hk;
+          w1 = dl;
+          clash |= cl;
+        }
+        dst[0] = w0;
+        dst[1] = w1;
         dst[2] = ft;
       }
+      if (clash) S.clash = 1u;
       asm volatile("s_waitcnt vmcnt(0)" ::: "memory");
     }
     asm volatile("s_waitcnt lgkmcnt(0)\n\ts_barrier" ::: "memory");
@@ -1447,7 +1499,7 @@
       }
     if (tid == 0) {
       sd.hdr[0] = fin ? S.nfin : S.nout;
-      sd.hdr[22] = fin ? 1u : 0u;
+      sd.hdr[22] = fin ? 1u : (p.changes != 0 ? (2u | (S.clash ? 0x100u : 0u)) : 0u);
       sd.hdr[23] = nrec;
       sd.hdr[30] = (uint32_t)(__builtin_amdgcn_s_memrealtime() - t_fin);
       sd.hdr[2] = (uint32_t)cnt;
@@ -1750,6 +1802,7 @@
   if (const char* e = std::getenv("SHREDWORD_WL_DRAIN")) drain_ = std::atoi(e) != 0;
   if (const char* e = std::getenv("SHREDWORD_WL_PROBES")) probes_ = std::atoi(e);
   if (const char* e = std::getenv("SHREDWORD_WL_FAST")) fast_ = std::atoi(e) != 0;
+  if (const char* e = std::getenv("SHREDWORD_WL_CHANGES")) changes_ = std::atoi(e) != 0;
   if (const char* e = std::getenv("SHREDWORD_SELECT_REPORT")) sel_report_ = std::atoi(e) != 0;
   for (auto& e : ev_) {
     hipEvent_t ev;
@@ -2148,6 +2201,7 @@
   p.prefetch = prefetch_ ? 1u : 0u;
   p.drain = drain_ ? 1u : 0u;
   p.fast = fast_ ? 1u : 0u;
+  p.changes = changes_ ? 1u : 0u;
   for (int k = 0; k < kSlots; ++k) {
     p.sl[k].recs = static_cast<DeltaRecord*>(slot_[k].dev_recs);
     p.sl[k].hdr = static_cast<uint32_t*>(slot_[k].dev_hdr);
@@ -2209,10 +2263,11 @@
   const uint64_t want = (g0 & 0xFFFFFFFFull) | (g1 << 32);
   const uint32_t n = __atomic_load_n(&sl.host_hdr[0], __ATOMIC_ACQUIRE);
   if (n > sl.rec_cap) return false;
+  const uint64_t tag = hand_tag(seq);
   uint64_t c = 0;
-  for (uint32_t i = 0; i < 16; ++i) c += __atomic_load_n(&h64[i], __ATOMIC_RELAXED) * hand_weight(i);
+  for (uint32_t i = 0; i < 16; ++i) c += hand_term(__atomic_load_n(&h64[i], __ATOMIC_RELAXED), i, tag);
   const uint64_t* r = reinterpret_cast<const uint64_t*>(sl.host_recs);
-  for (uint32_t i = 0; i < 3 * n; ++i) c += __atomic_load_n(&r[i], __ATOMIC_RELAXED) * hand_weight(16u + i);
+  for (uint32_t i = 0; i < 3 * n; ++i) c += hand_term(__atomic_load_n(&r[i], __ATOMIC_RELAXED), 16u + i, tag);
   return c == want;
 }
 
@@ -2223,7 +2278,12 @@
   unsigned spins = 0;
   for (;;) {
     if (__atomic_load_n(flag, __ATOMIC_ACQUIRE) == seq) break;
-    if ((uint32_t)(__atomic_load_n(&h64[kCksWord + 1], __ATOMIC_ACQUIRE) >> 32) == seq && handed_over(sl, seq)) break;
+    if ((uint32_t)(__atomic_load_n(&h64[kCksWord + 1], __ATOMIC_ACQUIRE) >> 32) == seq) {
+      if (handed_over(sl, seq)) break;
+      if ((uint32_t)(__atomic_load_n(&h64[kCksWord], __ATOMIC_ACQUIRE) >> 32) == seq &&
+          __atomic_load_n(&sl.host_hdr[0], __ATOMIC_ACQUIRE) > sl.rec_cap)
+        fatal("k_word_loop: record overflow");
+    }
     __builtin_ia32_pause();
     if (++spins % 4096 != 0) continue;
     const uint32_t st = __atomic_load_n(&status_[0], __ATOMIC_ACQUIRE);
@@ -2257,17 +2317,24 @@
   st_.run_ints_read += h[14];
   st_.run_ints_written += h[15];
   st_.records += h[0];
-  st_.raw_records += h[22] ? h[23] : h[0];
-  st_.finalized += h[22] ? 1u : 0u;
+  const uint32_t form = h[22] & 0xFFu;
+  const bool fin = form == 1u;
+  st_.raw_records += fin ? h[23] : h[0];
+  st_.finalized += fin ? 1u : 0u;
   st_.dev_out_us += 1e-2 * (double)h[30];
   st_.dev_rel_us += 1e-2 * (double)h[31];
   st_.spill_merges += h[19] ? 1u : 0u;
   st_.spill_keys += h[19];
-  if (h[22]) {
+  if (fin) {
     st_.dev_fin_us += 1e-2 * (double)h[30];
     st_.fin_records += h[23];
   }
-  last_changes_ = h[22] != 0;
+  last_form_ = fin ? RecordForm::kOrderedChanges : form == 2u ? RecordForm::kUnorderedChanges : RecordForm::kRecords;
+  last_needs_combine_ = form != 2u || (h[22] & 0x100u) != 0;
+  if (form == 2u) {
+    ++st_.change_merges;
+    st_.needs_combine += (h[22] & 0x100u) ? 1u : 0u;
+  }
   st_.changed += h[3];
   st_.occurrences += h64[2];
   st_.dev_us += 1e-2 * (double)h64[3];
@@ -2297,7 +2364,10 @@
   if (__atomic_load_n(sl.host_hdr + 1, __ATOMIC_ACQUIRE) != posted_.front().seq &&
       !handed_over(sl, posted_.front().seq))
     return false;
-  if (sl.host_hdr[22]) return false;
+  const uint32_t form = sl.host_hdr[22];
+  if ((form & 0xFFu) == 1u) return false;
+  peek_form_ = (form & 0xFFu) == 2u ? RecordForm::kUnorderedChanges : RecordForm::kRecords;
+  peek_needs_combine_ = (form & 0xFFu) != 2u || (form & 0x100u) != 0;
   const size_t k = sl.host_hdr[0];
   if (k > sl.rec_cap) return false;
   *recs = sl.host_recs;
diff --git a/shredword-trainer_amd/csrc/host/device.h b/shredword-trainer_amd/csrc/host/device.h
--- a/shredword-trainer_amd/csrc/host/device.h
+++ b/shredword-trainer_amd/csrc/host/device.h
@@ -63,7 +63,11 @@
   };
   void set_exchange(const Exchange& x);
   size_t collect(int32_t X, const DeltaRecord** recs) override;
-  bool records_are_changes() const override { return last_changes_; }
+  bool records_are_changes() const override { return last_form_ == RecordForm::kOrderedChanges; }
+  RecordForm record_form() const override { return last_form_; }
+  bool needs_combine() const override { return last_needs_combine_; }
+  RecordForm peek_form() const override;
+  bool peek_needs_combine() const override;
   bool peek(int32_t X, const DeltaRecord** recs, size_t* n) override;
   static constexpr int kChainMax = 8;
   int max_chain() const override {
@@ -277,7 +281,8 @@
   int32_t max_id_seen_ = 0;
   int32_t max_id0_ = 0;
   bool speculate_ = true;
-  bool last_changes_ = false;
+  RecordForm last_form_ = RecordForm::kRecords;
+  bool last_needs_combine_ = true;
   int64_t fin_ = -1;
   uint64_t rollbacks_ = 0;
 
diff --git a/shredword-trainer_amd/csrc/host/engine.cpp b/shredword-trainer_amd/csrc/host/engine.cpp
--- a/shredword-trainer_amd/csrc/host/engine.cpp
+++ b/shredword-trainer_amd/csrc/host/engine.cpp
@@ -65,7 +65,7 @@
 Engine::~Engine() { helper_stop(); }
 
 void Engine::helper_start() {
-  if (helper_ || !helper_on_) return;
+  if (helper_ || !helper_on_ || capture_) return;
   helper_ = new Helper();
   Helper* h = helper_;
   const Selector* sel = &sel_;
@@ -74,7 +74,11 @@
     for (;;) {
       const int st = h->state.load(std::memory_order_acquire);
       if (st == 1) {
-        sel->prepare(h->a, h->b, h->X, h->recs, h->n, &h->out, h->pf, h->pfm);
+        if (h->changes)
+          sel->prepare_changes(h->a, h->b, h->X, reinterpret_cast<const Selector::Change*>(h->recs), h->n,
+                               h->needs_combine, &h->out, h->pf, h->pfm);
+        else
+          sel->prepare(h->a, h->b, h->X, h->recs, h->n, &h->out, h->pf, h->pfm);
         h->state.store(2, std::memory_order_release);
         idle = 0;
       } else if (st == 3) {
@@ -115,6 +119,8 @@
   h->X = g.X;
   h->recs = recs;
   h->n = n;
+  h->changes = be.peek_form() == RecordForm::kUnorderedChanges;
+  h->needs_combine = be.peek_needs_combine();
   h->pf = sel_.table_base();
   h->pfm = sel_.table_mask();
   h->state.store(1, std::memory_order_release);
@@ -236,17 +242,22 @@
   }
   const size_t n = adopted ? 0 : be.collect(X, &recs);
   const double t3 = now_seconds();
-  if (capture_ && !adopted && !be.records_are_changes()) {
+  const RecordForm form = adopted ? RecordForm::kRecords : be.record_form();
+  if (capture_ && !adopted && form != RecordForm::kOrderedChanges) {
     const int32_t h[3] = {a, b, X};
-    const uint64_t nn = n;
-    std::fwrite("M", 1, 1, capture_);
+    const uint64_t nn = n, nc = be.needs_combine() ? 1 : 0;
+    std::fwrite(form == RecordForm::kRecords ? "M" : "C", 1, 1, capture_);
     std::fwrite(h, 4, 3, capture_);
     std::fwrite(&nn, 8, 1, capture_);
+    if (form != RecordForm::kRecords) std::fwrite(&nc, 8, 1, capture_);
+    static_assert(sizeof(DeltaRecord) == sizeof(Selector::Change), "one hand-off buffer, either form");
     std::fwrite(recs, sizeof(DeltaRecord), n, capture_);
   }
   if (!adopted) {
-    if (be.records_are_changes())
+    if (form == RecordForm::kOrderedChanges)
       sel_.apply_changes(a, b, X, reinterpret_cast<const Selector::Change*>(recs), n);
+    else if (form == RecordForm::kUnorderedChanges)
+      sel_.apply_unordered(a, b, X, reinterpret_cast<const Selector::Change*>(recs), n, be.needs_combine());
     else
       sel_.apply_combine(a, b, X, recs, n);
   }
@@ -393,7 +404,8 @@
       const DeltaRecord* recs = nullptr;
       const size_t nr = be.collect(X, &recs);
       net.clear();
-      if (be.records_are_changes()) {
+      const bool as_changes = be.record_form() != RecordForm::kRecords;
+      if (as_changes) {
         const auto* ch = reinterpret_cast<const Selector::Change*>(recs);
         for (size_t i = 0; i < nr; ++i) {
           const int32_t f = (int32_t)(uint32_t)(ch[i].hk >> 32), s = (int32_t)(uint32_t)ch[i].hk;
@@ -401,7 +413,7 @@
           net[pack_pair(f, s)] += ch[i].delta;
         }
       }
-      for (size_t i = 0; i < nr && !be.records_are_changes(); ++i) {
+      for (size_t i = 0; i < nr && !as_changes; ++i) {
         const uint32_t cat = recs[i].key & 3u, slot = recs[i].key >> 2;
         const int32_t id = slot == 0 ? unk_ : (int32_t)(slot - 1);
         int32_t f, s;
diff --git a/shredword-trainer_amd/csrc/host/engine.h b/shredword-trainer_amd/csrc/host/engine.h
--- a/shredword-trainer_amd/csrc/host/engine.h
+++ b/shredword-trainer_amd/csrc/host/engine.h
@@ -36,6 +36,12 @@
   int guesses_in_flight() const { return guesses_; }
   virtual size_t collect(int32_t X, const DeltaRecord** recs) = 0;
   virtual bool records_are_changes() const { return false; }
+  virtual RecordForm record_form() const {
+    return records_are_changes() ? RecordForm::kOrderedChanges : RecordForm::kRecords;
+  }
+  virtual bool needs_combine() const { return true; }
+  virtual RecordForm peek_form() const { return RecordForm::kRecords; }
+  virtual bool peek_needs_combine() const { return true; }
   virtual bool peek(int32_t X, const DeltaRecord** recs, size_t* n) { return false; }
   virtual int max_chain() const { return 1; }
   virtual bool can_overlap() const { return false; }
@@ -169,6 +175,7 @@
     int32_t a = 0, b = 0, X = 0;
     const DeltaRecord* recs = nullptr;
     size_t n = 0;
+    bool changes = false, needs_combine = true;
     const void* pf = nullptr;
     uint64_t pfm = 0;
     Selector::Prepared out;
diff --git a/shredword-trainer_amd/csrc/host/selector.cpp b/shredword-trainer_amd/csrc/host/selector.cpp
--- a/shredword-trainer_amd/csrc/host/selector.cpp
+++ b/shredword-trainer_amd/csrc/host/selector.cpp
@@ -418,6 +418,7 @@
   p->b = b;
   p->X = X;
   p->records = n;
+  p->combines = 1;
   std::vector<Change>& changes = p->changes;
   changes.clear();
   size_t cap = 64;
@@ -459,17 +460,78 @@
   }
   const uint64_t c1 = __builtin_ia32_rdtsc();
   p->cyc_combine = c1 - c0;
+  order_changes(changes.data(), changes.size(), p, nullptr, 0);
+  p->cyc_order = __builtin_ia32_rdtsc() - c1;
+}
+
+void Selector::prepare_changes(int32_t a, int32_t b, int32_t X, const Change* c, size_t n, bool needs_combine,
+                               Prepared* p, const void* prefetch_base, uint64_t prefetch_mask) const {
+  const uint64_t c0 = __builtin_ia32_rdtsc();
+  p->a = a;
+  p->b = b;
+  p->X = X;
+  p->records = n;
+  p->combines = needs_combine ? 1 : 0;
+  if (!needs_combine) {
+    p->cyc_combine = 0;
+    order_changes(c, n, p, prefetch_base, prefetch_mask);
+    p->cyc_order = __builtin_ia32_rdtsc() - c0;
+    return;
+  }
+  std::vector<Change>& changes = p->changes;
+  changes.clear();
+  size_t cap = 64;
+  while (cap < 2 * n + 2) cap <<= 1;
+  p->index.assign(cap, 0);
+  uint32_t* index = p->index.data();
+  const uint64_t cm = cap - 1;
+  const Info* pt = static_cast<const Info*>(prefetch_base);
+  for (size_t i = 0; i < n; ++i) {
+    const uint64_t hk = c[i].hk;
+    uint64_t j = mix64(hk) & cm;
+    for (;;) {
+      uint32_t s = index[j];
+      if (!s) {
+        if (pt) __builtin_prefetch(&pt[mix64(pack_pair((int32_t)(hk >> 32), (int32_t)hk)) & prefetch_mask]);
+        changes.push_back(c[i]);
+        index[j] = (uint32_t)changes.size();
+        break;
+      }
+      Change& e = changes[s - 1];
+      if (e.hk == hk) {
+        e.delta += c[i].delta;
+        if (c[i].ft < e.ft) e.ft = c[i].ft;
+        break;
+      }
+      j = (j + 1) & cm;
+    }
+  }
+  const uint64_t c1 = __builtin_ia32_rdtsc();
+  p->cyc_combine = c1 - c0;
+  order_changes(changes.data(), changes.size(), p, nullptr, 0);
+  p->cyc_order = __builtin_ia32_rdtsc() - c1;
+}
+
+void Selector::order_changes(const Change* src, size_t nc, Prepared* p, const void* prefetch_base,
+                             uint64_t prefetch_mask) {
   static_assert(kDeltaBuckets == 1024, "two 5-bit passes");
-  const size_t nc = changes.size();
   std::vector<Change>& staged = p->staged;
   std::vector<Change>& ordered = p->ordered;
   staged.resize(nc);
   ordered.resize(nc);
   {
     uint32_t cnt[33] = {};
-    for (const Change& c : changes) cnt[(c.hk & 31u) + 1]++;
+    if (const Info* pt = static_cast<const Info*>(prefetch_base)) {
+      for (size_t i = 0; i < nc; ++i) {
+        const uint64_t hk = src[i].hk;
+        __builtin_prefetch(&pt[mix64(pack_pair((int32_t)(hk >> 32), (int32_t)hk)) & prefetch_mask]);
+        cnt[(hk & 31u) + 1]++;
+      }
+    } else {
+      for (size_t i = 0; i < nc; ++i) cnt[(src[i].hk & 31u) + 1]++;
+    }
     for (int k = 0; k < 32; ++k) cnt[k + 1] += cnt[k];
-    for (const Change& c : changes) staged[cnt[c.hk & 31u]++] = c;
+    for (size_t i = 0; i < nc; ++i) staged[cnt[src[i].hk & 31u]++] = src[i];
   }
   {
     uint32_t cnt[33] = {};
@@ -492,13 +554,22 @@
     if (e - i > 1) std::sort(ordered.begin() + i, ordered.begin() + e, [](const Change& x, const Change& y) { return x.ft > y.ft; });
     i = e;
   }
-  p->cyc_order = __builtin_ia32_rdtsc() - c1;
 }
 
 void Selector::apply_combine(int32_t a, int32_t b, int32_t X, const DeltaRecord* recs, size_t n) {
   prepare(a, b, X, recs, n, &own_, table_.data(), mask_);
-  ctr_.records += n;
-  ctr_.changes += own_.changes.size();
+  count_prepared();
+}
+
+void Selector::apply_unordered(int32_t a, int32_t b, int32_t X, const Change* c, size_t n, bool needs_combine) {
+  prepare_changes(a, b, X, c, n, needs_combine, &own_, table_.data(), mask_);
+  count_prepared();
+}
+
+void Selector::count_prepared() {
+  ctr_.records += own_.records;
+  ctr_.changes += own_.ordered.size();
+  ctr_.combines += own_.combines;
   ctr_.cyc_combine += own_.cyc_combine;
   ctr_.cyc_order += own_.cyc_order;
 }
@@ -510,6 +581,7 @@
   own_.records = n;
   own_.ordered.assign(c, c + n);
   own_.cyc_combine = own_.cyc_order = 0;
+  own_.combines = 0;
   for (size_t i = 0; i < n; ++i)
     __builtin_prefetch(&table_[mix64(pack_pair((int32_t)(c[i].hk >> 32), (int32_t)c[i].hk)) & mask_]);
   ctr_.records += n;
@@ -520,10 +592,7 @@
   std::swap(own_, *p);
   for (const Change& c : own_.ordered)
     __builtin_prefetch(&table_[mix64(pack_pair((int32_t)(c.hk >> 32), (int32_t)c.hk)) & mask_]);
-  ctr_.records += own_.records;
-  ctr_.changes += own_.changes.size();
-  ctr_.cyc_combine += own_.cyc_combine;
-  ctr_.cyc_order += own_.cyc_order;
+  count_prepared();
 }
 
 bool Selector::predict_after(int32_t X, uint64_t above, int32_t* pa, int32_t* pb, uint64_t* pf) const {
diff --git a/shredword-trainer_amd/csrc/host/selector.h b/shredword-trainer_amd/csrc/host/selector.h
--- a/shredword-trainer_amd/csrc/host/selector.h
+++ b/shredword-trainer_amd/csrc/host/selector.h
@@ -60,6 +60,12 @@
   kNewRight = 3,
 };
 
+enum class RecordForm : uint32_t {
+  kRecords = 0,
+  kOrderedChanges = 1,
+  kUnorderedChanges = 2,
+};
+
 struct PairCount {
   int32_t a, b;
   uint64_t count;
@@ -80,10 +86,13 @@
     std::vector<Change> changes, staged, ordered;
     std::vector<uint32_t> index;
     uint64_t cyc_combine = 0, cyc_order = 0;
+    uint64_t combines = 0;
   };
   void apply_changes(int32_t a, int32_t b, int32_t X, const Change* c, size_t n);
   void prepare(int32_t a, int32_t b, int32_t X, const DeltaRecord* recs, size_t n, Prepared* p,
                const void* prefetch_base, uint64_t prefetch_mask) const;
+  void prepare_changes(int32_t a, int32_t b, int32_t X, const Change* c, size_t n, bool needs_combine, Prepared* p,
+                       const void* prefetch_base, uint64_t prefetch_mask) const;
   const void* table_base() const { return table_.data(); }
   uint64_t table_mask() const { return mask_; }
   void adopt(Prepared* p);
@@ -97,7 +106,9 @@
 
   void apply(int32_t a, int32_t b, int32_t X, const DeltaRecord* recs, size_t n);
   void apply_combine(int32_t a, int32_t b, int32_t X, const DeltaRecord* recs, size_t n);
+  void apply_unordered(int32_t a, int32_t b, int32_t X, const Change* c, size_t n, bool needs_combine);
   void apply_finish(int32_t a, int32_t b, int32_t X);
+  const std::vector<Change>& ordered_changes() const { return own_.ordered; }
   bool predict_after(int32_t X, uint64_t above, int32_t* pa, int32_t* pb, uint64_t* pf) const;
 
   bool predict_next(int32_t a, int32_t b, size_t window, int32_t* pa, int32_t* pb) const;
@@ -119,6 +130,7 @@
   int32_t unk_id() const { return unk_; }
   struct Counters {
     uint64_t pops = 0, stale = 0, pushes = 0, records = 0, changes = 0;
+    uint64_t combines = 0;
     uint64_t cyc_combine = 0, cyc_order = 0, cyc_walk = 0, cyc_push = 0;
   };
   const Counters& counters() const { return ctr_; }
@@ -165,6 +177,9 @@
   uint64_t mask_ = 0;
   HugeVec<HeapNode> heap_;
   Prepared own_;
+  static void order_changes(const Change* src, size_t nc, Prepared* p, const void* prefetch_base,
+                            uint64_t prefetch_mask);
+  void count_prepared();
   std::vector<HeapNode> pushes_;
   bool simulate_select(const int32_t* used, size_t n_used, uint64_t floor, int32_t* pa, int32_t* pb) const;
   bool simulate_pops_ = true;
diff --git a/shredword-trainer_amd/csrc/host/trainer.cpp b/shredword-trainer_amd/csrc/host/trainer.cpp
--- a/shredword-trainer_amd/csrc/host/trainer.cpp
+++ b/shredword-trainer_amd/csrc/host/trainer.cpp
@@ -502,6 +502,8 @@
       s->index_fin_records = w.fin_records;
       s->index_spill_merges = w.spill_merges;
       s->index_spill_keys = w.spill_keys;
+      s->index_change_merges = w.change_merges;
+      s->index_needs_combine = w.needs_combine;
       s->index_switch_merge = t->dev->switch_merge();
       s->index_switch_ms = t->dev->switch_ms();
       const SelectStats& q = wl->select_stats();
@@ -536,6 +538,7 @@
   s->apply_cycles_order = c.cyc_order;
   s->apply_cycles_walk = c.cyc_walk;
   s->apply_cycles_push = c.cyc_push;
+  s->apply_combines = c.combines;
   s->helper_adopted = t->engine.helper_used();
   if (t->dev) s->tiles_visited = t->dev->visited_tiles();
   if (t->dev) s->exchange_overflows = t->dev->exchange_overflows();
diff --git a/shredword-trainer_amd/csrc/host/word_loop.h b/shredword-trainer_amd/csrc/host/word_loop.h
--- a/shredword-trainer_amd/csrc/host/word_loop.h
+++ b/shredword-trainer_amd/csrc/host/word_loop.h
@@ -36,6 +36,8 @@
   uint64_t fin_records = 0;
   uint64_t spill_merges = 0;
   uint64_t spill_keys = 0;
+  uint64_t change_merges = 0;
+  uint64_t needs_combine = 0;
 };
 
 struct SelectStats {
@@ -71,7 +73,10 @@
 
   void post_merge(int32_t a, int32_t b, int32_t X);
   size_t collect(int32_t X, const DeltaRecord** recs);
-  bool last_changes() const { return last_changes_; }
+  RecordForm last_form() const { return last_form_; }
+  bool last_needs_combine() const { return last_needs_combine_; }
+  RecordForm peek_form() const { return peek_form_; }
+  bool peek_needs_combine() const { return peek_needs_combine_; }
   void set_finalize(uint32_t n) { fin_max_ = n; }
   uint32_t finalize_max() const { return fin_max_; }
   bool peek(int32_t X, const DeltaRecord** recs, size_t* n) const;
@@ -181,7 +186,11 @@
   bool drain_ = false;
   int probes_ = 32;
   bool fast_ = true;
-  bool last_changes_ = false;
+  bool changes_ = true;
+  RecordForm last_form_ = RecordForm::kRecords;
+  bool last_needs_combine_ = true;
+  mutable RecordForm peek_form_ = RecordForm::kRecords;
+  mutable bool peek_needs_combine_ = true;
   std::vector<Post> posted_;
   void sel_free();
   bool sel_rebuild(uint64_t min_freq);
diff --git a/shredword-trainer_amd/shredword/cbase.py b/shredword-trainer_amd/shredword/cbase.py
--- a/shredword-trainer_amd/shredword/cbase.py
+++ b/shredword-trainer_amd/shredword/cbase.py
@@ -79,7 +79,9 @@
                 ("host_apply_combine_seconds", c_double), ("host_apply_correct_seconds", c_double),
                 ("host_apply_finish_seconds", c_double), ("host_apply_early_seconds", c_double),
                 ("host_apply_offer_seconds", c_double), ("helper_adopted", c_uint64),
-                ("apply_cycles_push", c_uint64)]
+                ("apply_cycles_push", c_uint64),
+                ("index_change_merges", c_uint64), ("index_needs_combine", c_uint64),
+                ("apply_combines", c_uint64)]
 
 
 Trainer = c_void_p
```

New measurement: 68180, median of 5. +3.6%, better.
